# danihae/bio-image-unet

Hardware: AMD Instinct MI355X
Metric: voxels/sec fwd+bwd (higher is better)
Workload: dtype bf16; 1 GPU; cfg4: UNet3D(in_channels=1, out_channels=1, n_filter=32) input (4, 1, 128, 128, 128) per GPU, train step = forward + reference loss + backward + Adam; parallelism=dp1

## Files before the change

bio_image_unet_amd/_lib.py:

```python
from __future__ import annotations

import ctypes as C
import os

import torch

_HERE = os.path.dirname(os.path.abspath(__file__))
LIB_PATH = os.environ.get("BIU_LIB_PATH") or os.path.join(_HERE, "libbiu_hip.so")

BIU_F32, BIU_BF16 = 0, 1
BN_MAX_PARTIALS = 1024


class BiuError(RuntimeError):
    pass


class biu_act(C.Structure):
    _fields_ = [("p", C.c_void_p), ("n", C.c_int32), ("d", C.c_int32), ("h", C.c_int32), ("w", C.c_int32),
                ("c", C.c_int32), ("pitch", C.c_int32)]


class biu_pack_job(C.Structure):
    _fields_ = [("w", C.c_void_p), ("packed", C.c_void_p), ("transposed", C.c_int32), ("kind", C.c_int32), ("cin", C.c_int32),
                ("cout", C.c_int32), ("kd", C.c_int32), ("kh", C.c_int32), ("kw", C.c_int32), ("reserved", C.c_int32)]


class biu_xform(C.Structure):
    _fields_ = [("scale", C.c_void_p), ("shift", C.c_void_p), ("slope", C.c_void_p)]


class biu_mo2d_term(C.Structure):
    _fields_ = [("kind", C.c_int32), ("nb", C.c_int32), ("partial_off", C.c_longlong), ("numel", C.c_longlong), ("pixels", C.c_longlong),
                ("p0", C.c_float), ("p1", C.c_float), ("p2", C.c_float), ("weight", C.c_float)]


class biu_mo3d_term(C.Structure):
    _fields_ = [("kind", C.c_int32), ("rows", C.c_int32), ("partial_off", C.c_longlong), ("n", C.c_longlong), ("per_sample", C.c_longlong),
                ("pairs", C.c_longlong), ("p0", C.c_float), ("p1", C.c_float), ("p2", C.c_float), ("weight", C.c_float)]


class biu_aug_params(C.Structure):
    _fields_ = [("flags", C.c_uint32), ("rot_k", C.c_uint32), ("blur_k", C.c_uint32), ("index", C.c_uint32), ("m", C.c_double * 6),
                ("alpha", C.c_float), ("beta", C.c_float), ("noise_a", C.c_float), ("noise_b", C.c_float),
                ("angle", C.c_float), ("scale", C.c_float), ("dx", C.c_float), ("dy", C.c_float)]


class biu_augf_params(C.Structure):
    _fields_ = [("flags", C.c_uint32), ("rot_k", C.c_uint32), ("blur_k", C.c_uint32), ("index", C.c_uint32), ("m", C.c_double * 6),
                ("cos_t", C.c_float), ("sin_t", C.c_float), ("alpha", C.c_float), ("beta", C.c_float), ("shot_s", C.c_float),
                ("gauss_sigma", C.c_float), ("angle", C.c_float), ("scale", C.c_float), ("dx", C.c_float), ("dy", C.c_float)]


class biu_augf_source(C.Structure):
    _fields_ = [("offset", C.c_uint64), ("h", C.c_int32), ("w", C.c_int32)]


class biu_augv_source(C.Structure):
    _fields_ = [("offset", C.c_uint64), ("d", C.c_int32), ("h", C.c_int32), ("w", C.c_int32), ("z0", C.c_int32)]


_P = C.c_void_p
_A = C.POINTER(biu_act)
_X = C.POINTER(biu_xform)
_I = C.c_int
_F = C.c_float
_D = C.c_double
_Z = C.c_size_t

SIGNATURES = {
    "biu_last_error": (C.c_char_p, []),
    "biu_version": (_I, []),
    "biu_set_fp32_products": (_I, [_I]),
    "biu_set_fp32_products_3d": (_I, [_I]),
    "biu_conv_packed_bytes": (_Z, [_I, _I, _I, _I, _I, _I, _I, _I]),
    "biu_conv_pack": (_I, [_I, _P, _I, _I, _I, _I, _I, _I, _P, _P]),
    "biu_pack_batch": (_I, [_P, _I, _I, _P]),
    "biu_conv_split_workspace": (_Z, [_I, _A, _A, _I, _I, _I, _I, _I]),
    "biu_conv_fwd": (_I, [_A, _X, _P, _P, _P, _I, _I, _I, _I, _A, _P, _Z, _I, _P]),
    "biu_conv_fwd_stats_floats": (_Z, [_A, _I]),
    "biu_conv_fwd_stats": (_I, [_A, _X, _P, _P, _P, _I, _I, _I, _I, _A, _P, _Z, C.POINTER(C.c_int), _P, _Z, _I, _P]),
    "biu_conv_bwd_data": (_I, [_A, _P, _P, _I, _I, _I, _I, _A, _I, _P, _Z, _I, _P]),
    "biu_bwd_data_bnred_floats": (_Z, [_A, _I, _I]),
    "biu_conv_bwd_data_bnred": (_I, [_A, _P, _P, _I, _I, _I, _I, _A, _A, _P, _P, _P, _P, _P, _P, _Z, C.POINTER(C.c_int), _P, _Z, _I, _P]),
    "biu_convt_bwd_data_bnred": (_I, [_A, _P, _P, _I, _A, _A, _P, _P, _P, _P, _P, _P, _Z, C.POINTER(C.c_int), _I, _P]),
    "biu_conv_bwd_weight_workspace": (_Z, [_I, _I, _I, _I, _I, _I]),
    "biu_conv_bwd_weight": (_I, [_A, _X, _A, _I, _I, _I, _I, _P, _P, _P, _Z, _I, _P]),
    "biu_conv_bwd_weight_bn": (_I, [_A, _X, _A, _A, _P, _P, _P, _P, _P, _P, _I, _I, _I, _I, _P, _P, _Z, _I, _P]),
    "biu_conv_bwd_weight_bn_rank1_ok": (_I, [_A, _A, _A, _I, _I, _I, _I, _I, _I]),
    "biu_conv_bwd_weight_bn_rank1": (_I, [_A, _X, _P, _P, _I, _A, _A, _P, _P, _P, _P, _P, _P, _I, _I, _I, _I, _P, _P, _Z, _I, _P]),
    "biu_bn_stats": (_I, [_A, _P, C.POINTER(C.c_int), _I, _P]),
    "biu_bn_finalize": (_I, [_P, _I, _I, _D, _P, _P, _P, _P, _F, _F, _P, _P, _P, _P, _P]),
    "biu_bn_eval_affine": (_I, [_I, _P, _P, _P, _P, _F, _P, _P, _P]),
    "biu_xform_apply": (_I, [_A, _X, _A, _I, _P]),
    "biu_bn_bwd_reduce": (_I, [_A, _A, _P, _P, _P, _P, _P, _P, C.POINTER(C.c_int), _I, _P]),
    "biu_bn_bwd_finalize": (_I, [_P, _I, _I, _D, _P, _P, _P, _P, _P, _P, _P, _P, _P]),
    "biu_bn_bwd_finalize_eval": (_I, [_P, _I, _I, _P, _P, _P, _P, _P, _P, _P, _P]),
    "biu_bn_bwd_apply": (_I, [_A, _A, _P, _P, _P, _P, _P, _P, _A, _I, _P]),
    "biu_maxpool_fwd": (_I, [_A, _X, _A, _I, _P]),
    "biu_maxpool_bwd": (_I, [_A, _X, _A, _A, _I, _I, _P]),
    "biu_maxpool_bwd_bnred": (_I, [_A, _X, _A, _A, _I, _P, _P, _P, _Z, C.POINTER(C.c_int), _I, _P]),
    "biu_nearest_down_fwd": (_I, [_A, _X, _A, _I, _P]),
    "biu_nearest_down_bwd": (_I, [_A, _A, _I, _I, _P]),
    "biu_nearest_up_fwd": (_I, [_A, _X, _A, _I, _P]),
    "biu_upconv_ok": (_I, [_A, _A, _I]),
    "biu_upconv_packed_bytes": (_Z, [_I, _I, _I, _I]),
    "biu_upconv_pack": (_I, [_I, _P, _I, _I, _I, _P, _P]),
    "biu_upconv_bwd_data": (_I, [_A, _P, _A, _I, _I, _P]),
    "biu_upconv_bwd_weight_workspace": (_Z, [_I, _I, _I]),
    "biu_upconv_bwd_weight_bn": (_I, [_A, _X, _A, _A, _P, _P, _P, _P, _P, _P, _P, _P, _Z, _I, _P]),
    "biu_upconv_fwd_stats_floats": (_Z, [_A, _A]),
    "biu_upconv_fwd": (_I, [_A, _X, _P, _P, _A, _P, _Z, C.POINTER(C.c_int), _I, _P]),
    "biu_nearest_up_bwd": (_I, [_A, _A, _I, _I, _P]),
    "biu_bce_dice_blocks": (_I, [C.c_longlong]),
    "biu_bce_dice_fwd": (_I, [_P, _P, _I, C.c_longlong, _P, _P]),
    "biu_bce_dice_bwd": (_I, [_P, _P, _I, C.c_longlong, _P, _P, _I, _P]),
    "biu_pair_smooth_l1_blocks": (_I, [C.c_longlong]),
    "biu_pair_smooth_l1_fwd": (_I, [_P, _I, C.c_longlong, _P, _P]),
    "biu_pair_smooth_l1_bwd": (_I, [_P, _I, C.c_longlong, _P, _P, _I, _P]),
    "biu_seg_loss_finish": (_I, [_P, _I, _I, C.c_longlong, _P, _I, _F, _F, _F, _I, _F, _F, _F, _I, _F, _P, _P]),
    "biu_seg_loss_coef": (_I, [_P, _P, _I, C.c_longlong, _F, _F, _F, _I, _F, _F, _F, _I, _F, _P, _P, _P]),
    "biu_head_dlogits": (_I, [_P, _P, _P, _I, _I, _I, C.c_longlong, _P, _I, _I, _P]),
    "biu_mo2d_loss_blocks": (_I, [C.c_longlong]),
    "biu_mo2d_loss_fwd": (_I, [_I, _F, _F, _P, _I, _P, _I, _I, _I, _I, _P, _P]),
    "biu_mo2d_loss_finish": (_I, [_P, _I, _P, _P, _P]),
    "biu_mo2d_loss_coef": (_I, [_P, _I, _P, _P, _P, _P]),
    "biu_mo2d_loss_bwd": (_I, [_I, _F, _F, _P, _I, _P, _I, _I, _I, _I, _P, _P, _P]),
    "biu_mo3d_loss_blocks": (_I, [C.c_longlong]),
    "biu_mo3d_loss_fwd": (_I, [_I, _I, _P, _P, _I, _I, _I, _I, _I, _P, _P]),
    "biu_mo3d_loss_finish": (_I, [_P, _I, _P, _P, _P]),
    "biu_mo3d_loss_coef": (_I, [_P, _I, _P, _P, _P, _P]),
    "biu_mo3d_loss_bwd": (_I, [_I, _P, _P, _I, _I, _I, _I, _I, _P, _P, _P]),
    "biu_trilinear_up_fwd": (_I, [_A, _X, _A, _I, _P]),
    "biu_trilinear_up_bwd": (_I, [_A, _A, _I, _I, _P]),
    "biu_bilinear_up_fwd": (_I, [_A, _X, _A, _I, _P]),
    "biu_bilinear_up_bwd": (_I, [_A, _A, _I, _I, _P]),
    "biu_xcorr_fwd": (_I, [_A, _X, _A, _X, _A, _I, _P]),
    "biu_xcorr_bwd": (_I, [_A, _X, _A, _X, _A, _A, _A, _I, _I, _P]),
    "biu_conv_cat_ok": (_I, [_A, _A, _A, _I, _I, _I, _I, _I]),
    "biu_conv_fwd_cat": (_I, [_A, _X, _A, _X, _P, _P, _P, _I, _I, _I, _I, _A, _P, _Z, C.POINTER(C.c_int), _P, _Z, _I, _P]),
    "biu_conv_bwd_data_cat": (_I, [_A, _P, _P, _I, _I, _I, _I, _A, _I, _A, _I, _P, _Z, _I, _P]),
    "biu_conv_bwd_weight_cat": (_I, [_A, _X, _A, _X, _A, _A, _P, _P, _P, _P, _P, _P, _I, _I, _I, _I, _P, _P, _Z, _I, _P]),
    "biu_convt_packed_bytes": (_Z, [_I, _I, _I, _I, _I]),
    "biu_convt_pack": (_I, [_I, _P, _I, _I, _I, _I, _P, _P]),
    "biu_foldt_ok": (_I, [_A, _A, _A, _I]),
    "biu_foldt_packed_bytes": (_Z, [_I, _I, _I, _I]),
    "biu_foldt_pack": (_I, [_P, _P, _P, _P, _I, _I, _I, _I, _I, _P, _P]),
    "biu_foldt_fwd_stats_floats": (_Z, [_A, _A]),
    "biu_foldt_fwd_form": (_I, [_A, _A, _A, _I]),
    "biu_foldt_fwd": (_I, [_A, _X, _A, _X, _P, _A, _P, _Z, C.POINTER(C.c_int), _I, _P]),
    "biu_foldt_bwd_data_bnred_floats": (_Z, [_A]),
    "biu_foldt_bwd_data": (_I, [_A, _P, _A, _I, _A, _I, _A, _P, _P, _P, _P, _P, _P, _Z, C.POINTER(C.c_int), _P, _Z, _I, _P]),
    "biu_foldt_bwd_weight_workspace": (_Z, [_I, _I, _I, _I]),
    "biu_foldt_bwd_weight_bn": (_I, [_A, _X, _A, _X, _A, _A, _P, _P, _P, _P, _P, _P, _P, _P, _P, _P, _I, _P, _P, _P, _P, _Z, _I, _P]),
    "biu_foldt_bwd_weight_bn_phase": (_I, [_A, _X, _A, _X, _A, _A, _P, _P, _P, _P, _P, _P, _P, _P, _P, _P, _I, _P, _P, _P, _P, _Z, _I, _I, _P]),
    "biu_convt_fwd": (_I, [_A, _X, _P, _P, _P, _I, _A, _I, _P]),
    "biu_convt_bwd_data": (_I, [_A, _P, _P, _I, _A, _I, _I, _P]),
    "biu_convt_bwd_weight_workspace": (_Z, [_I, _I, _I, _I]),
    "biu_convt_bwd_weight": (_I, [_A, _X, _A, _I, _P, _P, _P, _Z, _I, _P]),
    "biu_head_fwd": (_I, [_A, _X, _P, _P, _I, _I, _P, _P, _I, _P]),
    "biu_head_bwd_workspace": (_Z, [_I]),
    "biu_head_bwd": (_I, [_A, _X, _P, _I, _P, _A, _P, _P, _P, _Z, _I, _P]),
    "biu_head_bwd_bnred": (_I, [_A, _X, _P, _I, _P, _A, _P, _P, _P, _Z, _P, _P, _P, _Z, C.POINTER(C.c_int), _I, _P]),
    "biu_max_join_fwd": (_I, [_A, _X, _A, _X, _A, _I, _P]),
    "biu_max_join_bwd": (_I, [_A, _X, _A, _X, _A, _A, _A, _I, _I, _P]),
    "biu_act_add": (_I, [_A, _A, _I, _I, _P]),
    "biu_add_relu_fwd": (_I, [_A, _X, _A, _X, _A, _I, _P]),
    "biu_add_relu_bwd": (_I, [_A, _A, _A, _A, _I, _I, _P]),
    "biu_gate_fwd": (_I, [_A, _X, _A, _X, _A, _I, _P]),
    "biu_gate_bwd": (_I, [_A, _X, _A, _X, _A, _A, _I, _A, _I, _P]),
    "biu_from_nchw": (_I, [_P, _A, _I, _P]),
    "biu_from_nchw_u8": (_I, [_P, _F, _A, _I, _P]),
    "biu_u8_to_f32": (_I, [_P, _F, _P, C.c_longlong, _P]),
    "biu_quantize_u8": (_I, [_P, _F, _P, C.c_longlong, _P]),
    "biu_stitch_add": (_I, [_P, _I, _P, _I, _I, _I, _I, _P, _P, _I, _I, _I, _I, _I, _I, _I, _P]),
    "biu_stitch_finish": (_I, [_P, _P, _I, _I, C.c_longlong, _P, _I, _P]),
    "biu_order_stats_workspace": (_Z, [C.c_longlong, _I]),
    "biu_order_stats": (_I, [_P, _I, C.c_longlong, C.c_longlong, C.c_longlong, C.POINTER(C.c_longlong), _I, _P, _P, _P, _Z, _P]),
    "biu_prep_finalize": (_I, [_P, _I, C.c_longlong, _D, _D, _I, _P, _P]),
    "biu_prep_tiles": (_I, [_P, _I, _I, _I, _I, _I, _P, _I, _I, _I, _I, _P, _I, _I, _I, _I, _P, _P]),
    "biu_lut_u8": (_I, [_P, _P, _P, C.c_longlong, _P]),
    "biu_morph_u8": (_I, [_P, _P, _I, _I, _I, _I, _I, _I, _P]),
    "biu_thin_step_u8": (_I, [_P, _P, _I, _I, _I, _I, _P, _P, _P]),
    "biu_tile_gather_u8": (_I, [_P, _I, _I, _I, _I, _P, _I, _I, _I, _I, _I, _P, _P]),
    "biu_to_nchw": (_I, [_A, _X, _P, _I, _P]),
    "biu_augment_u8": (_I, [_P, _P, _I, _I, _I, _I, _I, _P, _I, _I, C.c_ulonglong, C.c_uint, C.c_uint, _P]),
    "biu_augment_f32": (_I, [_P, _I, _P, _I, _I, _I, _I, _I, _P, _I, C.c_ulonglong, C.c_uint, C.c_uint, _P]),
    "biu_spline_prefilter_f32": (_I, [_P, _I, _P, _P, _I, _I, _I, _I, _P, _P]),
    "biu_augment_f32_cubic": (_I, [_P, _I, _P, _P, _P, _I, _I, _I, _I, _P, _P]),
    "biu_augment_f32_crop": (_I, [_P, _I, C.c_ulonglong, _P, _I, _I, _I, _I, _I, _P, _P, _F, _I, C.c_ulonglong, C.c_uint, C.c_uint, _P]),
    "biu_augment_vol_f32": (_I, [_P, _I, _P, _I, _I, _I, _I, _I, _I, _I, _P, _I, C.c_ulonglong, C.c_uint, C.c_uint, _P]),
    "biu_augment_vol_chunk": (_I, [_I] * 8),
    "biu_augment_vol_f32_crop": (_I, [_P, _I, C.c_ulonglong, _P, _I, _I, _I, _I, _I, _I, _I, _P, _P, _F, _I, C.c_ulonglong, C.c_uint, C.c_uint, _P]),
    "biu_philox_u32": (_I, [_P, C.c_longlong, C.c_ulonglong, C.c_uint, C.c_uint, C.c_uint, C.c_uint, _P]),
    "biu_adam_step": (_I, [_I, _P, _P, _P, _P, _P, _F, _F, _F, _F, _I, _F, _P]),
    "biu_adam_set_hyper": (_I, [_P, _F, _F, _F, _F, _I, _F, _P]),
    "biu_adam_step_hyper": (_I, [_I, _P, _P, _P, _P, _P, _P, _P]),
    "biu_grad_clip_scratch_floats": (_Z, [_I]),
    "biu_grad_clip": (_I, [_I, _P, _P, _F, _P, _Z, _P, _P]),
}


def _load():
    if not os.path.exists(LIB_PATH):
        raise ImportError(
            f"{LIB_PATH} is missing: the HIP kernels are not built. Run `python -c 'import __graft_entry__ as g; "
            f"g.build()'` from the repository root (needs hipcc). There is no CPU fallback.")
    lib = C.CDLL(LIB_PATH)
    for name, (res, args) in SIGNATURES.items():
        fn = getattr(lib, name)
        fn.restype = res
        fn.argtypes = args
    return lib


class _Lib:

    def __init__(self, cdll):
        object.__setattr__(self, "_c", cdll)
        object.__setattr__(self, "prof", None)
        object.__setattr__(self, "watch", None)
        object.__setattr__(self, "watched", [])
        object.__setattr__(self, "label", "")

    def __setattr__(self, k, v):
        object.__setattr__(self, k, v)

    def __getattr__(self, name):
        fn = getattr(self._c, name)
        if self.prof is None and self.watch is None:
            return fn
        if self.prof is None and self.watch != (name, self.label):
            return fn
        import torch

        def timed(*args):
            e0, e1 = torch.cuda.Event(enable_timing=True), torch.cuda.Event(enable_timing=True)
            e0.record()
            rc = fn(*args)
            e1.record()
            (self.prof if self.prof is not None else self.watched).append((name, self.label, e0, e1))
            return rc

        return timed


lib = _Lib(_load())


def ptr(t):
    return C.c_void_p(t.data_ptr()) if t is not None else None


def stream():
    return C.c_void_p(torch.cuda.current_stream().cuda_stream)


def check(status: int, what: str = ""):
    if status != 0:
        msg = lib.biu_last_error()
        raise BiuError(f"{what}: biu status {status}: {msg.decode() if msg else ''}")
```

bio_image_unet_amd/csrc/biu_api.hip:

```cpp
#include "biu_common.h"
#include "biu_internal.h"

#include <stdlib.h>
#include <string.h>

static const char* const kOffTokens[] = {
    "conv_fwd", "conv_dgrad", "conv_wgrad", "convt_fwd", "convt_dgrad", "convt_wgrad", "convt_all", "c1", "c1_mfma", "cat",
    "fused_stats", "wgrad_bn", "dgrad_bnred", "pool_pair", "pool_pipe", "pool_bnred", "head_bnred", "ksplit", "m16", "m16x2", "rr16",
    "wroll", "wroll16", "wroll2d", "upconv", "foldt", "foldall", "foldck8", "foldgemm", "croll", "froll", "prepack", "wsplitbn",
    "capturefork", "sidechain", "headrank1",
};
constexpr int kNumOffTokens = sizeof(kOffTokens) / sizeof(kOffTokens[0]);
static_assert(kNumOffTokens <= 64, "BiuEnv::off holds one bit per token");

static int off_index(const char* tok, size_t n) {
    for (int i = 0; i < kNumOffTokens; ++i)
        if (strlen(kOffTokens[i]) == n && strncmp(kOffTokens[i], tok, n) == 0) return i;
    return -1;
}
static void env_unknown(const char* var, const char* val, int n) {
    fprintf(stderr, "[biu] %s: unknown %s '%.*s' ignored\n", var, strcmp(var, "BIU_DISABLE") == 0 ? "token" : "value", n, val);
}
static bool parse_int(const char* s, int* v) {
    char* end = nullptr;
    const long r = strtol(s, &end, 10);
    if (end == s || *end) return false;
    *v = (int)r;
    return true;
}

const BiuEnv& biu_env() {
    static const BiuEnv env = [] {
        BiuEnv v{0, false, false, 0, 2, 0, 128};
        if (const char* p = getenv("BIU_DISABLE")) {
            while (true) {
                const size_t n = strcspn(p, ",");
                const int i = off_index(p, n);
                if (i >= 0) v.off |= 1ull << i;
                else if (n > 0) env_unknown("BIU_DISABLE", p, (int)n);
                if (!p[n]) break;
                p += n + 1;
            }
        }
        if (const char* e = getenv("BIU_ROLL"); e && *e) {
            if (strcmp(e, "always") == 0) v.roll_always = true;
            else env_unknown("BIU_ROLL", e, (int)strlen(e));
        }
        if (const char* e = getenv("BIU_FOLDT"); e && *e) {
            int n = 0;
            if (strcmp(e, "always") == 0) v.foldt_always = true;
            else if (strncmp(e, "cmax:", 5) == 0 && parse_int(e + 5, &n) && n > 0) v.foldt_cmax = n;
            else if (strcmp(e, "size") != 0) env_unknown("BIU_FOLDT", e, (int)strlen(e));
        }
        if (const char* e = getenv("BIU_FP32_PRODUCTS"); e && *e) {
            if (strcmp(e, "exact") == 0) v.fp32_products = 0;
            else if (strcmp(e, "bf16x3") == 0) v.fp32_products = 1;
            else if (strcmp(e, "bf16x6") != 0) env_unknown("BIU_FP32_PRODUCTS", e, (int)strlen(e));
        }
        if (const char* e = getenv("BIU_FP32_PRODUCTS_3D"); e && *e) {
            if (strcmp(e, "bf16x3") == 0) v.fp32_products_3d = 1;
            else if (strcmp(e, "bf16x6") == 0) v.fp32_products_3d = 2;
            else if (strcmp(e, "exact") != 0) env_unknown("BIU_FP32_PRODUCTS_3D", e, (int)strlen(e));
        }
        if (const char* e = getenv("BIU_FALL_MAXCA"); e && *e) {
            int n = 0;
            if (parse_int(e, &n)) v.fall_maxca = n;
            else env_unknown("BIU_FALL_MAXCA", e, (int)strlen(e));
        }
        return v;
    }();
    return env;
}

bool biu_off(const char* token) {
    const int i = off_index(token, strlen(token));
    return i >= 0 && ((biu_env().off >> i) & 1);
}

static void warn_slow_path(const char* op, const biu_act* x, const biu_act* y, int taps) {
    const double macs = (double)nvox(y) * x->c * y->c * taps;
    if (macs < 4e9) return;
    static int shown = 0;
    if (shown++ < 8)
        fprintf(stderr, "[biu] %s: %d->%d channels on %lld voxels takes the any-shape kernel (%.1f GMAC): expect it to be slow; "
                        "the MFMA path needs channel counts that are multiples of 8 (>= 16), dilation 1, 16-byte aligned slices "
                        "and samples under 4 GB\n", op, x->c, y->c, (long long)nvox(y), macs * 1e-9);
}

static bool conv_args_ok(const biu_act* x, const biu_act* y, int kd, int kh, int kw, int dil) {
    if (!valid_act(x) || !valid_act(y) || !same_space(x, y)) return false;
    if (!((kd == 1 || kd == 3) && kh == 3 && kw == 3) && !(kd == 1 && kh == 1 && kw == 1)) return false;
    return dil >= 1;
}

extern "C" size_t biu_conv_packed_bytes(int kind, int cin, int cout, int kd, int kh, int kw, int dilation, int dtype) {
    return biu_mfma_packed_bytes(kind, cin, cout, kd, kh, kw, dilation, dtype);
}

extern "C" int biu_conv_pack(int kind, const float* w, int cin, int cout, int kd, int kh, int kw, int dtype,
                             void* packed, biu_stream stream) {
    BIU_REQUIRE(w && packed, BIU_ERR_SHAPE, "conv_pack: null pointer");
    BIU_REQUIRE(biu_mfma_packed_bytes(kind, cin, cout, kd, kh, kw, 1, dtype) > 0, BIU_ERR_UNSUPPORTED,
                "conv_pack: shape (cin=%d, cout=%d, k=%dx%dx%d) is served by the direct kernels", cin, cout, kd, kh, kw);
    return biu_mfma_pack(kind, w, cin, cout, kd, kh, kw, dtype, packed, (hipStream_t)stream);
}

extern "C" int biu_pack_batch(const biu_pack_job* jobs, int n, int dtype, biu_stream stream) {
    BIU_REQUIRE(n >= 0 && (jobs || n == 0), BIU_ERR_SHAPE, "pack_batch: null job table");
    BIU_REQUIRE(n <= 65535, BIU_ERR_UNSUPPORTED, "pack_batch: more than 65535 jobs");
    return biu_mfma_pack_batch(jobs, n, dtype, (hipStream_t)stream);
}

static bool will_split(int cin, const biu_act* y, const biu_act* y1, int kd, int dtype, const void* ws, size_t ws_bytes) {
    const size_t need = biu_mfma_conv_split_bytes(cin, y, y1, kd, dtype);
    return need > 0 && ws && ws_bytes >= need;
}

extern "C" size_t biu_conv_split_workspace(int cin, const biu_act* y, const biu_act* y1, int kd, int kh, int kw, int dilation, int dtype) {
    if (!y || !valid_act(y) || (y1 && !valid_act(y1)) || kh != 3 || kw != 3 || (kd != 1 && kd != 3) || dilation != 1) return 0;
    biu_act xprobe = *y;
    xprobe.c = xprobe.pitch = cin;
    biu_act yall = *y;
    if (y1) yall.c = y->c + y1->c;
    if (!biu_mfma_conv_ok(&xprobe, &yall, kd, kh, kw, dilation, dtype)) return 0;
    return biu_mfma_conv_split_bytes(cin, y, y1, kd, dtype);
}

extern "C" int biu_conv_fwd_stats(const biu_act* x, const biu_xform* xf, const float* w, const void* packed,
                                  const float* bias, int kd, int kh, int kw, int dilation, const biu_act* y,
                                  float* bn_partial, size_t bn_partial_floats, int* bn_nblk, void* ws, size_t ws_bytes, int dtype,
                                  biu_stream stream) {
    BIU_REQUIRE(conv_args_ok(x, y, kd, kh, kw, dilation), BIU_ERR_SHAPE,
                "conv_fwd: x/y extents differ or unsupported kernel %dx%dx%d dil %d", kd, kh, kw, dilation);
    BIU_REQUIRE(w && bn_partial && bn_nblk, BIU_ERR_SHAPE, "conv_fwd_stats: null pointer");
    *bn_nblk = 0;
    if (!biu_off("c1") && !biu_off("fused_stats") && biu_c1m_ok(x, y, kd, kh, kw, dilation, dtype)) {
        const int nb = biu_c1m_fwd_rows(y, kd);
        if ((size_t)nb * y->c * 2 <= bn_partial_floats) {
            int rc = biu_c1m_fwd(x, xf, w, bias, kd, y, bn_partial, (hipStream_t)stream);
            if (rc == BIU_OK) *bn_nblk = nb;
            return rc;
        }
    }
    if (packed && !biu_off("conv_fwd") && !biu_off("fused_stats") && biu_mfma_conv_ok(x, y, kd, kh, kw, dilation, dtype) &&
        !will_split(x->c, y, nullptr, kd, dtype, ws, ws_bytes)) {
        const int nb = biu_mfma_conv_stat_rows(y, kd, x, dtype);
        if ((size_t)nb * y->c * 2 <= bn_partial_floats) {
            int rc = biu_mfma_conv(x, xf, packed, bias, kd, kh, kw, y, 0, bn_partial, dtype, (hipStream_t)stream);
            if (rc == BIU_OK) *bn_nblk = nb;
            return rc;
        }
    }
    int rc = biu_conv_fwd(x, xf, w, packed, bias, kd, kh, kw, dilation, y, ws, ws_bytes, dtype, stream);
    if (rc != BIU_OK) return rc;
    BIU_REQUIRE(bn_partial_floats >= (size_t)BIU_BN_MAX_PARTIALS * y->c * 2, BIU_ERR_WORKSPACE, "conv_fwd_stats: partial buffer too small");
    return biu_bn_stats(y, bn_partial, bn_nblk, dtype, stream);
}

extern "C" size_t biu_conv_fwd_stats_floats(const biu_act* y, int kd) {
    size_t a = (size_t)BIU_BN_MAX_PARTIALS * y->c * 2, b = (size_t)biu_mfma_conv_bricks(y, kd == 3 ? 3 : 1) * y->c * 2;
    return a > b ? a : b;
}

extern "C" int biu_conv_fwd(const biu_act* x, const biu_xform* xf, const float* w, const void* packed,
                            const float* bias, int kd, int kh, int kw, int dilation, const biu_act* y, void* ws, size_t ws_bytes,
                            int dtype, biu_stream stream) {
    BIU_REQUIRE(conv_args_ok(x, y, kd, kh, kw, dilation), BIU_ERR_SHAPE,
                "conv_fwd: x/y extents differ or unsupported kernel %dx%dx%d dil %d", kd, kh, kw, dilation);
    BIU_REQUIRE(w, BIU_ERR_SHAPE, "conv_fwd: null weight");
    if (!biu_off("c1") && biu_c1m_ok(x, y, kd, kh, kw, dilation, dtype))
        return biu_c1m_fwd(x, xf, w, bias, kd, y, nullptr, (hipStream_t)stream);
    if (!biu_off("c1") && biu_c1_conv_ok(x, y, kd, kh, kw, dilation, dtype))
        return biu_c1_conv_fwd(x, xf, w, bias, kd, y, dtype, (hipStream_t)stream);
    if (packed && !biu_off("conv_fwd") && biu_mfma_conv_ok(x, y, kd, kh, kw, dilation, dtype))
        return biu_mfma_conv(x, xf, packed, bias, kd, kh, kw, y, 0, nullptr, dtype, (hipStream_t)stream, nullptr, nullptr, ws, ws_bytes);
    warn_slow_path("conv_fwd", x, y, kd * kh * kw);
    return biu_conv_fwd_direct(x, xf, w, bias, kd, kh, kw, dilation, y, dtype, (hipStream_t)stream);
}

extern "C" int biu_conv_bwd_data(const biu_act* dy, const float* w, const void* packed, int kd, int kh, int kw,
                                 int dilation, const biu_act* dx, int accumulate, void* ws, size_t ws_bytes, int dtype, biu_stream stream) {
    BIU_REQUIRE(conv_args_ok(dy, dx, kd, kh, kw, dilation), BIU_ERR_SHAPE, "conv_bwd_data: dy/dx extents differ");
    BIU_REQUIRE(w, BIU_ERR_SHAPE, "conv_bwd_data: null weight");
    if (packed && !biu_off("conv_dgrad") && biu_mfma_conv_ok(dy, dx, kd, kh, kw, dilation, dtype))
        return biu_mfma_conv(dy, nullptr, packed, nullptr, kd, kh, kw, dx, accumulate, nullptr, dtype, (hipStream_t)stream, nullptr, nullptr, ws, ws_bytes);
    warn_slow_path("conv_bwd_data", dx, dy, kd * kh * kw);
    return biu_conv_bwd_data_direct(dy, w, kd, kh, kw, dilation, dx, accumulate, dtype, (hipStream_t)stream);
}

extern "C" size_t biu_bwd_data_bnred_floats(const biu_act* dx, int kd, int transposed) {
    size_t a = (size_t)BIU_BN_MAX_PARTIALS * dx->c * 2;
    size_t b = (size_t)(transposed ? biu_mfma_convt_dgrad_bricks(dx, kd) : biu_mfma_conv_bricks(dx, kd == 3 ? 3 : 1)) * dx->c * 2;
    return a > b ? a : b;
}
extern "C" int biu_conv_bwd_data_bnred(const biu_act* dy, const float* w, const void* packed, int kd, int kh, int kw, int dilation,
                                       const biu_act* dx, const biu_act* y_up, const float* scale, const float* shift,
                                       const float* slope, const float* mean, const float* invstd, float* partial,
                                       size_t partial_floats, int* nblk, void* ws, size_t ws_bytes, int dtype, biu_stream stream) {
    BIU_REQUIRE(conv_args_ok(dy, dx, kd, kh, kw, dilation) && valid_act(y_up) && same_space(y_up, dx) && y_up->c == dx->c, BIU_ERR_SHAPE,
                "conv_bwd_data_bnred: extents differ");
    BIU_REQUIRE(w && scale && shift && mean && invstd && partial && nblk, BIU_ERR_SHAPE, "conv_bwd_data_bnred: null pointer");
    const size_t es = dsize(dtype);
    const bool yok = ((uintptr_t)y_up->p % 16) == 0 && ((size_t)y_up->pitch * es) % 16 == 0;
    if (packed && yok && !biu_off("conv_dgrad") && !biu_off("dgrad_bnred") && biu_mfma_conv_ok(dy, dx, kd, kh, kw, dilation, dtype) &&
        !will_split(dy->c, dx, nullptr, kd, dtype, ws, ws_bytes)) {
        const int nb = biu_mfma_conv_stat_rows(dx, kd, dy, dtype, true);
        if ((size_t)nb * dx->c * 2 <= partial_floats) {
            BnRedFuse red{y_up, scale, shift, slope, mean, invstd};
            int rc = biu_mfma_conv(dy, nullptr, packed, nullptr, kd, kh, kw, dx, 0, partial, dtype, (hipStream_t)stream, &red);
            if (rc == BIU_OK) *nblk = nb;
            return rc;
        }
    }
    int rc = biu_conv_bwd_data(dy, w, packed, kd, kh, kw, dilation, dx, 0, ws, ws_bytes, dtype, stream);
    if (rc != BIU_OK) return rc;
    BIU_REQUIRE(partial_floats >= (size_t)BIU_BN_MAX_PARTIALS * dx->c * 2, BIU_ERR_WORKSPACE, "conv_bwd_data_bnred: partial buffer too small");
    return biu_bn_bwd_reduce(dx, y_up, scale, shift, slope, mean, invstd, partial, nblk, dtype, stream);
}
extern "C" int biu_convt_bwd_data_bnred(const biu_act* dy, const float* w, const void* packed, int kd, const biu_act* dx,
                                        const biu_act* y_up, const float* scale, const float* shift, const float* slope,
                                        const float* mean, const float* invstd, float* partial, size_t partial_floats, int* nblk,
                                        int dtype, biu_stream stream) {
    BIU_REQUIRE(valid_act(dx) && valid_act(dy) && w && biu_convt_shapes_ok(dx, dy, kd) && valid_act(y_up) && same_space(y_up, dx) &&
                    y_up->c == dx->c, BIU_ERR_SHAPE, "convt_bwd_data_bnred: extents differ");
    BIU_REQUIRE(scale && shift && mean && invstd && partial && nblk, BIU_ERR_SHAPE, "convt_bwd_data_bnred: null pointer");
    const size_t es = dsize(dtype);
    const bool yok = ((uintptr_t)y_up->p % 16) == 0 && ((size_t)y_up->pitch * es) % 16 == 0;
    if (packed && yok && !biu_off("convt_dgrad") && !biu_off("dgrad_bnred") && biu_mfma_convt_ok(1, dx, dy, kd, dtype) &&
        biu_convt_all_ok(dx, dy, kd, dtype)) {
        const int nb = biu_convt_all_dgrad_rows(dx, dy, kd);
        if ((size_t)nb * dx->c * 2 <= partial_floats) {
            BnRedFuse red{y_up, scale, shift, slope, mean, invstd};
            int rc = biu_convt_all_dgrad(dy, packed, kd, dx, 0, (hipStream_t)stream, partial, &red);
            if (rc == BIU_OK) *nblk = nb;
            return rc;
        }
    }
    if (packed && yok && !biu_off("convt_dgrad") && !biu_off("dgrad_bnred") && biu_mfma_convt_ok(1, dx, dy, kd, dtype)) {
        const int nb = biu_mfma_convt_dgrad_rows(dx, kd, dy->c, dtype);
        if ((size_t)nb * dx->c * 2 <= partial_floats) {
            BnRedFuse red{y_up, scale, shift, slope, mean, invstd};
            int rc = biu_mfma_convt_dgrad(dy, packed, kd, dx, 0, dtype, (hipStream_t)stream, partial, &red);
            if (rc == BIU_OK) *nblk = nb;
            return rc;
        }
    }
    int rc = biu_convt_bwd_data(dy, w, packed, kd, dx, 0, dtype, stream);
    if (rc != BIU_OK) return rc;
    BIU_REQUIRE(partial_floats >= (size_t)BIU_BN_MAX_PARTIALS * dx->c * 2, BIU_ERR_WORKSPACE, "convt_bwd_data_bnred: partial buffer too small");
    return biu_bn_bwd_reduce(dx, y_up, scale, shift, slope, mean, invstd, partial, nblk, dtype, stream);
}

extern "C" size_t biu_conv_bwd_weight_workspace(int cin, int cout, int kd, int kh, int kw, int dtype) {
    if (cin == 1 && kh == 3 && kw == 3) {
        const size_t a = biu_c1_wgrad_workspace(cout, kd), b = biu_c1m_wgrad_workspace(cout, kd);
        return a > b ? a : b;
    }
    return biu_mfma_wgrad_workspace(cin, cout, kd, kh, kw, dtype);
}

extern "C" int biu_conv_bwd_weight(const biu_act* x, const biu_xform* xf, const biu_act* dy, int kd, int kh, int kw,
                                   int dilation, float* dw, float* dbias, void* ws, size_t ws_bytes, int dtype,
                                   biu_stream stream) {
    BIU_REQUIRE(conv_args_ok(x, dy, kd, kh, kw, dilation), BIU_ERR_SHAPE, "conv_bwd_weight: x/dy extents differ");
    BIU_REQUIRE(dw, BIU_ERR_SHAPE, "conv_bwd_weight: null dw");
    if (!biu_off("c1") && biu_c1m_ok(x, dy, kd, kh, kw, dilation, dtype) && ws && ws_bytes >= biu_c1m_wgrad_workspace(dy->c, kd)) {
        int rc = biu_c1m_wgrad(x, xf, dy, nullptr, kd, dw, ws, ws_bytes, (hipStream_t)stream);
        if (rc == BIU_OK && dbias) rc = biu_chan_sum(dy, dbias, dtype, (hipStream_t)stream);
        return rc;
    }
    if (!biu_off("c1") && biu_c1_conv_ok(x, dy, kd, kh, kw, dilation, dtype) && ws && ws_bytes >= biu_c1_wgrad_workspace(dy->c, kd)) {
        int rc = biu_c1_conv_wgrad(x, xf, dy, kd, dw, ws, ws_bytes, dtype, (hipStream_t)stream);
        if (rc == BIU_OK && dbias) rc = biu_chan_sum(dy, dbias, dtype, (hipStream_t)stream);
        return rc;
    }
    if (!biu_off("conv_wgrad") && biu_mfma_wgrad_ok(x, dy, kd, kh, kw, dilation, dtype)) {
        BIU_REQUIRE(ws && ws_bytes >= biu_mfma_wgrad_workspace(x->c, dy->c, kd, kh, kw, dtype), BIU_ERR_WORKSPACE,
                    "conv_bwd_weight: workspace too small");
        return biu_mfma_wgrad(x, xf, dy, kd, kh, kw, dw, dbias, ws, ws_bytes, dtype, (hipStream_t)stream);
    }
    warn_slow_path("conv_bwd_weight", x, dy, kd * kh * kw);
    return biu_conv_bwd_weight_direct(x, xf, dy, kd, kh, kw, dilation, dw, dbias, dtype, (hipStream_t)stream);
}

extern "C" int biu_conv_bwd_weight_bn(const biu_act* x, const biu_xform* xf, const biu_act* da, const biu_act* y,
                                      const float* scale, const float* shift, const float* slope, const float* coefA,
                                      const float* coefB, const float* coefC, int kd, int kh, int kw, int dilation,
                                      float* dw, void* ws, size_t ws_bytes, int dtype, biu_stream stream) {
    BIU_REQUIRE(conv_args_ok(x, da, kd, kh, kw, dilation) && valid_act(y) && same_space(y, da) && y->c == da->c, BIU_ERR_SHAPE,
                "conv_bwd_weight_bn: extents differ");
    BIU_REQUIRE(dw && scale && shift && coefA && coefB && coefC, BIU_ERR_SHAPE, "conv_bwd_weight_bn: null pointer");
    const size_t es = dsize(dtype);
    const bool yok = ((uintptr_t)y->p % 16) == 0 && ((size_t)y->pitch * es) % 16 == 0 &&
                     (i64)y->d * y->h * y->w * y->pitch * (i64)es < (1LL << 32) - 65536;
    if (!biu_off("c1") && !biu_off("wgrad_bn") && yok && biu_c1m_ok(x, da, kd, kh, kw, dilation, dtype) && ws &&
        ws_bytes >= biu_c1m_wgrad_workspace(da->c, kd)) {
        BnBwdFuse bn{y, scale, shift, slope, coefA, coefB, coefC};
        return biu_c1m_wgrad(x, xf, da, &bn, kd, dw, ws, ws_bytes, (hipStream_t)stream);
    }
    if (!biu_off("conv_wgrad") && !biu_off("wgrad_bn") && yok && biu_mfma_wgrad_ok(x, da, kd, kh, kw, dilation, dtype)) {
        BIU_REQUIRE(ws && ws_bytes >= biu_mfma_wgrad_workspace(x->c, da->c, kd, kh, kw, dtype), BIU_ERR_WORKSPACE,
                    "conv_bwd_weight_bn: workspace too small");
        BnBwdFuse bn{y, scale, shift, slope, coefA, coefB, coefC};
        return biu_mfma_wgrad(x, xf, da, kd, kh, kw, dw, nullptr, ws, ws_bytes, dtype, (hipStream_t)stream, &bn);
    }
    int rc = biu_bn_bwd_apply(da, y, scale, shift, slope, coefA, coefB, coefC, da, dtype, stream);
    if (rc != BIU_OK) return rc;
    return biu_conv_bwd_weight(x, xf, da, kd, kh, kw, dilation, dw, nullptr, ws, ws_bytes, dtype, stream);
}

static bool rank1_y_ok(const biu_act* y, int dtype) {
    const size_t es = dsize(dtype);
    return ((uintptr_t)y->p % 16) == 0 && ((size_t)y->pitch * es) % 16 == 0 && (i64)y->d * y->h * y->w * y->pitch * (i64)es < (1LL << 32) - 65536;
// ... 269 lines not shown
```

bio_image_unet_amd/csrc/biu_conv_mfma.hip:

```cpp
#include "biu_internal.h"
#include <type_traits>
#include <cstring>
#include <mutex>
#include <cstdlib>

typedef float floatx16 __attribute__((ext_vector_type(16)));
typedef float floatx4 __attribute__((ext_vector_type(4)));
typedef __bf16 bf16x8 __attribute__((ext_vector_type(8)));

template <typename T> struct Frag;
template <> struct Frag<bf16_t> {
    static constexpr int PE = 8;
    __device__ static __forceinline__ void mma(const uint4& a, const uint4& b, floatx16& c) {
        c = __builtin_amdgcn_mfma_f32_32x32x16_bf16(__builtin_bit_cast(bf16x8, a), __builtin_bit_cast(bf16x8, b), c, 0, 0, 0);
    }
    __device__ static __forceinline__ void unpack(const uint4& v, float* f) {
        const unsigned u[4] = {v.x, v.y, v.z, v.w};
#pragma unroll
        for (int i = 0; i < 4; ++i) {
            f[2 * i] = __uint_as_float(u[i] << 16);
            f[2 * i + 1] = __uint_as_float(u[i] & 0xffff0000u);
        }
    }
    __device__ static __forceinline__ uint4 pack(const float* f) {
// ... 3388 lines not shown
            RSTAMP(3);
            finish(other, (s + 2) & 3, (s + 1) % 3, 2 * s + 2, true);
        }
        RSTAMP(4);
        __syncthreads();
        RSTAMP(5);
#ifdef BIU_DIAG
        dsum_[7] += 1;
#endif
    };
    __syncthreads();
    for (int kc = 0;; ++kc) {
        const int col = column_of(kc);
        if (col >= ncols) break;
        set_column(col);
        fetch_all(sl0, fetch_ctx(0, -1, 0, 0), false);
        wait_vmcnt<0>();
        finish(sl0, 0, 0, 0, false);
        fetch_all(sl0, fetch_ctx(1, 1, 0, 0), true);
        if (nsteps > 1) fetch_all(sl1, fetch_ctx(2, 3, 1, 2), true);
        wait_vmcnt<0>();
        finish(sl0, 1, 0, 0, true);
        __syncthreads();
        for (int s = 0; s < nsteps; s += 2) {
            step(sl0, sl1, s);
            if (s + 1 < nsteps) step(sl1, sl0, s + 1);
        }
    }

#ifdef BIU_DIAG
    if (wdiag && (tid & 63) == 0 && (tid >> 6) == (BIU_DIAG_WAVE)) {
        for (int q_ = 0; q_ < 8; ++q_) atomicAdd(wdiag + q_, dsum_[q_]);
        atomicAdd(wdiag + 8, __builtin_readcyclecounter() - t0c_);
        atomicAdd(wdiag + 9, __builtin_amdgcn_s_memrealtime() - t0r_);
    }
#endif
    const int hf = lane >> 5;
    const int jj = jt * CT + (lane & 31);
    if constexpr (A16) {
        const int uj = wave & 3;
        if (jj < a.CB) {
#pragma unroll
            for (int u = 0; u < 2; ++u) {
                if (u == 1 && !has_x) break;
                const int kw = u ? 2 : (wave >> 2);
#pragma unroll
                for (int tb = 0; tb < 3; ++tb)
#pragma unroll
                    for (int e = 0; e < 16; ++e) {
                        const int kd = uj - (e >> 3), ii = (e & 3) + 8 * ((e >> 2) & 1) + 4 * hf;
                        if (kd >= 0 && kd <= 2 && ii < a.CA) atomicAdd(a.ws + ((size_t)((kd * 3 + tb) * 3 + kw) * a.CA + ii) * a.CB + jj, acc[u * 3 + tb][e]);
                    }
            }
        }
        return;
    }
    if (jj < a.CB) {
#pragma unroll
        for (int t2 = 0; t2 < IPW; ++t2) {
            const int tap = tapid[t2];
            if (tap < TAPS) {
#pragma unroll
                for (int e = 0; e < 16; ++e) {
                    const int ii = it * CT + (e & 3) + 8 * (e >> 2) + 4 * hf;
                    if (ii < a.CA) atomicAdd(a.ws + ((size_t)tap * a.CA + ii) * a.CB + jj, acc[t2][e]);
                }
            }
        }
    }
}

static bool wroll_fits(const WgradArgs& a) {
    const int ncols = a.N * ((a.GH + WR_TH - 1) / WR_TH) * ((a.GW + WR_TW - 1) / WR_TW);
    return a.GD >= 8 && ncols >= 8;
}
static bool wroll2d_fits(const WgradArgs& a, i64 bytesA, i64 bytesB, i64 bytesY) {
    const int ncols = ((a.GH + WR_TH - 1) / WR_TH) * ((a.GW + WR_TW - 1) / WR_TW);
    return a.N >= 8 && ncols >= 8 && a.CA * a.CB > 1024 && bytesA < BIU_MAX_SAMPLE_BYTES && bytesB < BIU_MAX_SAMPLE_BYTES && bytesY < BIU_MAX_SAMPLE_BYTES;
}

static int launch_wgrad_roll(WgradArgs a, hipStream_t st, bool k2d = false) {
    if (k2d) { a.GD = a.BD = a.N; a.N = 1; }
    const bool a16 = !k2d && a.CA == 16 && !biu_off("wroll16");
    if (a.r1_dl && !(a16 && a.py)) return biu_fail(BIU_ERR_UNSUPPORTED, "wgrad_roll: the rank-one loader exists for the fused 16-channel form only");
    a.nbd = 1;
    a.nbh = (a.GH + WR_TH - 1) / WR_TH;
    a.nbw = (a.GW + WR_TW - 1) / WR_TW;
    const int ncols = a.N * a.nbh * a.nbw;
    a.nbricks = ncols;
    const int nit = (a.CA + 31) / 32;
    a.njt = (a.CB + 31) / 32;
    a.bricks_per_block = 0;
#ifdef BIU_DIAG
    a.diag = biu_diag_buffer;
#else
    a.diag = nullptr;
#endif
    static bool attr_set = false;
    if (!attr_set) {
        if (hipFuncSetAttribute((const void*)k_wgrad_roll<false, false>, hipFuncAttributeMaxDynamicSharedMemorySize, (int)WR_LDS) != hipSuccess ||
            hipFuncSetAttribute((const void*)k_wgrad_roll<true, false>, hipFuncAttributeMaxDynamicSharedMemorySize, (int)WR_LDS) != hipSuccess ||
            hipFuncSetAttribute((const void*)k_wgrad_roll<false, true>, hipFuncAttributeMaxDynamicSharedMemorySize, (int)WR_LDS) != hipSuccess ||
            hipFuncSetAttribute((const void*)k_wgrad_roll<true, true>, hipFuncAttributeMaxDynamicSharedMemorySize, (int)WR_LDS) != hipSuccess ||
            hipFuncSetAttribute((const void*)k_wgrad_roll<false, false, true>, hipFuncAttributeMaxDynamicSharedMemorySize, (int)WR_LDS) != hipSuccess ||
            hipFuncSetAttribute((const void*)k_wgrad_roll<true, false, true>, hipFuncAttributeMaxDynamicSharedMemorySize, (int)WR_LDS) != hipSuccess ||
            hipFuncSetAttribute((const void*)k_wgrad_roll<true, false, true, true>, hipFuncAttributeMaxDynamicSharedMemorySize, (int)WR_LDS) != hipSuccess)
            return biu_fail(BIU_ERR_LAUNCH, "wgrad_roll: cannot reserve %zu bytes of LDS", WR_LDS);
        attr_set = true;
    }
    auto launch = [&](int jt_begin, int jt_count, int write_back, bool with_bn) {
        WgradArgs b = a;
        if (!with_bn) b.py = nullptr;
        b.jt_begin = jt_begin; b.jt_count = jt_count; b.write_back = write_back;
        const int pairs = nit * jt_count;
        int g = num_cus() / pairs;
        if (g >= 16) g = grid_per_column(num_cus(), pairs);
        if (g < 1) g = 1;
        if (g > ncols) g = ncols;
        if (k2d) {
            if (with_bn) hipLaunchKernelGGL((k_wgrad_roll<true, true>), dim3(g, pairs), dim3(512), WR_LDS, st, b);
            else hipLaunchKernelGGL((k_wgrad_roll<false, true>), dim3(g, pairs), dim3(512), WR_LDS, st, b);
        } else if (a16) {
            if (with_bn && b.r1_dl) hipLaunchKernelGGL((k_wgrad_roll<true, false, true, true>), dim3(g, pairs), dim3(512), WR_LDS, st, b);
            else if (with_bn) hipLaunchKernelGGL((k_wgrad_roll<true, false, true>), dim3(g, pairs), dim3(512), WR_LDS, st, b);
            else hipLaunchKernelGGL((k_wgrad_roll<false, false, true>), dim3(g, pairs), dim3(512), WR_LDS, st, b);
        } else {
            if (with_bn) hipLaunchKernelGGL((k_wgrad_roll<true, false>), dim3(g, pairs), dim3(512), WR_LDS, st, b);
            else hipLaunchKernelGGL((k_wgrad_roll<false, false>), dim3(g, pairs), dim3(512), WR_LDS, st, b);
        }
    };
    if (a.py && a.njt > 1) {
        launch(0, 1, 1, true);
        BIU_CHECK_LAUNCH("wgrad_roll");
        launch(1, a.njt - 1, 0, false);
    } else {
        launch(0, a.njt, a.py ? 1 : 0, a.py != nullptr);
    }
    BIU_CHECK_LAUNCH("wgrad_roll");
    return BIU_OK;
}

__global__ void k_wgrad_finalize(const float* __restrict__ ws, int rows, int cols, int taps, float* __restrict__ dw, int ld_cols = 0, int c_off = 0) {
    const size_t total = (size_t)rows * cols * taps;
    for (size_t i = (size_t)blockIdx.x * blockDim.x + threadIdx.x; i < total; i += (size_t)gridDim.x * blockDim.x) {
        const int tap = (int)(i % taps);
        const size_t r = i / taps;
        const int c = (int)(r % cols);
        const int rr = (int)(r / cols);
        const size_t o = ld_cols > 0 ? ((size_t)rr * ld_cols + c_off + c) * taps + tap : i;
        dw[o] = ws[((size_t)tap * rows + rr) * cols + c];
    }
}

__global__ void k_zero_f32(float* __restrict__ p, size_t n, float* __restrict__ q, int nq) {
    for (size_t i = (size_t)blockIdx.x * blockDim.x + threadIdx.x; i < n; i += (size_t)gridDim.x * blockDim.x) p[i] = 0.f;
    if (q && blockIdx.x == 0)
        for (int i = threadIdx.x; i < nq; i += blockDim.x) q[i] = 0.f;
}
static int zero_ws(void* ws, size_t bytes, float* extra, int nextra, hipStream_t st) {
    const size_t n = bytes / sizeof(float);
    hipLaunchKernelGGL(k_zero_f32, dim3(grid_for((i64)n, 256, 1024)), dim3(256), 0, st, (float*)ws, n, extra, nextra);
    if (hipGetLastError() != hipSuccess) return biu_fail(BIU_ERR_LAUNCH, "wgrad: zero-fill launch failed");
    return BIU_OK;
}

static bool wgrad_chan_ok(int cin, int cout) { return cin >= 16 && cin % 8 == 0 && cout >= 16 && cout % 8 == 0; }

static size_t wgrad_acc_bytes(int cin, int cout, int taps) { return (((size_t)cin * cout * taps * sizeof(float)) + 255) & ~(size_t)255; }

size_t biu_mfma_wgrad_workspace(int cin, int cout, int kd, int kh, int kw, int dtype) {
    if (!wgrad_chan_ok(cin, cout)) return 0;
    const size_t red = biu_chan_sum_workspace(cout);
    if (kh == 3 && kw == 3 && (kd == 1 || kd == 3)) return wgrad_acc_bytes(cin, cout, kd * 9) + red;
    if (kh == 2 && kw == 2 && (kd == 1 || kd == 2)) return wgrad_acc_bytes(cin, cout, kd * 4) + red;
    return 0;
}

static bool wgrad_ptrs_ok(const biu_act* x, const biu_act* dy, int dtype) {
    const size_t es = dsize(dtype);
    if ((uintptr_t)x->p % 16 || (uintptr_t)dy->p % 16 || ((size_t)x->pitch * es) % 16 || ((size_t)dy->pitch * es) % 16) return false;
    if (sample_bytes(x, es) >= BIU_MAX_SAMPLE_BYTES || sample_bytes(dy, es) >= BIU_MAX_SAMPLE_BYTES) return false;
    const i64 plane_x = (i64)x->h * x->w, plane_y = (i64)dy->h * dy->w;
    return 10 * (plane_x > plane_y ? plane_x : plane_y) < (1LL << 24);
}

bool biu_mfma_wgrad_ok(const biu_act* x, const biu_act* dy, int kd, int kh, int kw, int dilation, int dtype) {
    if (dilation != 1 || kh != 3 || kw != 3 || (kd != 1 && kd != 3)) return false;
    if (!wgrad_chan_ok(x->c, dy->c) || !wgrad_ptrs_ok(x, dy, dtype)) return false;
    if (kd == 1 && x->d != 1) return false;
    return true;
}

bool biu_mfma_convt_wgrad_ok(const biu_act* x, const biu_act* dy, int kd, int dtype) {
    return (kd == 1 || kd == 2) && wgrad_chan_ok(x->c, dy->c) && wgrad_ptrs_ok(x, dy, dtype);
}

template <typename T, int KD, int KHW, int S, int TD, int TH, int TW, int KSPLIT, int NI = 1, bool RR16 = false, bool FALL = false>
static int launch_wgrad(WgradArgs a, hipStream_t st) {
    constexpr int SD = (KD == 1) ? 1 : S;
    constexpr int HV = ((TD - 1) * SD + (FALL ? 3 : KD)) * ((TH - 1) * S + (FALL ? 3 : KHW)) * ((TW - 1) * S + (FALL ? 3 : KHW));
    constexpr int BV = (FALL ? 8 : 1) * TD * TH * TW;
    constexpr int PPV_ = 32 / (16 / (int)sizeof(T));
    constexpr int NA_ = (BV * PPV_ * NI + 511) / 512, NB_ = (HV * PPV_ + 511) / 512;
    const size_t tile_bytes = (size_t)(HV + BV * NI) * 32 * (SplitOf<T>::parts ? 2 * SplitOf<T>::parts : sizeof(T));
    const size_t lds_bytes = tile_bytes + (3 + 9 * NI) * 32 * sizeof(float) + (wgrad_tab_in_lds(tile_bytes, NA_ + NB_) ? (size_t)(NA_ + NB_) * 512 * sizeof(unsigned) : 0);
    a.nbd = (a.GD + TD - 1) / TD;
    a.nbh = (a.GH + TH - 1) / TH;
    a.nbw = (a.GW + TW - 1) / TW;
    a.nbricks = a.N * a.nbd * a.nbh * a.nbw;
    const int nit = (a.CA + 32 * NI - 1) / (32 * NI);
    a.njt = (a.CB + 31) / 32;
    a.bricks_per_block = 0;
    auto kern = k_wgrad_pipe<T, KD, KHW, S, TD, TH, TW, KSPLIT, NI, RR16, FALL>;
    static bool attr_set = false;
    if (!attr_set) {
        if (hipFuncSetAttribute((const void*)kern, hipFuncAttributeMaxDynamicSharedMemorySize, (int)lds_bytes) != hipSuccess)
            return biu_fail(BIU_ERR_LAUNCH, "wgrad_pipe: cannot reserve %zu bytes of LDS", lds_bytes);
        attr_set = true;
    }
    auto launch = [&](int jt_begin, int jt_count, int write_back, bool with_bn) {
        WgradArgs b = a;
#ifdef BIU_DIAG
        b.diag = biu_diag_buffer;
#else
        b.diag = nullptr;
#endif
        if (!with_bn) b.py = nullptr;
        b.jt_begin = jt_begin; b.jt_count = jt_count; b.write_back = write_back;
        const int pairs = nit * jt_count;
        int g = num_cus() / pairs;
        if (g >= 16) g = grid_per_column(num_cus(), pairs);
        if (g < 1) g = 1;
        if (g > b.nbricks) g = b.nbricks;
        hipLaunchKernelGGL(kern, dim3(g, pairs), dim3(512), lds_bytes, st, b);
    };
    if (a.py && a.njt > 1) {
        launch(0, 1, 1, true);
        BIU_CHECK_LAUNCH("wgrad_pipe");
        launch(1, a.njt - 1, 0, false);
    } else {
        launch(0, a.njt, a.py ? 1 : 0, a.py != nullptr);
    }
    BIU_CHECK_LAUNCH("wgrad_pipe");
    return BIU_OK;
}

static int wgrad_xf(const biu_xform* xf, const float** s, const float** b, const float** l) {
    const bool has = xf && (xf->scale || xf->shift || xf->slope);
    if (has) BIU_REQUIRE(xf->scale && xf->shift && xf->slope, BIU_ERR_UNSUPPORTED, "wgrad_mfma: partial biu_xform");
    *s = has ? xf->scale : nullptr;
    *b = has ? xf->shift : nullptr;
    *l = has ? xf->slope : nullptr;
    return BIU_OK;
}

bool biu_mfma_wgrad_rank1_ok(const biu_act* x, const biu_act* dy, int kd, int kh, int kw, int dilation, int dtype) {
    if (dtype != BIU_BF16 || kd != 3 || dy->c != 16 || !biu_mfma_wgrad_ok(x, dy, kd, kh, kw, dilation, dtype)) return false;
    if (biu_off("wroll") || biu_off("wroll16") || (x->c == 16 && !biu_off("rr16"))) return false;
    if (!biu_off("wsplitbn") && x->c > 32 && nvox(dy) <= 4 * 32 * 32 * 32) return false;
    if ((i64)x->d * x->h * x->w * 4 >= (1LL << 32)) return false;
    WgradArgs a;
    a.N = x->n; a.GD = x->d; a.GH = x->h; a.GW = x->w;
    return biu_env().roll_always || wroll_fits(a);
}

int biu_mfma_wgrad(const biu_act* x, const biu_xform* xf, const biu_act* dy, int kd, int kh, int kw, float* dw, float* dbias,
                   void* ws, size_t ws_bytes, int dtype, hipStream_t st, const BnBwdFuse* bn, const biu_act* x1, const biu_xform* xf1,
                   int dw_ld_cols, int dw_c_off) {
    WgradArgs a;
    int rc_ = BIU_OK;
    if (bn && !biu_off("wsplitbn") && dtype == BIU_BF16 && kd == 3 && x->c + (x1 ? x1->c : 0) > 32 && nvox(dy) <= 4 * 32 * 32 * 32) {
        rc_ = biu_bn_bwd_apply(dy, bn->y, bn->scale, bn->shift, bn->slope, bn->cA, bn->cB, bn->cC, dy, dtype, (biu_stream)st);
        if (rc_ != BIU_OK) return rc_;
        bn = nullptr;
    }
    if (bn) {
        a.py = (const char*)bn->y->p; a.ypitch = bn->y->pitch;
        a.bn_scale = bn->scale; a.bn_shift = bn->shift; a.bn_slope = bn->slope;
        a.bn_cA = bn->cA; a.bn_cB = bn->cB; a.bn_cC = bn->cC;
        a.r1_dl = bn->r1_dl; a.r1_w = bn->r1_w;
    } else {
        a.py = nullptr; a.ypitch = 0;
        a.bn_scale = a.bn_shift = a.bn_slope = a.bn_cA = a.bn_cB = a.bn_cC = nullptr;
    }
    a.pa = (const char*)dy->p;  a.apitch = dy->pitch;  a.CA = dy->c;
    a.pb = (const char*)x->p;   a.bpitch = x->pitch;   a.CB = x->c;
    a.dbias_out = nullptr;
    a.fold_par = -1;
    a.pb1 = nullptr; a.bpitch1 = 0; a.bsplit = 0; a.bs1_ = a.bb1_ = a.bl1_ = nullptr;
    if (x1) {
        a.pb1 = (const char*)x1->p; a.bpitch1 = x1->pitch; a.bsplit = x->c; a.CB = x->c + x1->c;
        rc_ = wgrad_xf(xf1, &a.bs1_, &a.bb1_, &a.bl1_);
        if (rc_) return rc_;
    }
    a.ws = (float*)ws;
    a.as_ = a.ab_ = a.al_ = nullptr;
    int rc = wgrad_xf(xf, &a.bs_, &a.bb_, &a.bl_);
    if (rc) return rc;
    a.N = x->n;
    a.GD = a.BD = x->d; a.GH = a.BH = x->h; a.GW = a.BW = x->w;
    const int taps = kd * 9;
    const size_t need = wgrad_acc_bytes(a.CA, a.CB, taps);
    BIU_REQUIRE(ws_bytes >= need + (dbias ? biu_chan_sum_workspace(dy->c) : 0), BIU_ERR_WORKSPACE, "wgrad_mfma: workspace %zu too small", ws_bytes);
    if (int zr = zero_ws(ws, need, nullptr, 0, st)) return zr;
    if (a.r1_dl) rc = launch_wgrad_roll(a, st);
    else if (dtype == BIU_BF16 && kd == 3 && a.CB == 16 && !x1 && !biu_off("rr16")) rc = launch_wgrad<bf16_t, 3, 3, 1, 4, 8, 16, 1, 1, true>(a, st);
    else if (dtype == BIU_BF16 && kd == 3 && !biu_off("wroll") && wroll_fits(a)) rc = launch_wgrad_roll(a, st);
    else if (dtype == BIU_BF16 && kd == 1 && !biu_off("wroll") && !biu_off("wroll2d") &&
             wroll2d_fits(a, (i64)nvox(dy) * dy->pitch * 2, (i64)nvox(x) * x->pitch * 2 > (x1 ? (i64)nvox(x1) * x1->pitch * 2 : 0) ? (i64)nvox(x) * x->pitch * 2 : (i64)nvox(x1) * x1->pitch * 2,
                          bn ? (i64)nvox(bn->y) * bn->y->pitch * 2 : 0))
        rc = launch_wgrad_roll(a, st, true);
    else if (dtype == BIU_BF16) rc = (kd == 3) ? launch_wgrad<bf16_t, 3, 3, 1, 4, 8, 16, 1>(a, st) : launch_wgrad<bf16_t, 1, 3, 1, 1, 16, 32, 4>(a, st);
    else if (kd == 1 && x3_mode_of(kd, dtype) == 2) rc = launch_wgrad<f32x6_t, 1, 3, 1, 1, 16, 16, 4>(a, st);
    else if (kd == 1 && x3_mode_of(kd, dtype) == 1) rc = launch_wgrad<f32x3_t, 1, 3, 1, 1, 16, 16, 4>(a, st);
    else if (kd == 3 && x3_mode_of(kd, dtype) == 2) rc = launch_wgrad<f32x6_t, 3, 3, 1, 2, 4, 16, 1>(a, st);
    else if (kd == 3 && x3_mode_of(kd, dtype) == 1) rc = launch_wgrad<f32x3_t, 3, 3, 1, 2, 4, 16, 1>(a, st);
    else rc = (kd == 3) ? launch_wgrad<float, 3, 3, 1, 4, 4, 16, 1>(a, st) : launch_wgrad<float, 1, 3, 1, 1, 16, 16, 4>(a, st);
    if (rc != BIU_OK) return rc;
    hipLaunchKernelGGL(k_wgrad_finalize, dim3(grid_for((i64)a.CA * a.CB * taps, 256, 2048)), dim3(256), 0, st, (const float*)ws,
                       a.CA, a.CB, taps, dw, dw_ld_cols, dw_c_off);
    BIU_CHECK_LAUNCH("wgrad_finalize");
    if (dbias) return biu_chan_sum_vec(dy, dbias, (char*)ws + need, dtype, st);
    return BIU_OK;
}

__global__ void k_upconv_wgrad_unfold(const float* __restrict__ ws, size_t slice_f, int cout, int cin, float* __restrict__ dw) {
    const size_t total = (size_t)cout * cin * 27;
    for (size_t idx = (size_t)blockIdx.x * blockDim.x + threadIdx.x; idx < total; idx += (size_t)gridDim.x * blockDim.x) {
        const int k = (int)(idx % 27);
        const size_t r = idx / 27;
        const int ci = (int)(r % cin), co = (int)(r / cin);
        const int kk[3] = {k / 9, (k / 3) % 3, k % 3};
        float sum = 0.f;
        for (int p = 0; p < 8; ++p) {
            int t = 0;
#pragma unroll
            for (int ax = 0; ax < 3; ++ax) {
                const int pa = (p >> (2 - ax)) & 1;
                const int ta = pa == 0 ? (kk[ax] >= 1 ? 1 : 0) : (kk[ax] == 2 ? 1 : 0);
                t |= ta << (2 - ax);
            }
            sum += ws[(size_t)p * slice_f + ((size_t)t * cout + co) * cin + ci];
        }
        dw[idx] = sum;
    }
}
size_t biu_mfma_upconv_wgrad_workspace(int cin, int cout, int dtype) {
    if ((dtype != BIU_BF16 && dtype != BIU_F32) || !wgrad_chan_ok(cin, cout)) return 0;
    return 8 * wgrad_acc_bytes(cout, cin, 8);
}
int biu_mfma_upconv_wgrad(const biu_act* x, const biu_xform* xf, const biu_act* dy, float* dw, void* ws, size_t ws_bytes, int dtype,
                          hipStream_t st, const BnBwdFuse* bn) {
    WgradArgs a;
    if (bn) {
        a.py = (const char*)bn->y->p; a.ypitch = bn->y->pitch;
        a.bn_scale = bn->scale; a.bn_shift = bn->shift; a.bn_slope = bn->slope;
        a.bn_cA = bn->cA; a.bn_cB = bn->cB; a.bn_cC = bn->cC;
    } else {
        a.py = nullptr; a.ypitch = 0;
        a.bn_scale = a.bn_shift = a.bn_slope = a.bn_cA = a.bn_cB = a.bn_cC = nullptr;
    }
    a.pa = (const char*)dy->p;  a.apitch = dy->pitch;  a.CA = dy->c;
    a.pb = (const char*)x->p;   a.bpitch = x->pitch;   a.CB = x->c;
    a.dbias_out = nullptr;
    a.pb1 = nullptr; a.bpitch1 = 0; a.bsplit = 0; a.bs1_ = a.bb1_ = a.bl1_ = nullptr;
    a.as_ = a.ab_ = a.al_ = nullptr;
    int rc = wgrad_xf(xf, &a.bs_, &a.bb_, &a.bl_);
    if (rc) return rc;
    a.N = x->n;
    a.GD = a.BD = x->d; a.GH = a.BH = x->h; a.GW = a.BW = x->w;
    const size_t slice = wgrad_acc_bytes(a.CA, a.CB, 8);
    BIU_REQUIRE(ws_bytes >= 8 * slice, BIU_ERR_WORKSPACE, "upconv_wgrad: workspace %zu too small (need %zu)", ws_bytes, 8 * slice);
    if (int zr = zero_ws(ws, 8 * slice, nullptr, 0, st)) return zr;
    a.fold_slice_f = slice / sizeof(float);
    if (dtype == BIU_BF16 && a.CA <= biu_env().fall_maxca && bn == nullptr && !biu_off("foldall")) {
        a.ws = (float*)ws;
        a.fold_par = 8;
        rc = launch_wgrad<bf16_t, 2, 2, 1, 2, 4, 16, 8, 1, false, true>(a, st);
        if (rc != BIU_OK) return rc;
    } else
    for (int p = 0; p < 8; ++p) {
        a.ws = (float*)((char*)ws + (size_t)p * slice);
        a.fold_par = p;
        if (x3_mode_of(2, dtype) == 2) rc = launch_wgrad<f32x6_t, 2, 2, 1, 4, 4, 16, 1>(a, st);
        else if (x3_mode_of(2, dtype) == 1) rc = launch_wgrad<f32x3_t, 2, 2, 1, 4, 4, 16, 1>(a, st);
        else if (a.CA > 32) rc = dtype == BIU_BF16 ? launch_wgrad<bf16_t, 2, 2, 1, 4, 8, 16, 1, 2>(a, st) : launch_wgrad<float, 2, 2, 1, 4, 4, 16, 1, 2>(a, st);
        else rc = dtype == BIU_BF16 ? launch_wgrad<bf16_t, 2, 2, 1, 4, 8, 16, 1>(a, st) : launch_wgrad<float, 2, 2, 1, 4, 4, 16, 1>(a, st);
        if (rc != BIU_OK) return rc;
    }
    if (!dw) return BIU_OK;
    hipLaunchKernelGGL(k_upconv_wgrad_unfold, dim3(grid_for((i64)a.CA * a.CB * 27, 256, 2048)), dim3(256), 0, st, (const float*)ws, slice / sizeof(float),
                       a.CA, a.CB, dw);
    BIU_CHECK_LAUNCH("upconv_wgrad_unfold");
    return BIU_OK;
}

int biu_mfma_foldt_dgrad(const biu_act* dy, const void* packed, const biu_act* dx_low, int acc_low, const biu_act* dskip, int acc_skip, int dtype,
                         hipStream_t st, float* bn_partial_low, const BnRedFuse* red_low, void* ws, size_t ws_bytes) {
    const FoldtBlob b = foldt_blob(dx_low->c, dskip->c, dy->c, dtype);
    const char* base = (const char*)packed;
    int rc = biu_mfma_conv(dy, nullptr, base + b.sdg, nullptr, 3, 3, 3, dskip, acc_skip, nullptr, dtype, st, nullptr, nullptr, ws, ws_bytes);
    if (rc != BIU_OK) return rc;
    return biu_mfma_upconv_dgrad(dy, base + b.dg, dx_low, acc_low, dtype, st, bn_partial_low, red_low);
}
constexpr int FOLDT_SUM_BLOCKS = 1024;
inline size_t foldt_sum_lds(int c) { return (size_t)27 * (c > 256 ? c : 256) * sizeof(float); }
template <typename T>
__global__ __launch_bounds__(256) void k_foldt_border_sums(const char* __restrict__ dy, ShellDims sd, int c, int pitch, float* __restrict__ partial) {
    extern __shared__ float tab[];
    const int lanes_c = c < 256 ? c : 256, slots = 256 / lanes_c;
    for (int i = threadIdx.x; i < slots * 27 * c; i += 256) tab[i] = 0.f;
    __syncthreads();
    const int cc0 = (int)threadIdx.x % lanes_c, slot = (int)threadIdx.x / lanes_c;
    const long nsv = sd.nA + sd.nB + sd.nC;
    const long stride = (long)gridDim.x * slots;
    if (slot < slots) {
        float* mine = tab + (size_t)slot * 27 * c;
        for (long v = (long)blockIdx.x * slots + slot; v < nsv; v += 4 * stride) {
            const T* p[4]; float* r[4]; bool ok[4];
#pragma unroll
            for (int u = 0; u < 4; ++u) {
                const long vv = v + u * stride;
                ok[u] = vv < nsv;
                long vox = 0; int st = 0;
                if (ok[u]) shell_voxel(sd, vv, vox, st);
                p[u] = (const T*)dy + (size_t)vox * pitch;
                r[u] = mine + st * c;
            }
            for (int cc = cc0; cc < c; cc += lanes_c) {
                float val[4];
#pragma unroll
                for (int u = 0; u < 4; ++u) val[u] = ok[u] ? (float)p[u][cc] : 0.f;
#pragma unroll
                for (int u = 0; u < 4; ++u) if (ok[u]) r[u][cc] += val[u];
            }
        }
    }
    __syncthreads();
    for (int i = threadIdx.x; i < 27 * c; i += 256) {
        float t = 0.f;
        for (int sl = 0; sl < slots; ++sl) t += tab[(size_t)sl * 27 * c + i];
        partial[(size_t)blockIdx.x * 27 * c + i] = t;
    }
}
constexpr int FOLDT_RED_SPLIT = 8;
__global__ __launch_bounds__(256) void k_foldt_reduce_tables(const float* __restrict__ partial, int nblocks, int cout, float* __restrict__ R) {
    __shared__ float red[256];
    const int s_ = (int)blockIdx.x, per = (nblocks + (int)gridDim.y - 1) / (int)gridDim.y;
    const int b0 = (int)blockIdx.y * per, b1 = b0 + per < nblocks ? b0 + per : nblocks;
    for (int c0 = 0; c0 < cout; c0 += 32) {
        const int co = c0 + (int)(threadIdx.x & 31), part = (int)(threadIdx.x >> 5);
        float s4[4] = {0.f, 0.f, 0.f, 0.f};
        if (co < cout) {
            int b = b0 + part;
            for (; b + 24 < b1; b += 32)
#pragma unroll
                for (int u = 0; u < 4; ++u) s4[u] += partial[((size_t)(b + 8 * u) * 27 + s_) * cout + co];
            for (; b < b1; b += 8) s4[0] += partial[((size_t)b * 27 + s_) * cout + co];
        }
        red[threadIdx.x] = (s4[0] + s4[1]) + (s4[2] + s4[3]);
        __syncthreads();
        if (threadIdx.x < 32 && co < cout) {
            float t = 0.f;
            for (int pp = 0; pp < 8; ++pp) t += red[pp * 32 + threadIdx.x];
            R[((size_t)blockIdx.y * 27 + s_) * cout + co] = t;
        }
        __syncthreads();
    }
}
__global__ __launch_bounds__(256) void k_foldt_inside_sums(const float* __restrict__ R, int nsplit, int cout, float* __restrict__ Sk, const float* __restrict__ total) {
    __shared__ float red[256];
    const int k = (int)blockIdx.x, co = (int)blockIdx.y * 32 + (int)(threadIdx.x & 31), part = (int)(threadIdx.x >> 5);
    float sum = (total && part == 0 && co < cout) ? total[co] : 0.f;
    if (co < cout)
        for (int sp = part; sp < nsplit; sp += 8) {
#pragma unroll 9
            for (int s_ = 0; s_ < 27; ++s_) {
                const float v = R[((size_t)sp * 27 + s_) * cout + co];
                sum -= (s_ != 13 && tap_outside(k, s_)) ? v : 0.f;
            }
        }
    red[threadIdx.x] = sum;
    __syncthreads();
    if (threadIdx.x < 32 && co < cout) {
        float t = 0.f;
        for (int pp = 0; pp < 8; ++pp) t += red[pp * 32 + threadIdx.x];
        Sk[k * cout + co] = t;
    }
}
__global__ __launch_bounds__(256) void k_foldt_chain_wconv(const float* __restrict__ G, size_t slice_f, const float* __restrict__ wt, int cin_low, int cup, int cout,
                                                           int ccat, float* __restrict__ dwc, const float* __restrict__ bt, const float* __restrict__ Sk) {
    __shared__ long offA[8], offB[8];
    const int k = (int)blockIdx.z;
    if (threadIdx.x < 8) {
        int t, q;
        foldt_tq((int)threadIdx.x, k, t, q);
        offA[threadIdx.x] = (long)threadIdx.x * (long)slice_f + (long)t * cout * cin_low;
        offB[threadIdx.x] = q;
    }
    __syncthreads();
    const int m0 = (int)blockIdx.y * 32, n0 = (int)blockIdx.x * 32;
    float acc[2][2] = {{0.f, 0.f}, {0.f, 0.f}};
    small_gemm_tile(8, cout, cup, cin_low, m0, n0, SgView{G, cin_low, 1}, offA, SgView{wt, (long)cup * 8, 8}, offB, acc);
    const int ty = threadIdx.x >> 4, tx = threadIdx.x & 15;
#pragma unroll
    for (int i = 0; i < 2; ++i)
#pragma unroll
        for (int j = 0; j < 2; ++j) {
            const int co = m0 + 2 * ty + i, c = n0 + 2 * tx + j;
            if (co < cout && c < cup) dwc[((size_t)co * ccat + c) * 27 + k] = bt ? fmaf(bt[c], Sk[k * cout + co], acc[i][j]) : acc[i][j];
        }
}
__global__ __launch_bounds__(256) void k_foldt_chain_wt(const float* __restrict__ G, size_t slice_f, const float* __restrict__ wc, int cin_low, int cup, int cout,
                                                        int ccat, float* __restrict__ dwt) {
    __shared__ long offA[27], offB[27];
    const int q = (int)blockIdx.z;
    if (threadIdx.x < 27) {
        const int k = (int)threadIdx.x, kk[3] = {k / 9, (k / 3) % 3, k % 3};
        int p = 0, t = 0;
#pragma unroll
        for (int ax = 0; ax < 3; ++ax) {
            const int qa = (q >> (2 - ax)) & 1, pa = (qa + kk[ax] + 1) & 1;
            const int ta = pa == 0 ? (kk[ax] >= 1 ? 1 : 0) : (kk[ax] == 2 ? 1 : 0);
            p |= pa << (2 - ax); t |= ta << (2 - ax);
        }
        offA[k] = (long)p * (long)slice_f + (long)t * cout * cin_low;
        offB[k] = k;
    }
    __syncthreads();
    const int m0 = (int)blockIdx.y * 32, n0 = (int)blockIdx.x * 32;
    float acc[2][2] = {{0.f, 0.f}, {0.f, 0.f}};
    small_gemm_tile(27, cin_low, cup, cout, m0, n0, SgView{G, 1, cin_low}, offA, SgView{wc, (long)ccat * 27, 27}, offB, acc);
    const int ty = threadIdx.x >> 4, tx = threadIdx.x & 15;
#pragma unroll
    for (int i = 0; i < 2; ++i)
#pragma unroll
        for (int j = 0; j < 2; ++j) {
            const int ci = m0 + 2 * ty + i, c = n0 + 2 * tx + j;
            if (ci < cin_low && c < cup) dwt[((size_t)ci * cup + c) * 8 + q] = acc[i][j];
        }
}
__global__ __launch_bounds__(256) void k_foldt_chain_bt(const float* __restrict__ Sk, const float* __restrict__ wc, int cup, int cout, int ccat, float* __restrict__ dbt) {
    __shared__ float red[256];
    const int c = (int)blockIdx.x;
    float sum = 0.f;
    for (int i = threadIdx.x; i < cout * 27; i += 256) {
        const int co = i / 27, k = i % 27;
        sum = fmaf(wc[((size_t)co * ccat + c) * 27 + k], Sk[k * cout + co], sum);
    }
    red[threadIdx.x] = sum;
    __syncthreads();
    for (int st = 128; st > 0; st >>= 1) {
        if ((int)threadIdx.x < st) red[threadIdx.x] += red[threadIdx.x + st];
        __syncthreads();
    }
    if (threadIdx.x == 0) dbt[c] = red[0];
}
size_t biu_mfma_foldt_wgrad_workspace(int cin_low, int cskip, int cout, int dtype) {
    if (!wgrad_chan_ok(cin_low, cout) || !wgrad_chan_ok(cskip, cout)) return 0;
    const size_t g = 8 * wgrad_acc_bytes(cout, cin_low, 8), sk = biu_mfma_wgrad_workspace(cskip, cout, 3, 3, 3, dtype);
    return (g > sk ? g : sk) + al256((size_t)FOLDT_SUM_BLOCKS * 27 * cout * sizeof(float)) + al256((size_t)(1 + FOLDT_RED_SPLIT) * 27 * cout * sizeof(float)) +
           al256(biu_fold_gemm_layout_floats(cin_low, cin_low, cout) * sizeof(float));
}
int biu_mfma_foldt_wgrad(const biu_act* x_low, const biu_xform* xf_low, const biu_act* skip, const biu_xform* xf_skip, const biu_act* da, const BnBwdFuse* bn,
                         const float* dy_sum, const float* w_conv, const float* w_t, const float* b_t, int cup, float* dw_conv, float* dw_t, float* db_t, void* ws, size_t ws_bytes,
                         int dtype, hipStream_t st, int phases) {
    const int cin_low = x_low->c, cskip = skip->c, cout = da->c, ccat = cup + cskip;
    const size_t need = biu_mfma_foldt_wgrad_workspace(cin_low, cskip, cout, dtype);
    BIU_REQUIRE(need > 0 && ws_bytes >= need, BIU_ERR_WORKSPACE, "foldt_wgrad: workspace %zu too small (need %zu)", ws_bytes, need);
    const size_t pbytes = al256((size_t)FOLDT_SUM_BLOCKS * 27 * cout * sizeof(float)), sbytes = al256((size_t)(1 + FOLDT_RED_SPLIT) * 27 * cout * sizeof(float));
    const size_t lbytes = al256(biu_fold_gemm_layout_floats(cin_low, cin_low, cout) * sizeof(float));
    const size_t main_bytes = need - pbytes - sbytes - lbytes;
    float* R = (float*)((char*)ws + main_bytes);
    float* Sk = (float*)((char*)ws + main_bytes + pbytes);
    float* lay = (float*)((char*)ws + main_bytes + pbytes + sbytes);
    const bool has_bias = b_t != nullptr || db_t != nullptr;
    if (phases & 1) {
        int rc = biu_mfma_wgrad(skip, xf_skip, da, 3, 3, 3, dw_conv, nullptr, ws, main_bytes, dtype, st, bn, nullptr, nullptr, ccat, cup);
        if (rc != BIU_OK) return rc;
    }
    if (phases & 4) {
        int rc = biu_mfma_upconv_wgrad(x_low, xf_low, da, nullptr, ws, main_bytes, dtype, st, nullptr);
        if (rc != BIU_OK) return rc;
    }
    if (!(phases & 2)) return BIU_OK;
    if (has_bias) {
        const ShellDims sh = shell_dims(da->n, da->d, da->h, da->w);
        BIU_DISPATCH_DTYPE(dtype, hipLaunchKernelGGL(k_foldt_border_sums<T>, dim3(FOLDT_SUM_BLOCKS), dim3(256), foldt_sum_lds(cout), st,
                                                     (const char*)da->p, sh, da->c, da->pitch, R));
        BIU_CHECK_LAUNCH("foldt_border_sums");
        float* Rsum = Sk + 27 * cout;
        hipLaunchKernelGGL(k_foldt_reduce_tables, dim3(27, FOLDT_RED_SPLIT), dim3(256), 0, st, (const float*)R, FOLDT_SUM_BLOCKS, cout, Rsum);
        hipLaunchKernelGGL(k_foldt_inside_sums, dim3(27, (cout + 31) / 32), dim3(256), 0, st, (const float*)Rsum, FOLDT_RED_SPLIT, cout, Sk, dy_sum);
        BIU_CHECK_LAUNCH("foldt_inside_sums");
    }
    const size_t slice_f = wgrad_acc_bytes(cout, cin_low, 8) / sizeof(float);
    if (cup <= cin_low && biu_fold_gemm_ok(cin_low, cup, cout)) {
        int rc = biu_fold_gemm_layouts(w_conv, ccat, cup, cout, w_t, cin_low, lay, st);
        if (rc == BIU_OK) rc = biu_fold_gemm_chain((const float*)ws, slice_f, lay, cin_low, cup, cout, ccat, dw_conv, dw_t, b_t, (const float*)Sk, st);
        if (rc != BIU_OK) return rc;
        if (db_t) hipLaunchKernelGGL(k_foldt_chain_bt, dim3(cup), dim3(256), 0, st, (const float*)Sk, w_conv, cup, cout, ccat, db_t);
        BIU_CHECK_LAUNCH("foldt_chain_bt");
        return BIU_OK;
    }
    hipLaunchKernelGGL(k_foldt_chain_wconv, dim3((cup + 31) / 32, (cout + 31) / 32, 27), dim3(256), 0, st, (const float*)ws, slice_f, w_t, cin_low, cup, cout, ccat,
                       dw_conv, b_t, (const float*)Sk);
    hipLaunchKernelGGL(k_foldt_chain_wt, dim3((cup + 31) / 32, (cin_low + 31) / 32, 8), dim3(256), 0, st, (const float*)ws, slice_f, w_conv, cin_low, cup, cout, ccat,
                       dw_t);
    if (db_t) hipLaunchKernelGGL(k_foldt_chain_bt, dim3(cup), dim3(256), 0, st, (const float*)Sk, w_conv, cup, cout, ccat, db_t);
    BIU_CHECK_LAUNCH("foldt_chain");
    return BIU_OK;
}

int biu_mfma_convt_wgrad(const biu_act* x, const biu_xform* xf, const biu_act* dy, int kd, float* dw, float* dbias, void* ws,
                         size_t ws_bytes, int dtype, hipStream_t st) {
    WgradArgs a;
    a.py = nullptr; a.ypitch = 0;
    a.bn_scale = a.bn_shift = a.bn_slope = a.bn_cA = a.bn_cB = a.bn_cC = nullptr;
    a.pa = (const char*)x->p;   a.apitch = x->pitch;   a.CA = x->c;
    a.pb = (const char*)dy->p;  a.bpitch = dy->pitch;  a.CB = dy->c;
    a.fold_par = -1;
    a.pb1 = nullptr; a.bpitch1 = 0; a.bsplit = 0; a.bs1_ = a.bb1_ = a.bl1_ = nullptr;
    a.ws = (float*)ws;
    int rc = wgrad_xf(xf, &a.as_, &a.ab_, &a.al_);
    if (rc) return rc;
    a.bs_ = a.bb_ = a.bl_ = nullptr;
    a.N = x->n;
    a.GD = x->d; a.GH = x->h; a.GW = x->w;
    a.BD = dy->d; a.BH = dy->h; a.BW = dy->w;
    const int taps = kd * 4;
    const size_t need = wgrad_acc_bytes(a.CA, a.CB, taps);
    BIU_REQUIRE(ws_bytes >= need + (dbias ? biu_chan_sum_workspace(dy->c) : 0), BIU_ERR_WORKSPACE, "convt_wgrad_mfma: workspace %zu too small", ws_bytes);
    a.dbias_out = dbias;
    if (int zr = zero_ws(ws, need, dbias, dbias ? dy->c : 0, st)) return zr;
    const bool wide = a.CA > 32;
    if (dtype == BIU_BF16) {
        if (wide) rc = (kd == 2) ? launch_wgrad<bf16_t, 2, 2, 2, 2, 4, 16, 2, 2>(a, st) : launch_wgrad<bf16_t, 1, 2, 2, 1, 8, 16, 4, 2>(a, st);
        else rc = (kd == 2) ? launch_wgrad<bf16_t, 2, 2, 2, 2, 4, 16, 2>(a, st) : launch_wgrad<bf16_t, 1, 2, 2, 1, 8, 16, 4>(a, st);
    } else {
        if (kd == 1 && x3_mode_of(kd, dtype) == 2) rc = wide ? launch_wgrad<f32x6_t, 1, 2, 2, 1, 8, 16, 4, 2>(a, st) : launch_wgrad<f32x6_t, 1, 2, 2, 1, 8, 16, 4>(a, st);
        else if (kd == 1 && x3_mode_of(kd, dtype) == 1) rc = wide ? launch_wgrad<f32x3_t, 1, 2, 2, 1, 8, 16, 4, 2>(a, st) : launch_wgrad<f32x3_t, 1, 2, 2, 1, 8, 16, 4>(a, st);
        else if (kd == 2 && x3_mode_of(kd, dtype) == 2) rc = launch_wgrad<f32x6_t, 2, 2, 2, 1, 4, 16, 2>(a, st);
        else if (kd == 2 && x3_mode_of(kd, dtype) == 1) rc = launch_wgrad<f32x3_t, 2, 2, 2, 2, 4, 16, 2>(a, st);
        else if (wide && kd == 1) rc = launch_wgrad<float, 1, 2, 2, 1, 8, 16, 4, 2>(a, st);
        else rc = (kd == 2) ? launch_wgrad<float, 2, 2, 2, 2, 4, 16, 2>(a, st) : launch_wgrad<float, 1, 2, 2, 1, 8, 16, 4>(a, st);
    }
    if (rc != BIU_OK) return rc;
    hipLaunchKernelGGL(k_wgrad_finalize, dim3(grid_for((i64)a.CA * a.CB * taps, 256, 2048)), dim3(256), 0, st, (const float*)ws,
                       a.CA, a.CB, taps, dw);
    BIU_CHECK_LAUNCH("convt_wgrad_finalize");
    return BIU_OK;
}
```

bio_image_unet_amd/csrc/biu_internal.h:

```cpp
#pragma once
#include "biu_common.h"

struct BiuEnv {
    unsigned long long off;
    bool roll_always;
    bool foldt_always;
    int foldt_cmax;
    int fp32_products;
    int fp32_products_3d;
    int fall_maxca;
};
const BiuEnv& biu_env();
bool biu_off(const char* token);

#define BIU_HIDDEN __attribute__((visibility("hidden")))
extern "C" BIU_HIDDEN int biu_conv_fwd_direct(const biu_act* x, const biu_xform* xf, const float* w, const float* bias, int kd,
                                   int kh, int kw, int dil, const biu_act* y, int dtype, hipStream_t st);
extern "C" BIU_HIDDEN int biu_conv_bwd_data_direct(const biu_act* dy, const float* w, int kd, int kh, int kw, int dil,
                                        const biu_act* dx, int accumulate, int dtype, hipStream_t st);
extern "C" BIU_HIDDEN int biu_conv_bwd_weight_direct(const biu_act* x, const biu_xform* xf, const biu_act* dy, int kd, int kh,
                                          int kw, int dil, float* dw, float* dbias, int dtype, hipStream_t st);
extern "C" BIU_HIDDEN int biu_convt_fwd_direct(const biu_act* x, const biu_xform* xf, const float* w, const float* bias, int kd,
                                    const biu_act* y, int dtype, hipStream_t st);
extern "C" BIU_HIDDEN int biu_convt_bwd_data_direct(const biu_act* dy, const float* w, int kd, const biu_act* dx, int accumulate,
                                         int dtype, hipStream_t st);
extern "C" BIU_HIDDEN int biu_convt_bwd_weight_direct(const biu_act* x, const biu_xform* xf, const biu_act* dy, int kd, float* dw,
                                           float* dbias, int dtype, hipStream_t st);
int biu_chan_sum(const biu_act* a, float* out, int dtype, hipStream_t st);
bool biu_convt_shapes_ok(const biu_act* lo, const biu_act* hi, int kd);

size_t biu_mfma_packed_bytes(int kind, int cin, int cout, int kd, int kh, int kw, int dilation, int dtype);
int biu_mfma_pack(int kind, const float* w, int cin, int cout, int kd, int kh, int kw, int dtype, void* packed,
                  hipStream_t st);
bool biu_mfma_conv_ok(const biu_act* x, const biu_act* y, int kd, int kh, int kw, int dilation, int dtype);
struct BnRedFuse {
    const biu_act* y;
    const float *scale, *shift, *slope, *mean, *invstd;
};
bool biu_mfma_conv_cat_ok(const biu_act* x0, const biu_act* x1, const biu_act* y, int kd, int kh, int kw, int dilation, int dtype);
struct ConvCat {
    const biu_act* x1; const biu_xform* xf1;
    const biu_act* y1; int accumulate1;
};
int biu_mfma_conv(const biu_act* x, const biu_xform* xf, const void* packed, const float* bias, int kd, int kh, int kw,
                  const biu_act* y, int accumulate, float* bn_partial, int dtype, hipStream_t st, const BnRedFuse* red = nullptr,
                  const ConvCat* cat = nullptr, void* split_ws = nullptr, size_t split_ws_bytes = 0);
bool biu_conv_roll_ok(const biu_act* x, const biu_act* y, int dtype, bool has_cat, int accumulate, bool red);
int biu_conv_roll_mshape(const biu_act* x, const biu_act* y, int dtype);
int biu_conv_roll_rows(const biu_act* x, const biu_act* y, int dtype);
int biu_conv_roll(const biu_act* x, const biu_xform* xf, const void* packed, const float* bias, const biu_act* y, float* bn_partial, const BnRedFuse* red,
                  hipStream_t st, int accumulate = 0);
bool biu_fold_roll_ok(const biu_act* x_low, const biu_act* y, int dtype);
int biu_fold_roll(const biu_act* x_low, const biu_xform* xf, const void* packed_fwd, const float* bias_sum, const float* fix, const biu_act* y, hipStream_t st);
size_t biu_fold_gemm_layout_floats(int cin_low, int cup, int cout);
bool biu_fold_gemm_ok(int cin_low, int cup, int cout);
int biu_fold_gemm_layouts(const float* w_conv, int ccat, int cup, int cout, const float* w_t, int cin_low, float* layouts, hipStream_t st);
int biu_fold_gemm_compose(const float* layouts, int cin_low, int cup, int cout, const float* b_t, float* wfold, float* wb, hipStream_t st);
int biu_fold_gemm_chain(const float* G, size_t slice_f, const float* layouts, int cin_low, int cup, int cout, int ccat, float* dw_conv, float* dw_t,
                        const float* b_t, const float* Sk, hipStream_t st);
size_t biu_mfma_conv_split_bytes(int cin, const biu_act* y, const biu_act* y1, int kd, int dtype);
int biu_mfma_convt_dgrad_bricks(const biu_act* dx, int kd);
int biu_mfma_convt_dgrad_rows(const biu_act* dx, int kd, int cdy, int dtype);
int biu_mfma_pack_batch(const biu_pack_job* jobs_device, int n, int dtype, hipStream_t st);
int biu_mfma_set_fp32_products(int mode);
int biu_mfma_set_fp32_products_3d(int mode);
int biu_mfma_conv_ksplit(int cin, const biu_act* y, int kd, int dtype);
int biu_mfma_conv_stat_rows(const biu_act* y, int kd, const biu_act* x = nullptr, int dtype = -1, bool red = false, int cin = -1);
int biu_mfma_conv_bricks(const biu_act* y, int kd, const biu_act* x = nullptr, int dtype = -1, int cin = -1);
size_t biu_mfma_wgrad_workspace(int cin, int cout, int kd, int kh, int kw, int dtype);
bool biu_mfma_wgrad_ok(const biu_act* x, const biu_act* dy, int kd, int kh, int kw, int dilation, int dtype);
struct BnBwdFuse {
    const biu_act* y;
    const float *scale, *shift, *slope, *cA, *cB, *cC;
    const float* r1_dl = nullptr;
    const float* r1_w = nullptr;
};
bool biu_mfma_wgrad_rank1_ok(const biu_act* x, const biu_act* dy, int kd, int kh, int kw, int dilation, int dtype);
int biu_mfma_wgrad(const biu_act* x, const biu_xform* xf, const biu_act* dy, int kd, int kh, int kw, float* dw,
                   float* dbias, void* ws, size_t ws_bytes, int dtype, hipStream_t st, const BnBwdFuse* bn = nullptr,
                   const biu_act* x1 = nullptr, const biu_xform* xf1 = nullptr, int dw_ld_cols = 0, int dw_c_off = 0);

size_t biu_mfma_convt_packed_bytes(int kind, int cin, int cout, int kd, int dtype);
int biu_mfma_convt_pack(int kind, const float* w, int cin, int cout, int kd, int dtype, void* packed, hipStream_t st);
bool biu_mfma_upconv_ok(const biu_act* x, const biu_act* y, int dtype);
size_t biu_mfma_upconv_packed_bytes(int kind, int cin, int cout, int dtype);
int biu_mfma_upconv_pack(int kind, const float* w, int cin, int cout, int dtype, void* packed, hipStream_t st, const float* wf = nullptr);
int biu_mfma_upconv_dgrad_rows(const biu_act* dx);
int biu_mfma_upconv_dgrad(const biu_act* dy, const void* packed, const biu_act* dx, int accumulate, int dtype, hipStream_t st, float* bn_partial = nullptr,
                          const BnRedFuse* red = nullptr);
struct BnBwdFuse;
size_t biu_mfma_upconv_wgrad_workspace(int cin, int cout, int dtype);
int biu_mfma_upconv_wgrad(const biu_act* x, const biu_xform* xf, const biu_act* dy, float* dw, void* ws, size_t ws_bytes, int dtype,
                          hipStream_t st, const BnBwdFuse* bn);
int biu_mfma_upconv_stat_rows(const biu_act* x, const biu_act* y);
int biu_mfma_upconv_fwd(const biu_act* x, const biu_xform* xf, const void* packed, const float* bias, const biu_act* y, float* bn_partial,
                        int dtype, hipStream_t st, int accumulate = 0);
bool biu_mfma_foldt_ok(const biu_act* x_low, const biu_act* skip, const biu_act* y, int dtype);
bool biu_mfma_foldt_worth(const biu_act* x_low, const biu_act* y);
size_t biu_mfma_foldt_packed_bytes(int cin_low, int cskip, int cout, int dtype);
int biu_mfma_foldt_pack(const float* w_conv, const float* b_conv, const float* w_t, const float* b_t, int cin_low, int cup, int cskip, int cout, int dtype,
                        void* packed, hipStream_t st);
int biu_mfma_foldt_stat_rows(const biu_act* x_low, const biu_act* y, const biu_act* skip = nullptr, int dtype = -1);
int biu_mfma_foldt_form(const biu_act* x_low, const biu_act* skip, const biu_act* y, int dtype);
int biu_mfma_foldt_fwd(const biu_act* x_low, const biu_xform* xf_low, const biu_act* skip, const biu_xform* xf_skip, const void* packed, const biu_act* y,
                       float* bn_partial, int dtype, hipStream_t st);
int biu_mfma_foldt_dgrad(const biu_act* dy, const void* packed, const biu_act* dx_low, int acc_low, const biu_act* dskip, int acc_skip, int dtype,
                         hipStream_t st, float* bn_partial_low, const BnRedFuse* red_low, void* ws, size_t ws_bytes);
size_t biu_mfma_foldt_wgrad_workspace(int cin_low, int cskip, int cout, int dtype);
int biu_mfma_foldt_wgrad(const biu_act* x_low, const biu_xform* xf_low, const biu_act* skip, const biu_xform* xf_skip, const biu_act* da, const BnBwdFuse* bn,
                         const float* dy_sum, const float* w_conv, const float* w_t, const float* b_t, int cup, float* dw_conv, float* dw_t, float* db_t, void* ws, size_t ws_bytes,
                         int dtype, hipStream_t st, int phases = 7);
bool biu_mfma_convt_ok(int kind, const biu_act* lo, const biu_act* hi, int kd, int dtype);
int biu_mfma_convt_fwd(const biu_act* x, const biu_xform* xf, const void* packed, const float* bias, int kd, const biu_act* y,
                       int dtype, hipStream_t st);
int biu_mfma_convt_dgrad(const biu_act* dy, const void* packed, int kd, const biu_act* dx, int accumulate, int dtype, hipStream_t st,
                         float* bn_partial = nullptr, const BnRedFuse* red = nullptr);
bool biu_mfma_convt_wgrad_ok(const biu_act* x, const biu_act* dy, int kd, int dtype);
int biu_mfma_convt_wgrad(const biu_act* x, const biu_xform* xf, const biu_act* dy, int kd, float* dw, float* dbias, void* ws,
                         size_t ws_bytes, int dtype, hipStream_t st);

bool biu_c1_conv_ok(const biu_act* x, const biu_act* y, int kd, int kh, int kw, int dil, int dtype);
int biu_c1_conv_fwd(const biu_act* x, const biu_xform* xf, const float* w, const float* bias, int kd, const biu_act* y, int dtype, hipStream_t st);
size_t biu_c1_wgrad_workspace(int cout, int kd);
int biu_c1_conv_wgrad(const biu_act* x, const biu_xform* xf, const biu_act* dy, int kd, float* dw, void* ws, size_t ws_bytes, int dtype, hipStream_t st);
bool biu_vec_reduce_ok(const biu_act* a, int dtype);
int biu_bn_stats_vec(const biu_act* y, float* partial, int* nblk_out, int dtype, hipStream_t st);
int biu_bn_bwd_reduce_vec(const biu_act* da, const biu_act* y, const float* scale, const float* shift, const float* slope,
                          const float* mean, const float* invstd, float* partial, int* nblk_out, int dtype, hipStream_t st);
size_t biu_chan_sum_workspace(int c);
int biu_chan_sum_vec(const biu_act* a, float* out, void* ws, int dtype, hipStream_t st);
bool biu_head_bwd_fused_ok(const biu_act* x, const biu_act* dx, int cout, int dtype);
size_t biu_head_bwd_fused_workspace(int cin);
bool biu_head_bwd_bnred_ok(const biu_act* x, const biu_act* dx, int cout, int dtype);
int biu_head_bwd_bnred_fused(const biu_act* x, const biu_xform* xf, const float* w, int cout, const float* dl, const biu_act* dx, float* dw,
                             float* db, void* ws, const float* mean, const float* invstd, float* bn_partial, int* bn_nblk, int dtype,
                             hipStream_t st);
int biu_head_bwd_fused(const biu_act* x, const biu_xform* xf, const float* w, int cout, const float* dl, const biu_act* dx, float* dw,
                       float* db, void* ws, size_t ws_bytes, int dtype, hipStream_t st);
bool biu_rowvec_ok(const biu_act* a, int dtype);
int biu_bn_bwd_apply_rv(const biu_act* da, const biu_act* y, const float* scale, const float* shift, const float* slope,
                        const float* A, const float* B, const float* Cc, const biu_act* dy, int dtype, hipStream_t st);
int biu_xform_apply_rv(const biu_act* x, const biu_xform* xf, const biu_act* out, int dtype, hipStream_t st);
int biu_maxpool_fwd_rv(const biu_act* x, const biu_xform* xf, const biu_act* out, int pd, int dtype, hipStream_t st);
int biu_maxpool_bwd_rv(const biu_act* x, const biu_xform* xf, const biu_act* dout, const biu_act* dx, int pd, int accumulate, int dtype, hipStream_t st);
int biu_maxpool_bwd_bnred_rv(const biu_act* x, const biu_xform* xf, const biu_act* dout, const biu_act* dx, int pd, int accumulate,
                             const float* mean, const float* invstd, float* partial, size_t partial_floats, int* nblk, int dtype,
                             hipStream_t st);
int biu_nearest_rv(int mode, const biu_act* src, const biu_xform* xf, const biu_act* dst, int pd, int accumulate, int dtype, hipStream_t st);

bool biu_convt_all_ok(const biu_act* lo, const biu_act* hi, int kd, int dtype);
int biu_convt_all_fwd(const biu_act* x, const biu_xform* xf, const void* packed, const float* bias, int kd, const biu_act* y, hipStream_t st);
int biu_convt_all_dgrad_rows(const biu_act* dx, const biu_act* dy, int kd);
int biu_convt_all_dgrad(const biu_act* dy, const void* packed, int kd, const biu_act* dx, int accumulate, hipStream_t st,
                        float* bn_partial = nullptr, const BnRedFuse* red = nullptr);

bool biu_c1m_ok(const biu_act* x, const biu_act* y, int kd, int kh, int kw, int dil, int dtype);
int biu_c1m_fwd_rows(const biu_act* y, int kd);
int biu_c1m_fwd(const biu_act* x, const biu_xform* xf, const float* w, const float* bias, int kd, const biu_act* y, float* bn_partial, hipStream_t st);
size_t biu_c1m_wgrad_workspace(int cout, int kd);
int biu_c1m_wgrad(const biu_act* x, const biu_xform* xf, const biu_act* da, const BnBwdFuse* bn, int kd, float* dw, void* ws, size_t ws_bytes,
                  hipStream_t st);
```

bio_image_unet_amd/engine.py:

```python
from __future__ import annotations

import contextlib
import ctypes as C
import os
import weakref
from typing import Dict, List, Optional, Sequence, Tuple

import torch
from torch import nn

from . import _lib
from ._lib import BIU_BF16, BIU_F32, BN_MAX_PARTIALS, biu_act, biu_xform, check, lib
from ._lib import ptr as _ptr, stream as _stream

LRELU_SLOPE = 0.1


def _disabled(token: str, env: Optional[str] = None) -> bool:
    return token in (os.environ.get("BIU_DISABLE", "") if env is None else env).split(",")


_NO_CAPTURE_FORK = _disabled("capturefork")
_NO_SIDE_CHAIN = _disabled("sidechain")
_NO_PREPACK = _disabled("prepack")
_NO_HEAD_RANK1 = _disabled("headrank1") or _disabled("head_bnred")
_SIDE_WGRAD_VOX = int(os.environ.get("BIU_SIDE_WGRAD_VOX", str(4 * 32 ** 3)))

class Buf:

    def __init__(self, eng: "Engine", n, d, h, w, c):
        self.eng = eng
        self.shape = (n, d, h, w, c)
        self.t = torch.empty(self.shape, dtype=eng.tdtype, device=eng.device)
        self.g: Optional[torch.Tensor] = None
        self.scale = torch.ones(c, dtype=torch.float32, device=eng.device)
        self.shift = torch.zeros(c, dtype=torch.float32, device=eng.device)
        self.slope = torch.ones(c, dtype=torch.float32, device=eng.device)
        self.leaves: Dict[Tuple[int, int], bool] = {}
        self.lazy: Dict[Tuple[int, int], bool] = {}
        self.ncons: Dict[Tuple[int, int], int] = {}
        self.nwr: Dict[Tuple[int, int], int] = {}
        self.producer: Dict[Tuple[int, int], "Node"] = {}
        self.acts = []

    def slice(self, c0: int, c: int, lazy: bool) -> "Act":
        self.leaves[(c0, c)] = False
        self.lazy[(c0, c)] = lazy
        return Act(self, c0, c, [(c0, c)])

    def span(self, c0: int, c: int) -> "Act":
        keys = sorted(k for k in self.leaves if c0 <= k[0] < c0 + c)
        cov = c0
        for k0, kc in keys:
            assert k0 == cov, "span has a hole"
            cov += kc
        assert cov == c0 + c, "span does not end on a slice boundary"
        return Act(self, c0, c, keys)

    def full(self) -> "Act":
        keys = sorted(self.leaves)
        cov = 0
        for c0, c in keys:
            assert c0 == cov, "concat buffer has a hole"
            cov += c
        assert cov == self.shape[4]
        return Act(self, 0, cov, keys)

    def grad(self) -> torch.Tensor:
        assert self.t is not None, "a released buffer has no gradient either"
        if self.g is None:
            self.g = torch.empty(self.shape, dtype=self.eng.tdtype, device=self.eng.device)
        return self.g

    def release(self):
        self.t = None
        self.g = None
        for a in self.acts:
            a._a.p = None


class Act:

    def __init__(self, buf: Buf, c0: int, c: int, leaves):
        self.buf, self.c0, self.c, self.leaves = buf, c0, c, leaves
        n, d, h, w, ctot = buf.shape
        isz = buf.t.element_size()
        self.n, self.d, self.h, self.w = n, d, h, w
        self._a = biu_act(buf.t.data_ptr() + c0 * isz, n, d, h, w, c, ctot)
        self._g = None
        self._x = None
        self.is_input = False
        buf.acts.append(self)

    @property
    def nvox(self):
        return self.n * self.d * self.h * self.w

    @property
    def space(self):
        return (self.n, self.d, self.h, self.w)

    def a(self):
        return C.byref(self._a)

    def g(self):
        if self._g is None:
            gt = self.buf.grad()
            self._g = biu_act(gt.data_ptr() + self.c0 * gt.element_size(), self.n, self.d, self.h, self.w, self.c,
                              self.buf.shape[4])
        return C.byref(self._g)

    def is_lazy(self):
        return any(self.buf.lazy[k] for k in self.leaves)

    def xf(self):
        if not self.is_lazy():
            return None
        if self._x is None:
            o = 4 * self.c0
            self._x = biu_xform(self.buf.scale.data_ptr() + o, self.buf.shift.data_ptr() + o,
                                self.buf.slope.data_ptr() + o)
        return C.byref(self._x)

    def vec(self, name):
        buf = self.buf
        return getattr(buf, name)[self.c0:self.c0 + self.c]

    def g_written(self) -> bool:
        flags = [self.buf.leaves[k] for k in self.leaves]
        assert all(flags) or not any(flags), "partially written concat gradient"
        return flags[0]

    def g_accumulate(self) -> int:
        flags = [self.buf.leaves[k] for k in self.leaves]
        if all(flags) or not any(flags):
            return int(flags[0])
        g = self.buf.grad()
        for k, f in zip(self.leaves, flags):
            if not f:
                g[..., k[0]:k[0] + k[1]].zero_()
                self.buf.leaves[k] = True
        return 1

    def mark_g(self):
        for k in self.leaves:
            self.buf.leaves[k] = True
            self.buf.nwr[k] = self.buf.nwr.get(k, 0) + 1

    def completed_producer(self, k: int = 1, unwritten: bool = False):
        if len(self.leaves) != 1:
            return None
        key = self.leaves[0]
        if self.buf.ncons.get(key, 0) - self.buf.nwr.get(key, 0) != k or (unwritten and self.buf.leaves[key]):
            return None
        up = self.buf.producer.get(key)
        if up is None or not up.batch_stats or up.y.c != self.c or up.y.c0 != self.c0:
            return None
        return up

    def consumed(self):
        for k in self.leaves:
            self.buf.ncons[k] = self.buf.ncons.get(k, 0) + 1


class CatAct:

    def __init__(self, p0: Act, p1: Act):
        assert p0.space == p1.space
        self.parts = (p0, p1)
        self.c = p0.c + p1.c
        self.n, self.d, self.h, self.w = p0.n, p0.d, p0.h, p0.w
        self.is_input = False

    @property
    def nvox(self):
        return self.parts[0].nvox

    @property
    def space(self):
        return self.parts[0].space

    def consumed(self):
        for p in self.parts:
            p.consumed()


class CatBuf:

    def __init__(self, eng: "Engine", space, c_first, c_second):
        n, d, h, w = space
        self.c_first, self.c_second = c_first, c_second
        self.bufs = (eng.new_buf(n, d, h, w, c_first), eng.new_buf(n, d, h, w, c_second))
        self.acts = [None, None]

    def slice(self, c0: int, c: int, lazy: bool) -> Act:
        k = 0 if (c0, c) == (0, self.c_first) else 1
        assert (c0, c) == ((0, self.c_first) if k == 0 else (self.c_first, self.c_second)), "a planar concat has exactly two slices"
        self.acts[k] = self.bufs[k].slice(0, c, lazy)
        return self.acts[k]

    def full(self) -> CatAct:
        assert self.acts[0] is not None and self.acts[1] is not None, "both parts must be produced before the concatenation is read"
        return CatAct(self.acts[0], self.acts[1])


class Packed:

    def __init__(self, eng: "Engine", nbytes: int, params, what: str, pack, job=None):
        self.buf = torch.empty(nbytes, dtype=torch.uint8, device=eng.device) if nbytes else None
        self.params = [p for p in params if p is not None]
        self.what, self.pack, self.job = what, pack, job
        self.ver = None
        self.used = False
        eng.images.append(self)

    def version(self):
        return tuple((p.data_ptr(), p._version) for p in self.params)

    def ptr(self, ahead=None):
        if self.buf is None:
            return None
        self.used = True
        ver = self.version()
        if self.ver != ver:
            check(self.pack(_ptr(self.buf), _stream()), self.what)
            self.ver = ver
        elif ahead is not None:
            torch.cuda.current_stream().wait_event(ahead)
        return _ptr(self.buf)


class Node:
    params: Sequence[nn.Parameter] = ()
    label = "node"

    def fwd(self, eng: "Engine"):
        raise NotImplementedError

    def bwd(self, eng: "Engine"):
        raise NotImplementedError


def _ksize(w: torch.Tensor):
    if w.dim() == 5:
        return tuple(w.shape[2:])
    return (1,) + tuple(w.shape[2:])


class ConvBlockNode(Node):

    def __init__(self, eng, seq: nn.Sequential, xin: Act, yout: Act, dropout_follows: bool = False, fold_src: Optional[Act] = None,
                 convt: Optional["ConvTNode"] = None):
        conv, bn = seq[0], seq[1]
        self.conv, self.bn, self.xin, self.y = conv, bn, xin, yout
        act = seq[2] if len(seq) > 2 else None
        self.slope = float(act.negative_slope) if isinstance(act, nn.LeakyReLU) else (0.0 if isinstance(act, nn.ReLU) else 1.0)
        xin.consumed()
        if len(yout.leaves) == 1:
            yout.buf.producer[yout.leaves[0]] = self
        self.batch_stats = False
        self.red_partial: Optional[torch.Tensor] = None
        self.red_nblk = 0
        self.rank1 = None
        self.fold_ws, self.fold_ev = None, None
        self.wg_ws, self.wg_ev = None, None
        self.kd, self.kh, self.kw = _ksize(conv.weight)
        self.dil = int(conv.dilation[0])
        drop = seq[3] if len(seq) > 3 else None
        if drop is not None and getattr(drop, "p", 0.0) != 0.0 and not dropout_follows:
            raise NotImplementedError("Dropout p != 0 needs a DropoutNode behind the block (models.Unet_v0 / BabyUnet build one)")
        assert tuple(conv.weight.shape[:2]) == (yout.c, xin.c), (conv.weight.shape, yout.c, xin.c)
        assert xin.space == yout.space
        self.params = [conv.weight, conv.bias, bn.weight, bn.bias]
        w, cout, dt, dev = conv.weight, yout.c, eng.dtype, eng.device
        self.save_mean = torch.empty(cout, dtype=torch.float32, device=dev)
        self.save_invstd = torch.empty(cout, dtype=torch.float32, device=dev)
        yout.vec("slope").fill_(self.slope)
        eng.need_partial(cout)
        eng.need_partial_floats(lib.biu_conv_fwd_stats_floats(yout.a(), self.kd))
        parts = xin.parts if isinstance(xin, CatAct) else (xin,)
        k333 = (self.kd, self.kh, self.kw, self.dil) == (3, 3, 3, 1)
        self.form = "cat" if len(parts) == 2 else "plain"
        self.foldt, self.foldt_img = None, None
        self.fold_src, self.fold_slot, self.fold_dg_slot, self.fold_wg, self.fold_all = None, None, None, False, False
        if (convt is not None and len(parts) == 2 and parts[0] is convt.y and convt.kd == 2 and k333 and convt.up.bias is not None
                and lib.biu_foldt_ok(convt.xin.a(), parts[1].a(), yout.a(), dt)
                and lib.biu_foldt_bwd_weight_workspace(convt.xin.c, parts[1].c, cout, dt) > 0):
            self.form, self.foldt = "foldt", convt
            lo, skip, up = convt.xin, parts[1], convt.up
            self.foldt_img = Packed(eng, lib.biu_foldt_packed_bytes(lo.c, skip.c, cout, dt), (w, conv.bias, up.weight, up.bias), "foldt_pack",
                                    lambda dst, st: lib.biu_foldt_pack(_ptr(w.data), _ptr(conv.bias.data) if conv.bias is not None else None,
                                                                       _ptr(up.weight.data), _ptr(up.bias.data), lo.c, convt.y.c, skip.c, cout, dt, dst, st))
            eng.need_partial_floats(lib.biu_foldt_fwd_stats_floats(lo.a(), yout.a()))
            eng.need_ws(lib.biu_foldt_bwd_weight_workspace(lo.c, skip.c, cout, dt))
        elif (fold_src is not None and k333 and len(parts) == 1 and fold_src.c == xin.c and lib.biu_upconv_ok(fold_src.a(), yout.a(), dt)):
            self.form, self.fold_src = "upconv", fold_src

            def folded(kind, nbytes):
                return Packed(eng, nbytes, (w,), "upconv_pack", lambda dst, st: lib.biu_upconv_pack(kind, _ptr(w.data), xin.c, cout, dt, dst, st))
            self.fold_slot = folded(0, lib.biu_upconv_packed_bytes(0, xin.c, cout, dt))
            nb1 = lib.biu_upconv_packed_bytes(1, xin.c, cout, dt)
            if nb1:
                self.fold_dg_slot = folded(1, nb1)
            wsf = lib.biu_upconv_bwd_weight_workspace(xin.c, cout, dt)
            if wsf:
                self.fold_wg = True
                eng.need_ws(wsf)
            self.fold_all = self.fold_dg_slot is not None and self.fold_wg
            eng.need_partial_floats(lib.biu_upconv_fwd_stats_floats(fold_src.a(), yout.a()))
        geom = (xin.c, cout, self.kd, self.kh, self.kw)
        self.pk_f, self.pk_b = (Packed(eng, lib.biu_conv_packed_bytes(kind, *geom, self.dil, dt), (w,), "conv_pack",
                                       lambda dst, st, kind=kind: lib.biu_conv_pack(kind, _ptr(w.data), *geom, dt, dst, st), job=(0, kind) + geom)
                                for kind in (0, 1))
        eng.need_ws(lib.biu_conv_bwd_weight_workspace(*geom, dt))
        eng.need_ws(lib.biu_conv_split_workspace(xin.c, yout.a(), None, self.kd, self.kh, self.kw, self.dil, dt))
        eng.need_ws(lib.biu_conv_split_workspace(cout, parts[0].a(), parts[1].a() if len(parts) == 2 else None, self.kd, self.kh, self.kw, self.dil, dt))

    def fwd(self, eng):
        st, y, train = _stream(), self.y, eng.bn_training(self.bn)
        w, b = self.conv.weight.data, self.conv.bias.data if self.conv.bias is not None else None
        packed = self.pk_f.ptr()
        nblk = C.c_int(0)
        stats = (_ptr(eng.partial), eng.partial.numel(), C.byref(nblk)) if train else (None, 0, None)
        if self.form == "foldt":
            lo, skip = self.foldt.xin, self.xin.parts[1]
            blob = self.foldt_img.ptr(ahead=eng._fold_ev)
            check(lib.biu_foldt_fwd(lo.a(), lo.xf(), skip.a(), skip.xf(), blob, y.a(), *stats, eng.dtype, st), "foldt_fwd")
        elif self.form == "upconv":
            src, folded = self.fold_src, self.fold_slot.ptr()
            check(lib.biu_upconv_fwd(src.a(), src.xf(), folded, _ptr(b), y.a(), *stats, eng.dtype, st), "upconv_fwd")
        elif self.form == "cat":
            p0, p1 = self.xin.parts
            check(lib.biu_conv_fwd_cat(p0.a(), p0.xf(), p1.a(), p1.xf(), _ptr(w), packed, _ptr(b), self.kd, self.kh, self.kw, self.dil, y.a(),
                                       *stats, _ptr(eng.ws), eng.ws_bytes, eng.dtype, st), "conv_fwd_cat")
        elif train:
            check(lib.biu_conv_fwd_stats(self.xin.a(), self.xin.xf(), _ptr(w), packed, _ptr(b), self.kd, self.kh, self.kw, self.dil, y.a(),
                                         *stats, _ptr(eng.ws), eng.ws_bytes, eng.dtype, st), "conv_fwd_stats")
        else:
            check(lib.biu_conv_fwd(self.xin.a(), self.xin.xf(), _ptr(w), packed, _ptr(b), self.kd, self.kh, self.kw, self.dil, y.a(),
                                   _ptr(eng.ws), eng.ws_bytes, eng.dtype, st), "conv_fwd")
        self._fwd_bn(eng, train, nblk.value, st)

    def _fwd_bn(self, eng, train: bool, nblk: int, st):
        bn, y = self.bn, self.y
        scale, shift = y.vec("scale"), y.vec("shift")
        if train:
            mom = bn.momentum if bn.momentum is not None else 0.1
            track = bn.track_running_stats and bn.running_mean is not None
            check(lib.biu_bn_finalize(_ptr(eng.partial), nblk, y.c, float(y.nvox), _ptr(bn.weight.data),
                                      _ptr(bn.bias.data), _ptr(bn.running_mean) if track else None,
                                      _ptr(bn.running_var) if track else None, mom, bn.eps, _ptr(scale), _ptr(shift),
                                      _ptr(self.save_mean), _ptr(self.save_invstd), st), "bn_finalize")
            if track and bn.num_batches_tracked is not None:
                eng.nbt_bump.append(bn.num_batches_tracked)
        else:
            check(lib.biu_bn_eval_affine(y.c, _ptr(bn.weight.data), _ptr(bn.bias.data), _ptr(bn.running_mean),
                                         _ptr(bn.running_var), bn.eps, _ptr(scale), _ptr(shift), st), "bn_eval_affine")
            if eng.grad_mode:
                self.save_mean.copy_(bn.running_mean)
                torch.rsqrt(bn.running_var.float() + bn.eps, out=self.save_invstd)
        self.batch_stats = train

    def wgrad_route(self, eng, rank1: bool):
        if self.form == "foldt":
            return "foldt", eng.chain_stream()
        if self.form == "cat":
            return "cat", None
        if self.fold_wg:
            return "upconv", None
        if self.kd == 3 and eng.tdtype == torch.bfloat16 and self.y.nvox <= _SIDE_WGRAD_VOX:
            side = eng.chain_stream()
            if side is not None:
                return "side", side
        return ("rank1" if rank1 else "fused"), None

    def rank1_ok(self, eng, head_cout: int) -> bool:
        if eng.trace or _NO_HEAD_RANK1 or eng.tdtype != torch.bfloat16 or not self.batch_stats:
            return False
        if self.wgrad_route(eng, True)[0] != "rank1":
            return False
        return bool(lib.biu_conv_bwd_weight_bn_rank1_ok(self.xin.a(), self.y.g(), self.y.a(), head_cout, self.kd, self.kh, self.kw, self.dil,
                                                        eng.dtype))

    def bwd(self, eng):
        rank1, self.rank1 = self.rank1, None
        if not self.y.g_written():
            return
        st = _stream()
        y, cout, xin, w = self.y, self.y.c, self.xin, self.conv.weight
        k4 = (self.kd, self.kh, self.kw, self.dil)
        scale, shift, slope = _ptr(y.vec("scale")), _ptr(y.vec("shift")), _ptr(y.vec("slope"))
        nblk = C.c_int(0)
        if self.red_nblk:
            partial, nblk.value, self.red_nblk = self.red_partial, self.red_nblk, 0
        else:
            partial = eng.partial
            check(lib.biu_bn_bwd_reduce(y.g(), y.a(), scale, shift, slope, _ptr(self.save_mean), _ptr(self.save_invstd),
                                        _ptr(partial), C.byref(nblk), eng.dtype, st), "bn_bwd_reduce")
        dgamma, dbeta = eng.new_grad(self.bn.weight), eng.new_grad(self.bn.bias)
        A, B, Cc = eng.coef[0][:cout], eng.coef[1][:cout], eng.coef[2][:cout]
        dw = eng.new_grad(w)
        dy_sum = None
        if self.batch_stats:
            check(lib.biu_bn_bwd_finalize(_ptr(partial), nblk.value, cout, float(y.nvox), scale, _ptr(self.save_mean),
                                          _ptr(self.save_invstd), _ptr(dgamma), _ptr(dbeta), _ptr(A), _ptr(B), _ptr(Cc), st),
                  "bn_bwd_finalize")
            db = eng.zero_like_bias(self.conv.bias) if self.conv.bias is not None else None
        else:
            dy_sum = torch.empty(cout, dtype=torch.float32, device=eng.device)
            check(lib.biu_bn_bwd_finalize_eval(_ptr(partial), nblk.value, cout, scale, _ptr(dgamma), _ptr(dbeta), _ptr(dy_sum), _ptr(A), _ptr(B),
                                               _ptr(Cc), st), "bn_bwd_finalize_eval")
            db = dy_sum if self.conv.bias is not None else None
        bn_args = (y.g(), y.a(), scale, shift, slope, _ptr(A), _ptr(B), _ptr(Cc))
        ws = (_ptr(eng.ws), eng.ws_bytes, eng.dtype, st)
        route, side = self.wgrad_route(eng, rank1 is not None)
        if route == "foldt":
            ct, skip = self.foldt, xin.parts[1]
            lo, up = ct.xin, ct.up
            dwt, dbt = eng.new_grad(up.weight), eng.new_grad(up.bias)
            args = (lo.a(), lo.xf(), skip.a(), skip.xf(), *bn_args, _ptr(dy_sum), _ptr(w.data), _ptr(up.weight.data), _ptr(up.bias.data), ct.y.c,
                    _ptr(dw), _ptr(dwt), _ptr(dbt))
            if side is None:
                check(lib.biu_foldt_bwd_weight_bn(*args, *ws), "foldt_bwd_weight_bn")
                eng.add_grad(up.weight, dwt)
                eng.add_grad(up.bias, dbt)
            else:
                if self.fold_ws is None:
                    self.fold_ws = torch.empty(lib.biu_foldt_bwd_weight_workspace(lo.c, skip.c, cout, eng.dtype), dtype=torch.uint8, device=eng.device)
                    self.fold_ev = (torch.cuda.Event(), torch.cuda.Event())
                args += (_ptr(self.fold_ws), self.fold_ws.numel(), eng.dtype)
                check(lib.biu_foldt_bwd_weight_bn_phase(*args, 1 | 4, st), "foldt_bwd_weight_bn_phase(1 | 4)")
                with eng.fork(side, self.fold_ev, "/chain", [(up.weight, dwt), (up.bias, dbt), (w, dw)], keep=(A, B, Cc, dy_sum)):
                    check(lib.biu_foldt_bwd_weight_bn_phase(*args, 2, _stream()), "foldt_bwd_weight_bn_phase(2)")
        elif route == "cat":
            p0, p1 = xin.parts
            check(lib.biu_conv_bwd_weight_cat(p0.a(), p0.xf(), p1.a(), p1.xf(), *bn_args, *k4, _ptr(dw), *ws), "conv_bwd_weight_cat")
        elif route == "upconv":
            check(lib.biu_upconv_bwd_weight_bn(self.fold_src.a(), self.fold_src.xf(), *bn_args, _ptr(dw), *ws), "upconv_bwd_weight_bn")
        elif route == "side":
            check(lib.biu_bn_bwd_apply(*bn_args, y.g(), eng.dtype, st), "bn_bwd_apply")
            if self.wg_ws is None:
                self.wg_ws = torch.empty(max(lib.biu_conv_bwd_weight_workspace(xin.c, cout, self.kd, self.kh, self.kw, eng.dtype), 16), dtype=torch.uint8,
                                         device=eng.device)
                self.wg_ev = (torch.cuda.Event(), torch.cuda.Event())
            with eng.fork(side, self.wg_ev, "/wgrad", [(w, dw)]):
                check(lib.biu_conv_bwd_weight(xin.a(), xin.xf(), y.g(), *k4, _ptr(dw), None, _ptr(self.wg_ws), self.wg_ws.numel(), eng.dtype, _stream()),
                      "conv_bwd_weight")
        elif route == "rank1":
            check(lib.biu_conv_bwd_weight_bn_rank1(xin.a(), xin.xf(), _ptr(rank1[0]), _ptr(rank1[1]), 1, *bn_args, *k4, _ptr(dw), *ws),
                  "conv_bwd_weight_bn_rank1")
        else:
            check(lib.biu_conv_bwd_weight_bn(xin.a(), xin.xf(), *bn_args, *k4, _ptr(dw), *ws), "conv_bwd_weight_bn")
        if side is None:
            eng.add_grad(w, dw)
        if db is not None:
            eng.add_grad(self.conv.bias, db)
        eng.add_grad(self.bn.weight, dgamma)
        eng.add_grad(self.bn.bias, dbeta)
        if self.form == "foldt":
            lo, skip = self.foldt.xin, xin.parts[1]
            if not eng.wants_grad(lo):
                raise NotImplementedError("foldt: the coarse input of a decoder level always wants its gradient")
            blob = self.foldt_img.ptr()
            up = lo.completed_producer(unwritten=True)
            if up is not None:
                up.red_from(eng, lib.biu_foldt_bwd_data_bnred_floats(lo.a()), "foldt_bwd_data", lambda *red: lib.biu_foldt_bwd_data(
                    y.g(), blob, lo.g(), 0, skip.g(), int(skip.g_written()), lo.a(), *up.red_coeffs(), *red, *ws))
            else:
                check(lib.biu_foldt_bwd_data(y.g(), blob, lo.g(), int(lo.g_written()), skip.g(), int(skip.g_written()), None, None, None, None, None, None,
                                             None, 0, None, *ws), "foldt_bwd_data")
            lo.mark_g()
            skip.mark_g()
        elif self.form == "cat":
            p0, p1 = xin.parts
            check(lib.biu_conv_bwd_data_cat(y.g(), _ptr(w.data), self.pk_b.ptr(), *k4, p0.g(), p0.g_accumulate(), p1.g(), p1.g_accumulate(), *ws),
                  "conv_bwd_data_cat")
            p0.mark_g()
            p1.mark_g()
        elif self.fold_dg_slot is not None and eng.wants_grad(self.fold_src):
            src = self.fold_src
            check(lib.biu_upconv_bwd_data(y.g(), self.fold_dg_slot.ptr(), src.g(), int(src.g_written()), eng.dtype, st), "upconv_bwd_data")
            src.mark_g()
        elif eng.wants_grad(xin):
            packed = self.pk_b.ptr()
            up = xin.completed_producer(unwritten=True)
            if up is not None:
                up.red_from(eng, lib.biu_bwd_data_bnred_floats(xin.a(), self.kd, 0), "conv_bwd_data_bnred", lambda *red: lib.biu_conv_bwd_data_bnred(
                    y.g(), _ptr(w.data), packed, *k4, xin.g(), xin.a(), *up.red_coeffs(), *red, *ws))
            else:
                check(lib.biu_conv_bwd_data(y.g(), _ptr(w.data), packed, *k4, xin.g(), int(xin.g_written()), *ws), "conv_bwd_data")
            xin.mark_g()

    def red_from(self, eng, need: int, what: str, call):
        if self.red_partial is None or self.red_partial.numel() < need:
            self.red_partial = torch.empty(need, dtype=torch.float32, device=eng.device)
        n = C.c_int(0)
        check(call(_ptr(self.red_partial), self.red_partial.numel(), C.byref(n)), what)
        self.red_nblk = n.value

    def red_coeffs(self):
        y = self.y
        return (_ptr(y.vec("scale")), _ptr(y.vec("shift")), _ptr(y.vec("slope")), _ptr(self.save_mean),
                _ptr(self.save_invstd))


class ConvTNode(Node):

    def __init__(self, eng, up: nn.Module, xin: Act, yout: Act):
        self.up, self.xin, self.y = up, xin, yout
        xin.consumed()
        w = up.weight
        self.kd = 2 if w.dim() == 5 else 1
        assert tuple(w.shape[:2]) == (xin.c, yout.c)
        self.params = [up.weight, up.bias]
        self.folded_into = None
        geom, dt = (xin.c, yout.c, self.kd), eng.dtype
        self.pk_f, self.pk_b = (Packed(eng, lib.biu_convt_packed_bytes(kind, *geom, dt), (w,), "convt_pack",
                                       lambda dst, st, kind=kind: lib.biu_convt_pack(kind, _ptr(w.data), *geom, dt, dst, st), job=(1, kind) + geom + (2, 2))
                                for kind in (0, 1))
        eng.need_ws(lib.biu_convt_bwd_weight_workspace(*geom, dt))

    def fwd(self, eng):
        if self.folded_into is not None:
            return
        check(lib.biu_convt_fwd(self.xin.a(), self.xin.xf(), _ptr(self.up.weight.data), self.pk_f.ptr(), _ptr(self.up.bias.data),
                                self.kd, self.y.a(), eng.dtype, _stream()), "convt_fwd")

    def bwd(self, eng):
        if self.folded_into is not None or not self.y.g_written():
            return
        st = _stream()
        dw, db = eng.new_grad(self.up.weight), eng.new_grad(self.up.bias)
        check(lib.biu_convt_bwd_weight(self.xin.a(), self.xin.xf(), self.y.g(), self.kd, _ptr(dw), _ptr(db), _ptr(eng.ws),
                                       eng.ws_bytes, eng.dtype, st), "convt_bwd_weight")
        eng.add_grad(self.up.weight, dw)
        eng.add_grad(self.up.bias, db)
        if eng.wants_grad(self.xin):
            packed = self.pk_b.ptr()
            up = self.xin.completed_producer(unwritten=True)
            if up is not None:
                up.red_from(eng, lib.biu_bwd_data_bnred_floats(self.xin.a(), self.kd, 1), "convt_bwd_data_bnred", lambda *red: lib.biu_convt_bwd_data_bnred(
                    self.y.g(), _ptr(self.up.weight.data), packed, self.kd, self.xin.g(), self.xin.a(), *up.red_coeffs(), *red, eng.dtype, st))
            else:
                check(lib.biu_convt_bwd_data(self.y.g(), _ptr(self.up.weight.data), packed, self.kd, self.xin.g(),
                                             int(self.xin.g_written()), eng.dtype, st), "convt_bwd_data")
            self.xin.mark_g()


class ResampleNode(Node):

    def __init__(self, eng, kind: str, xin: Act, yout: Act):
        assert kind in ("maxpool", "down", "up", "trilinear", "bilinear")
        self.kind, self.xin, self.y = kind, xin, yout
        self.only_for_backward = False
        self.skip = False
        xin.consumed()

    def fwd(self, eng):
        if self.skip or (self.only_for_backward and not eng.grad_mode):
            return
        f = {"maxpool": lib.biu_maxpool_fwd, "down": lib.biu_nearest_down_fwd, "up": lib.biu_nearest_up_fwd,
             "trilinear": lib.biu_trilinear_up_fwd, "bilinear": lib.biu_bilinear_up_fwd}[self.kind]
        check(f(self.xin.a(), self.xin.xf(), self.y.a(), eng.dtype, _stream()), self.kind + "_fwd")

    def bwd(self, eng):
        if not self.y.g_written() or not eng.wants_grad(self.xin):
            return
        acc, st = int(self.xin.g_written()), _stream()
        if self.kind == "maxpool":
            up = self.xin.completed_producer() if self.xin.xf() is not None else None
            if up is not None:
                up.red_from(eng, lib.biu_bwd_data_bnred_floats(self.xin.a(), up.kd, 0), "maxpool_bwd_bnred", lambda *red: lib.biu_maxpool_bwd_bnred(
                    self.xin.a(), self.xin.xf(), self.y.g(), self.xin.g(), acc, _ptr(up.save_mean), _ptr(up.save_invstd), *red, eng.dtype, st))
            else:
                check(lib.biu_maxpool_bwd(self.xin.a(), self.xin.xf(), self.y.g(), self.xin.g(), acc, eng.dtype, st), "maxpool_bwd")
        elif self.kind == "down":
            check(lib.biu_nearest_down_bwd(self.y.g(), self.xin.g(), acc, eng.dtype, st), "nearest_down_bwd")
        elif self.kind == "trilinear":
            check(lib.biu_trilinear_up_bwd(self.y.g(), self.xin.g(), acc, eng.dtype, st), "trilinear_up_bwd")
        elif self.kind == "bilinear":
            check(lib.biu_bilinear_up_bwd(self.y.g(), self.xin.g(), acc, eng.dtype, st), "bilinear_up_bwd")
        else:
            check(lib.biu_nearest_up_bwd(self.y.g(), self.xin.g(), acc, eng.dtype, st), "nearest_up_bwd")
        self.xin.mark_g()


class MaxJoinNode(Node):

    def __init__(self, eng, a: Act, b: Act, out: Act):
        self.a_, self.b_, self.y = a, b, out
        a.consumed()
        b.consumed()

    def fwd(self, eng):
        check(lib.biu_max_join_fwd(self.a_.a(), self.a_.xf(), self.b_.a(), self.b_.xf(), self.y.a(), eng.dtype, _stream()),
              "max_join_fwd")

    def bwd(self, eng):
        if not self.y.g_written():
            return
        assert self.a_.g_written() == self.b_.g_written()
        check(lib.biu_max_join_bwd(self.a_.a(), self.a_.xf(), self.b_.a(), self.b_.xf(), self.y.g(), self.a_.g(),
                                   self.b_.g(), int(self.a_.g_written()), eng.dtype, _stream()), "max_join_bwd")
        self.a_.mark_g()
        self.b_.mark_g()


class XCorrNode(Node):

    def __init__(self, eng, a: Act, b: Act, out: Act):
        self.a_, self.b_, self.y = a, b, out
        a.consumed()
        b.consumed()

    def fwd(self, eng):
        check(lib.biu_xcorr_fwd(self.a_.a(), self.a_.xf(), self.b_.a(), self.b_.xf(), self.y.a(), eng.dtype, _stream()), "xcorr_fwd")

    def bwd(self, eng):
        if not self.y.g_written():
            return
        assert self.a_.g_written() == self.b_.g_written()
        check(lib.biu_xcorr_bwd(self.a_.a(), self.a_.xf(), self.b_.a(), self.b_.xf(), self.y.g(), self.a_.g(), self.b_.g(),
                                int(self.a_.g_written()), eng.dtype, _stream()), "xcorr_bwd")
        self.a_.mark_g()
        self.b_.mark_g()


class CopyNode(Node):

    def __init__(self, eng, xin: Act, out: Act):
        self.xin, self.y = xin, out
        xin.consumed()

    def fwd(self, eng):
        check(lib.biu_xform_apply(self.xin.a(), self.xin.xf(), self.y.a(), eng.dtype, _stream()), "xform_apply")

    def bwd(self, eng):
        if not self.y.g_written() or not eng.wants_grad(self.xin):
            return
        check(lib.biu_act_add(self.y.g(), self.xin.g(), self.xin.g_accumulate(), eng.dtype, _stream()), "act_add")
        self.xin.mark_g()


class DropoutNode(Node):

    def __init__(self, eng, drop: nn.Module, xin: Act, out: Act):
        self.drop, self.xin, self.y = drop, xin, out
        xin.consumed()
        self.mask_override: Optional[torch.Tensor] = None
        self.factor: Optional[torch.Tensor] = None
        self._keep = []

    def _sample(self, act: Act, tensor: torch.Tensor, n: int) -> biu_act:
        per = act.d * act.h * act.w * act.buf.shape[4] * tensor.element_size()
        return biu_act(tensor.data_ptr() + act.c0 * tensor.element_size() + n * per, 1, act.d, act.h, act.w, act.c, act.buf.shape[4])

    def fwd(self, eng):
        x, st = self.xin, _stream()
        p = float(self.drop.p)
        if self.drop.training and p > 0.0:
            if self.mask_override is not None:
                keep = self.mask_override.to(device=eng.device, dtype=torch.float32)
            else:
                keep = torch.bernoulli(torch.full((x.n, x.c), 1.0 - p, device=eng.device))
            self.factor = keep / (1.0 - p)
        else:
            self.factor = torch.ones((x.n, x.c), device=eng.device)
        sc = (x.vec("scale")[None, :] * self.factor).contiguous()
        sh = (x.vec("shift")[None, :] * self.factor).contiguous()
        sl = x.vec("slope").contiguous()
        self._keep = [sc, sh, sl]
        for n in range(x.n):
            xf = biu_xform(sc[n].data_ptr(), sh[n].data_ptr(), sl.data_ptr())
            a_in, a_out = self._sample(x, x.buf.t, n), self._sample(self.y, self.y.buf.t, n)
            check(lib.biu_xform_apply(C.byref(a_in), C.byref(xf), C.byref(a_out), eng.dtype, st), "dropout_fwd")

    def bwd(self, eng):
        if not self.y.g_written() or not eng.wants_grad(self.xin):
            return
        assert not self.xin.g_written(), "DropoutNode is the only reader of its input"
        st = _stream()
        f = self.factor.contiguous()
        zero, one = torch.zeros_like(f[0]), torch.ones_like(f[0])
        self._keep += [f, zero, one]
        for n in range(self.xin.n):
            xf = biu_xform(f[n].data_ptr(), zero.data_ptr(), one.data_ptr())
            g_out, g_in = self._sample(self.y, self.y.buf.grad(), n), self._sample(self.xin, self.xin.buf.grad(), n)
            check(lib.biu_xform_apply(C.byref(g_out), C.byref(xf), C.byref(g_in), eng.dtype, st), "dropout_bwd")
        self.xin.mark_g()


class AddReluNode(Node):

    def __init__(self, eng, a: Act, b: Act, out: Act):
        self.a_, self.b_, self.y = a, b, out
        a.consumed()
        b.consumed()

    def fwd(self, eng):
        check(lib.biu_add_relu_fwd(self.a_.a(), self.a_.xf(), self.b_.a(), self.b_.xf(), self.y.a(), eng.dtype, _stream()), "add_relu_fwd")

    def bwd(self, eng):
        if not self.y.g_written():
            return
        assert self.a_.g_written() == self.b_.g_written()
        check(lib.biu_add_relu_bwd(self.y.a(), self.y.g(), self.a_.g(), self.b_.g(), int(self.a_.g_written()), eng.dtype, _stream()),
              "add_relu_bwd")
        self.a_.mark_g()
        self.b_.mark_g()


class GateNode(Node):

    def __init__(self, eng, e: Act, psi: Act, out: Act):
        assert psi.c == 1 and e.c == out.c
        self.e_, self.psi_, self.y = e, psi, out
        e.consumed()
        psi.consumed()

    def fwd(self, eng):
        check(lib.biu_gate_fwd(self.e_.a(), self.e_.xf(), self.psi_.a(), self.psi_.xf(), self.y.a(), eng.dtype, _stream()), "gate_fwd")

    def bwd(self, eng):
        if not self.y.g_written():
            return
        assert not self.psi_.g_written()
        check(lib.biu_gate_bwd(self.e_.a(), self.e_.xf(), self.psi_.a(), self.psi_.xf(), self.y.g(), self.e_.g(),
                               int(self.e_.g_written()), self.psi_.g(), eng.dtype, _stream()), "gate_bwd")
        self.e_.mark_g()
        self.psi_.mark_g()


_ACT_CODE = {None: 0, "none": 0, "sigmoid": 1, "tanh": 2, "relu": 3}


class HeadNode(Node):

    def __init__(self, eng, conv: nn.Module, xin: Act, activation, want_logits: bool, want_act: bool):
        self.conv, self.xin = conv, xin
        xin.consumed()
        self.cout = conv.weight.shape[0]
        assert conv.weight.shape[1] == xin.c
        if activation not in _ACT_CODE:
            activation = None
        self.activation = activation
        self.act = _ACT_CODE[activation]
        self.want_logits, self.want_act = want_logits, want_act
        self.params = [conv.weight, conv.bias]
        eng.need_ws(lib.biu_head_bwd_workspace(xin.c))
        self.logits = self.activated = None
        self._keep = ()

    def out_shape(self, eng):
        x = self.xin
        return (x.n, self.cout, x.d, x.h, x.w) if eng.nd == 3 else (x.n, self.cout, x.h, x.w)

    def fwd(self, eng):
        shp = self.out_shape(eng)
        self.logits = torch.empty(shp, dtype=torch.float32, device=eng.device) if self.want_logits else None
        self.activated = torch.empty(shp, dtype=torch.float32, device=eng.device) if self.want_act else None
        w = self.conv.weight.data.reshape(self.cout, self.xin.c)
        check(lib.biu_head_fwd(self.xin.a(), self.xin.xf(), _ptr(w), _ptr(self.conv.bias.data), self.cout, self.act,
                               _ptr(self.logits), _ptr(self.activated), eng.dtype, _stream()), "head_fwd")

    def dlogits(self, eng, g_logits, g_act, a, dst=None, ctot=None, c0=0):
        if g_act is None and dst is None and g_logits.dtype == torch.float32 and g_logits.is_contiguous():
            return g_logits
        shp = self.out_shape(eng)
        n, spatial = shp[0], 1
        for v in shp[2:]:
            spatial *= v
        if dst is None:
            dst, ctot, c0 = torch.empty(shp, dtype=torch.float32, device=eng.device), self.cout, 0
        f32 = lambda t: None if t is None else t.contiguous().float()
        gl, ga = f32(g_logits), f32(g_act)
        self._keep = (gl, ga, a)
        check(lib.biu_head_dlogits(_ptr(gl), _ptr(ga), _ptr(a) if ga is not None else None, self.act, n, self.cout, spatial,
                                   _ptr(dst), ctot, c0, _stream()), "head_dlogits")
        return dst

    def bwd_with(self, eng, dl: Optional[torch.Tensor], logits_only: bool = False):
        if dl is None:
            return
        dl = dl.contiguous().float()
        st = _stream()
        dw, db = eng.new_grad(self.conv.weight), eng.new_grad(self.conv.bias)
        want_dx = eng.wants_grad(self.xin)
        assert not self.xin.g_written(), "heads that share a trunk go through Engine._backward_heads"
        up = self.xin.completed_producer() if (want_dx and self.xin.xf() is not None) else None
        if up is not None:
            need = lib.biu_bwd_data_bnred_floats(self.xin.a(), up.kd, 0)
            rank1 = logits_only and self.cout == 1 and up.rank1_ok(eng, self.cout)
            if rank1:
                up.rank1 = (dl, self.conv.weight.data)
            up.red_from(eng, need, "head_bwd_bnred", lambda *red: lib.biu_head_bwd_bnred(
                self.xin.a(), self.xin.xf(), _ptr(self.conv.weight.data), self.cout, _ptr(dl), None if rank1 else self.xin.g(), _ptr(dw), _ptr(db),
                _ptr(eng.ws), eng.ws_bytes, _ptr(up.save_mean), _ptr(up.save_invstd), *red, eng.dtype, st))
        else:
            check(lib.biu_head_bwd(self.xin.a(), self.xin.xf(), _ptr(self.conv.weight.data), self.cout, _ptr(dl),
                                   self.xin.g() if want_dx else None, _ptr(dw), _ptr(db), _ptr(eng.ws), eng.ws_bytes,
                                   eng.dtype, st), "head_bwd")
        eng.add_grad(self.conv.weight, dw)
        eng.add_grad(self.conv.bias, db)
        if want_dx:
            self.xin.mark_g()


class Engine:

    def __init__(self, device, tdtype, nd: int):
        if torch.device(device).type != "cuda":
            raise RuntimeError("bio_image_unet_amd executes only through its HIP kernels on an MI355X; "
                               f"got device '{device}'. There is no CPU fallback.")
        self.device, self.tdtype, self.nd = torch.device(device), tdtype, nd
        self.dtype = {torch.float32: BIU_F32, torch.bfloat16: BIU_BF16}[tdtype]
        self.nodes: List[Node] = []
        self.heads: List[HeadNode] = []
        self.bufs: List[Buf] = []
        self.inputs: List[Act] = []
        self._partial_c, self._partial_floats = 0, 0
        self.ws_bytes = 0
        self.partial = self.ws = None
        self.coef = None
        self.params: List[nn.Parameter] = []
        self._pcount: Dict[nn.Parameter, int] = {}
        self._pseen: Dict[nn.Parameter, int] = {}
        self.grads: Dict[nn.Parameter, torch.Tensor] = {}
        self.nbt_bump: List[torch.Tensor] = []
        self.grad_mode = False
        self.input_requires_grad = False
        self._zero_flat, self._zero_used = None, 0
        self._stack_w: Dict[tuple, torch.Tensor] = {}
        self.images: List[Packed] = []
        self._job_key, self._job_tab = None, None
        self.grad_hook = None
        self.grad_alloc = None
        self.trace = None
        self.generation = 0
        self._live = None
        self._side = None
        self._deferred = []
        self._fold_ev = None

    def busy(self) -> bool:
        return self._live is not None and self._live() is not None

    def invalidate_packed(self):
        for im in self.images:
            im.ver = None

    def new_buf(self, n, d, h, w, c) -> Buf:
        b = Buf(self, n, d, h, w, c)
        self.bufs.append(b)
        return b

    def new_cat(self, space, c_first, c_second, consumer_cout, kd):
        n, d, h, w = space
        probe = lambda c: biu_act(256, n, d, h, w, c, c)
        a0, a1, ay = probe(c_first), probe(c_second), probe(consumer_cout)
        if lib.biu_conv_cat_ok(C.byref(a0), C.byref(a1), C.byref(ay), kd, 3, 3, 1, self.dtype) == 1:
            return CatBuf(self, space, c_first, c_second)
        return self.new_buf(n, d, h, w, c_first + c_second)

    def new_act(self, space, c, lazy: bool) -> Act:
        n, d, h, w = space
        return self.new_buf(n, d, h, w, c).slice(0, c, lazy)

    def add(self, node: Node):
        self.nodes.append(node)
        return node

    def need_partial(self, c):
        self._partial_c = max(self._partial_c, c)

    def need_partial_floats(self, n):
        self._partial_floats = max(self._partial_floats, int(n))

    def need_ws(self, nbytes):
        self.ws_bytes = max(self.ws_bytes, int(nbytes))

    def finalize(self):
        dev = self.device
        c = max(self._partial_c, 1)
        self.partial = torch.empty(max(BN_MAX_PARTIALS * c * 2, self._partial_floats), dtype=torch.float32, device=dev)
        self.coef = torch.empty((3, c), dtype=torch.float32, device=dev)
        self.ws = torch.empty(max(self.ws_bytes, 16), dtype=torch.uint8, device=dev)
        seen = set()
        for nd_ in self.nodes:
            for p in nd_.params:
                if p is not None:
                    self._pcount[p] = self._pcount.get(p, 0) + 1
                    if id(p) not in seen:
                        seen.add(id(p))
                        self.params.append(p)

    def pack_all(self):
        stale = [s for s in self.images if s.job is not None and s.used and s.ver != s.version()]
        if len(stale) < 2:
            return
        key = tuple((id(s), s.params[0].data_ptr()) for s in stale)
        if self._job_key != key:
            from ._lib import biu_pack_job
            arr = (biu_pack_job * len(stale))()
            for j, s in zip(arr, stale):
                tr, kind, cin, cout, kd, kh, kw = s.job
                j.w, j.packed = s.params[0].data_ptr(), s.buf.data_ptr()
                j.transposed, j.kind, j.cin, j.cout, j.kd, j.kh, j.kw, j.reserved = tr, kind, cin, cout, kd, kh, kw, 0
            raw = torch.frombuffer(bytearray(bytes(arr)), dtype=torch.uint8)
            self._job_tab = raw.to(self.device)
            self._job_key = key
        check(lib.biu_pack_batch(_ptr(self._job_tab), len(stale), self.dtype, _stream()), "pack_batch")
        for s in stale:
            s.ver = s.version()

    def bn_training(self, bn: nn.Module) -> bool:
        return bn.training or bn.running_mean is None

    def wants_grad(self, act: Act) -> bool:
        return self.input_requires_grad if act.is_input else True

    def new_input(self, space, c) -> Act:
        a = self.new_act(space, c, lazy=False)
        a.is_input = True
        self.inputs.append(a)
        return a

    def new_grad(self, p: nn.Parameter) -> torch.Tensor:
        if self.grad_alloc is not None and self._pcount.get(p, 1) == 1:
            v = self.grad_alloc(p)
            if v is not None:
                return v
        return torch.empty(p.shape, dtype=torch.float32, device=self.device)

    def zero_like_bias(self, b: torch.Tensor) -> torch.Tensor:
        n = b.numel()
        if self._zero_flat is None or self._zero_used + n > self._zero_flat.numel() or self._zero_flat.dtype != b.dtype:
            self._zero_flat = torch.zeros(max(4096, 4 * n), dtype=b.dtype, device=b.device)
            self._zero_used = 0
        v = self._zero_flat[self._zero_used:self._zero_used + n].view_as(b)
        self._zero_used += n
        return v

    def add_grad(self, p: nn.Parameter, g: torch.Tensor):
        if p in self.grads:
            self.grads[p] = self.grads[p] + g
        else:
            self.grads[p] = g
        if self.grad_hook is not None:
            self._pseen[p] = self._pseen.get(p, 0) + 1
            if self._pseen[p] == self._pcount.get(p, 1):
                self.grad_hook(p, self.grads[p])

    def load_inputs(self, xs: Sequence[torch.Tensor]):
        st = _stream()
        for act, x in zip(self.inputs, xs):
            x = x.detach()
            if x.dtype == torch.uint8:
                x = x.contiguous()
                check(lib.biu_from_nchw_u8(_ptr(x), 255.0, act.a(), self.dtype, st), "from_nchw_u8")
                continue
            if x.dtype != torch.float32:
                x = x.float()
            x = x.contiguous()
            check(lib.biu_from_nchw(_ptr(x), act.a(), self.dtype, st), "from_nchw")

    def _prepack_folds(self):
        self._fold_ev = None
        if _NO_PREPACK or (torch.cuda.is_current_stream_capturing() and _NO_CAPTURE_FORK):
            return
        stale = [n for n in self.nodes if isinstance(n, ConvBlockNode) and n.form == "foldt" and n.foldt_img.ver != n.foldt_img.version()]
        if not stale:
            return
        cur = torch.cuda.current_stream()
        if self._side is None:
            self._side = torch.cuda.Stream(device=self.device)
        self._side.wait_stream(cur)
        with torch.cuda.stream(self._side):
            for n in stale:
                lib.label = n.label + ":pack"
                n.foldt_img.ptr()
            self._fold_ev = torch.cuda.Event()
            self._fold_ev.record(self._side)

    def forward(self):
        self.generation += 1
        self.nbt_bump = []
        lib.label = "pack:fwd"
        self.pack_all()
        self._prepack_folds()
        for nd_ in self.nodes:
            lib.label = nd_.label + ":fwd"
            if self.trace:
                self.trace("fwd", nd_, "pre")
            nd_.fwd(self)
            if self.trace:
                self.trace("fwd", nd_, "post")
        if self.nbt_bump:
            counts: Dict[int, list] = {}
            for t in self.nbt_bump:
                counts.setdefault(id(t), [t, 0])[1] += 1
            by_k: Dict[int, list] = {}
            for t, k in counts.values():
                by_k.setdefault(k, []).append(t)
            for k, ts in by_k.items():
                torch._foreach_add_(ts, k)

    def chain_stream(self):
        if self.trace or _NO_SIDE_CHAIN or (torch.cuda.is_current_stream_capturing() and _NO_CAPTURE_FORK):
            return None
        if self._side is None:
            self._side = torch.cuda.Stream(device=self.device)
        return self._side

    @contextlib.contextmanager
    def fork(self, side, events, suffix: str, grads, keep=()):
        ready, done = events
        ready.record(torch.cuda.current_stream())
        side.wait_event(ready)
        label = lib.label
        with torch.cuda.stream(side):
            lib.label = label + suffix
            yield
            done.record(side)
        lib.label = label
        self._deferred.append((done, grads, keep))

    def _flush_deferred(self, keep_last: int):
        while len(self._deferred) > keep_last:
            done, grads, _ = self._deferred.pop(0)
            torch.cuda.current_stream().wait_event(done)
            for p, g in grads:
                self.add_grad(p, g)

    def backward(self, head_grads: Sequence[Optional[torch.Tensor]]):
        self.grads = {}
        self._deferred = []
        self._pseen = {}
        self._zero_flat, self._zero_used = None, 0
        for b in self.bufs:
            for k in b.leaves:
                b.leaves[k] = False
                b.nwr[k] = 0
        lib.label = "head:bwd"
        if self.trace:
            self.trace("bwd", ("heads", head_grads), "pre")
        self._backward_heads(head_grads)
        if self.trace:
            self.trace("bwd", ("heads", head_grads), "post")
        for nd_ in reversed(self.nodes):
            if isinstance(nd_, HeadNode):
                continue
            lib.label = nd_.label + ":bwd"
            if self.trace:
                self.trace("bwd", nd_, "pre")
            self._flush_deferred(2)
            nd_.bwd(self)
            if self.trace:
                self.trace("bwd", nd_, "post")
        self._flush_deferred(0)
        return self.grads

    def _backward_heads(self, head_grads):
        live = [(h, g) for h, g in zip(self.heads, head_grads) if g is not None]
        if not live:
            return
        groups: Dict[int, list] = {}
        for h, g in live:
            groups.setdefault(id(h.xin), []).append((h, g))
        for grp in groups.values():
            self._backward_head_group(grp)

    def _backward_head_group(self, live):
        if len(live) == 1:
            h, (gl, ga, a) = live[0]
            h.bwd_with(self, h.dlogits(self, gl, ga, a), logits_only=ga is None)
            return
        x = live[0][0].xin
        assert all(h.xin is x for h, _ in live)
        cout = sum(h.cout for h, _ in live)
        shp = live[0][0].out_shape(self)
        dl = torch.empty((shp[0], cout) + tuple(shp[2:]), dtype=torch.float32, device=self.device)
        key = tuple(id(h) for h, _ in live)
        if key not in self._stack_w:
            self._stack_w[key] = torch.empty((cout, x.c), dtype=torch.float32, device=self.device)
        w, o = self._stack_w[key], 0
        for h, (gl, ga, a) in live:
            w[o:o + h.cout].copy_(h.conv.weight.data.reshape(h.cout, x.c))
            h.dlogits(self, gl, ga, a, dst=dl, ctot=cout, c0=o)
            o += h.cout
        dw = torch.empty_like(w)
        db = torch.empty(cout, dtype=torch.float32, device=self.device)
        up = x.completed_producer(len(live), unwritten=True) if (self.wants_grad(x) and x.xf() is not None) else None
        if up is not None:
            up.red_from(self, lib.biu_bwd_data_bnred_floats(x.a(), up.kd, 0), "head_bwd_bnred(stacked)", lambda *red: lib.biu_head_bwd_bnred(
                x.a(), x.xf(), _ptr(w), cout, _ptr(dl), x.g(), _ptr(dw), _ptr(db), _ptr(self.ws), self.ws_bytes, _ptr(up.save_mean),
                _ptr(up.save_invstd), *red, self.dtype, _stream()))
        else:
            check(lib.biu_head_bwd(x.a(), x.xf(), _ptr(w), cout, _ptr(dl), x.g(), _ptr(dw), _ptr(db), _ptr(self.ws),
                                   self.ws_bytes, self.dtype, _stream()), "head_bwd(stacked)")
        x.mark_g()
        o = 0
        for h, _ in live:
            self.add_grad(h.conv.weight, dw[o:o + h.cout].reshape(h.conv.weight.shape).clone())
            self.add_grad(h.conv.bias, db[o:o + h.cout].clone())
            o += h.cout

    def input_grads(self) -> List[Optional[torch.Tensor]]:
        outs = []
        st = _stream()
        for act in self.inputs:
            if not self.input_requires_grad or not act.g_written():
                outs.append(None)
                continue
            shp = (act.n, act.c, act.d, act.h, act.w) if self.nd == 3 else (act.n, act.c, act.h, act.w)
            t = torch.empty(shp, dtype=torch.float32, device=self.device)
            ga = biu_act(act.buf.grad().data_ptr(), act.n, act.d, act.h, act.w, act.c, act.buf.shape[4])
            check(lib.biu_to_nchw(C.byref(ga), None, _ptr(t), self.dtype, st), "to_nchw")
            outs.append(t)
        return outs


class _Token:
    __slots__ = ("__weakref__",)


class _NetFn(torch.autograd.Function):

    @staticmethod
    def forward(ctx, eng: Engine, n_inputs: int, out_spec, *tensors):
        xs, ctx.n_inputs = tensors[:n_inputs], n_inputs
        if eng.busy():
            raise RuntimeError("engine re-entered while an earlier forward still awaits its backward (models take a second "
                               "engine for that case: this is a bug in the caller of engine.run)")
        eng.load_inputs(xs)
        eng.forward()
        ctx.eng, ctx.out_spec = eng, out_spec
        ctx.generation = eng.generation
        if eng.grad_mode:
            ctx.token = _Token()
            eng._live = weakref.ref(ctx.token)
        else:
            eng._live = None
        outs = []
        for hi, kind in out_spec:
            h = eng.heads[hi]
            outs.append(h.logits if kind == "logits" else h.activated)
        ctx.act_slot = {hi: i for i, (hi, kind) in enumerate(out_spec) if kind == "act"}
        ctx.save_for_backward(*[outs[i] for i in ctx.act_slot.values()])
        ctx.set_materialize_grads(False)
        for h in eng.heads:
            h.logits = h.activated = None
        return tuple(outs)

    @staticmethod
    def backward(ctx, *gouts):
        eng: Engine = ctx.eng
        if ctx.generation != eng.generation:
            raise RuntimeError("backward of a forward whose activations were overwritten: the engine ran another forward of the "
                               "same input shape in between (generation %d, now %d)" % (ctx.generation, eng.generation))
        per_head: Dict[int, List[Optional[torch.Tensor]]] = {}
        for (hi, kind), g in zip(ctx.out_spec, gouts):
            slot = per_head.setdefault(hi, [None, None])
            slot[0 if kind == "logits" else 1] = g
        saved = dict(zip(ctx.act_slot.keys(), ctx.saved_tensors))
        head_grads = []
        for hi, h in enumerate(eng.heads):
            gl, ga = per_head.get(hi, [None, None])
            head_grads.append((gl, ga, saved.get(hi)) if (gl is not None or ga is not None) else None)
        grads = eng.backward(head_grads)
        dxs = eng.input_grads()
        pg = [grads.pop(p, None) for p in eng.params]
        eng.grads = {}
        del grads
        ctx.token = None
        eng._live = None
        eng.generation += 1
        return (None, None, None, *dxs, *pg)


def run(eng: Engine, xs: Sequence[torch.Tensor], out_spec):
    eng.grad_mode = torch.is_grad_enabled()
    eng.input_requires_grad = eng.grad_mode and any(x.requires_grad for x in xs)
    return _NetFn.apply(eng, len(xs), tuple(out_spec), *xs, *eng.params)
```

include/biu.h:

```cpp
#ifndef BIU_H
#define BIU_H

#include <stddef.h>
#include <stdint.h>

#ifdef __cplusplus
extern "C" {
#endif

typedef void* biu_stream;

enum { BIU_F32 = 0, BIU_BF16 = 1 };

typedef enum {
    BIU_OK = 0,
    BIU_ERR_SHAPE = -1,
    BIU_ERR_UNSUPPORTED = -2,
    BIU_ERR_ALIGN = -3,
    BIU_ERR_WORKSPACE = -4,
    BIU_ERR_LAUNCH = -5
} biu_status;

typedef struct {
    void*   p;
    int32_t n, d, h, w;
    int32_t c;
    int32_t pitch;
} biu_act;

typedef struct {
    const float* scale;
    const float* shift;
    const float* slope;
} biu_xform;

const char* biu_last_error(void);
int  biu_version(void);

int  biu_set_fp32_products(int mode);

int  biu_set_fp32_products_3d(int mode);


size_t biu_conv_packed_bytes(int kind, int cin, int cout, int kd, int kh, int kw, int dilation, int dtype);
int    biu_conv_pack(int kind, const float* w, int cin, int cout, int kd, int kh, int kw, int dtype,
                     void* packed, biu_stream stream);

typedef struct biu_pack_job {
    const void* w;
    void* packed;
    int32_t transposed, kind, cin, cout, kd, kh, kw, reserved;
} biu_pack_job;
int biu_pack_batch(const biu_pack_job* jobs, int n, int dtype, biu_stream stream);

size_t biu_conv_split_workspace(int cin, const biu_act* y, const biu_act* y1, int kd, int kh, int kw, int dilation, int dtype);

int biu_conv_fwd(const biu_act* x, const biu_xform* xf, const float* w, const void* packed,
                 const float* bias, int kd, int kh, int kw, int dilation,
                 const biu_act* y, void* ws, size_t ws_bytes, int dtype, biu_stream stream);

size_t biu_conv_fwd_stats_floats(const biu_act* y, int kd);
int biu_conv_fwd_stats(const biu_act* x, const biu_xform* xf, const float* w, const void* packed,
                       const float* bias, int kd, int kh, int kw, int dilation, const biu_act* y,
                       float* bn_partial, size_t bn_partial_floats, int* bn_nblk, void* ws, size_t ws_bytes, int dtype,
                       biu_stream stream);

int biu_conv_bwd_data(const biu_act* dy, const float* w, const void* packed,
                      int kd, int kh, int kw, int dilation,
                      const biu_act* dx, int accumulate, void* ws, size_t ws_bytes, int dtype, biu_stream stream);

size_t biu_bwd_data_bnred_floats(const biu_act* dx, int kd, int transposed);
int biu_conv_bwd_data_bnred(const biu_act* dy, const float* w, const void* packed, int kd, int kh, int kw, int dilation,
                            const biu_act* dx, const biu_act* y_up, const float* scale, const float* shift,
                            const float* slope, const float* mean, const float* invstd, float* partial,
                            size_t partial_floats, int* nblk, void* ws, size_t ws_bytes, int dtype, biu_stream stream);
int biu_convt_bwd_data_bnred(const biu_act* dy, const float* w, const void* packed, int kd, const biu_act* dx,
                             const biu_act* y_up, const float* scale, const float* shift, const float* slope,
                             const float* mean, const float* invstd, float* partial, size_t partial_floats, int* nblk,
                             int dtype, biu_stream stream);

size_t biu_conv_bwd_weight_workspace(int cin, int cout, int kd, int kh, int kw, int dtype);
int biu_conv_bwd_weight(const biu_act* x, const biu_xform* xf, const biu_act* dy,
                        int kd, int kh, int kw, int dilation,
                        float* dw, float* dbias, void* ws, size_t ws_bytes, int dtype, biu_stream stream);

int biu_conv_bwd_weight_bn(const biu_act* x, const biu_xform* xf, const biu_act* da, const biu_act* y,
                           const float* scale, const float* shift, const float* slope, const float* coefA,
                           const float* coefB, const float* coefC, int kd, int kh, int kw, int dilation,
                           float* dw, void* ws, size_t ws_bytes, int dtype, biu_stream stream);
int biu_conv_bwd_weight_bn_rank1_ok(const biu_act* x, const biu_act* dy, const biu_act* y, int head_cout, int kd, int kh, int kw,
                                    int dilation, int dtype);
int biu_conv_bwd_weight_bn_rank1(const biu_act* x, const biu_xform* xf, const float* dlogits, const float* w_head, int head_cout,
                                 const biu_act* dy, const biu_act* y, const float* scale, const float* shift, const float* slope,
                                 const float* coefA, const float* coefB, const float* coefC, int kd, int kh, int kw, int dilation,
                                 float* dw, void* ws, size_t ws_bytes, int dtype, biu_stream stream);

#define BIU_BN_MAX_PARTIALS 1024
int biu_bn_stats(const biu_act* y, float* partial, int* nblk_out, int dtype, biu_stream stream);

int biu_bn_finalize(const float* partial, int nblk, int c, double count,
                    const float* gamma, const float* beta, float* running_mean, float* running_var,
                    float momentum, float eps, float* scale, float* shift,
                    float* save_mean, float* save_invstd, biu_stream stream);

int biu_bn_eval_affine(int c, const float* gamma, const float* beta, const float* running_mean,
                       const float* running_var, float eps, float* scale, float* shift, biu_stream stream);

int biu_xform_apply(const biu_act* x, const biu_xform* xf, const biu_act* out, int dtype, biu_stream stream);

int biu_bn_bwd_reduce(const biu_act* da, const biu_act* y, const float* scale, const float* shift,
                      const float* slope, const float* save_mean, const float* save_invstd,
                      float* partial, int* nblk_out, int dtype, biu_stream stream);
int biu_bn_bwd_finalize(const float* partial, int nblk, int c, double count,
                        const float* scale, const float* save_mean, const float* save_invstd,
                        float* dgamma, float* dbeta, float* coefA, float* coefB, float* coefC,
                        biu_stream stream);
int biu_bn_bwd_finalize_eval(const float* partial, int nblk, int c, const float* scale,
                             float* dgamma, float* dbeta, float* dbias, float* coefA, float* coefB, float* coefC,
                             biu_stream stream);
int biu_bn_bwd_apply(const biu_act* da, const biu_act* y, const float* scale, const float* shift,
                     const float* slope, const float* coefA, const float* coefB, const float* coefC,
                     const biu_act* dy, int dtype, biu_stream stream);

int biu_maxpool_fwd(const biu_act* x, const biu_xform* xf, const biu_act* out, int dtype, biu_stream stream);
int biu_maxpool_bwd(const biu_act* x, const biu_xform* xf, const biu_act* dout, const biu_act* dx,
                    int accumulate, int dtype, biu_stream stream);
int biu_maxpool_bwd_bnred(const biu_act* x, const biu_xform* xf, const biu_act* dout, const biu_act* dx, int accumulate,
                          const float* mean, const float* invstd, float* partial, size_t partial_floats, int* nblk,
                          int dtype, biu_stream stream);
int biu_nearest_down_fwd(const biu_act* x, const biu_xform* xf, const biu_act* out, int dtype, biu_stream stream);
int biu_nearest_down_bwd(const biu_act* dout, const biu_act* dx, int accumulate, int dtype, biu_stream stream);
int biu_nearest_up_fwd(const biu_act* x, const biu_xform* xf, const biu_act* out, int dtype, biu_stream stream);
int biu_nearest_up_bwd(const biu_act* dout, const biu_act* dx, int accumulate, int dtype, biu_stream stream);

int    biu_upconv_ok(const biu_act* x, const biu_act* y, int dtype);
size_t biu_upconv_packed_bytes(int kind, int cin, int cout, int dtype);
int    biu_upconv_pack(int kind, const float* w, int cin, int cout, int dtype, void* packed, biu_stream stream);
int    biu_upconv_bwd_data(const biu_act* dy, const void* packed, const biu_act* dx, int accumulate, int dtype, biu_stream stream);
size_t biu_upconv_bwd_weight_workspace(int cin, int cout, int dtype);
int    biu_upconv_bwd_weight_bn(const biu_act* x, const biu_xform* xf, const biu_act* da, const biu_act* y, const float* scale,
                                const float* shift, const float* slope, const float* coefA, const float* coefB, const float* coefC,
                                float* dw, void* ws, size_t ws_bytes, int dtype, biu_stream stream);
size_t biu_upconv_fwd_stats_floats(const biu_act* x, const biu_act* y);
int    biu_upconv_fwd(const biu_act* x, const biu_xform* xf, const void* packed, const float* bias, const biu_act* y,
                      float* bn_partial, size_t bn_partial_floats, int* bn_nblk, int dtype, biu_stream stream);

int biu_bce_dice_blocks(long long per_sample);
int biu_bce_dice_fwd(const float* logits, const float* target, int n, long long per_sample, float* partial, biu_stream stream);
int biu_bce_dice_bwd(const float* logits, const float* target, int n, long long per_sample, const float* coef, float* dlogits,
                     int accumulate, biu_stream stream);

int biu_pair_smooth_l1_blocks(long long pairs);
int biu_pair_smooth_l1_fwd(const float* logits, int n, long long per_sample, float* partial, biu_stream stream);
int biu_pair_smooth_l1_bwd(const float* logits, int n, long long per_sample, const float* coef, float* dlogits, int accumulate,
                           biu_stream stream);
int biu_seg_loss_finish(const float* partial, int n, int nb, long long per_sample, const float* time_partial, int nbt,
                        float a_bce, float a_dice, float smooth, int has_tversky, float tv_alpha, float tv_beta, float tv_smooth,
                        int logcosh, float w_time, float* saved, biu_stream stream);
int biu_seg_loss_coef(const float* g, const float* saved, int n, long long per_sample, float a_bce, float a_dice, float smooth,
                      int has_tversky, float tv_alpha, float tv_beta, float tv_smooth, int logcosh, float w_time, float* coef,
                      float* time_coef, biu_stream stream);
int biu_head_dlogits(const float* g_logits, const float* g_act, const float* activated, int act, int n, int ch, long long spatial,
                     float* dst, int dst_channels, int dst_c0, biu_stream stream);

#define BIU_MO2D_MAX_LEVELS 4
#define BIU_MO2D_MAX_TERMS 32
#define BIU_MO2D_SLOTS 8
typedef struct biu_mo2d_term {
    int kind, nb;
    long long partial_off;
    long long numel, pixels;
    float p0, p1, p2, weight;
} biu_mo2d_term;
int biu_mo2d_loss_blocks(long long numel);
int biu_mo2d_loss_fwd(int kind, float ea, float eb, const float* const* pred, int nlev, const float* target, int n, int c, int h, int w,
                      float* partial, biu_stream stream);
int biu_mo2d_loss_finish(const biu_mo2d_term* terms, int nterms, const float* workspace, float* saved, biu_stream stream);
int biu_mo2d_loss_coef(const biu_mo2d_term* terms, int nterms, const float* g, const float* saved, float* coef, biu_stream stream);
int biu_mo2d_loss_bwd(int kind, float ea, float eb, const float* const* pred, int nlev, const float* target, int n, int c, int h, int w,
                      const float* coef, float* const* dpred, biu_stream stream);

#define BIU_MO3D_MAX_TERMS 16
#define BIU_MO3D_SLOTS 8
#define BIU_MO3D_SAVED_HEADER 32
typedef struct biu_mo3d_term {
    int kind, rows;
    long long partial_off;
    long long n, per_sample;
    long long pairs;
    float p0, p1, p2, weight;
} biu_mo3d_term;
int biu_mo3d_loss_blocks(long long numel);
int biu_mo3d_loss_fwd(int kind, int pre_act, const float* x, const float* target, int n, int c, int d, int h, int w, float* partial,
                      biu_stream stream);
int biu_mo3d_loss_finish(const biu_mo3d_term* terms, int nterms, const float* workspace, float* saved, biu_stream stream);
int biu_mo3d_loss_coef(const biu_mo3d_term* terms, int nterms, const float* g, const float* saved, float* coef, biu_stream stream);
int biu_mo3d_loss_bwd(int kind, const float* x, const float* target, int n, int c, int d, int h, int w, const float* coef, float* dx,
                      biu_stream stream);

int biu_trilinear_up_fwd(const biu_act* x, const biu_xform* xf, const biu_act* out, int dtype, biu_stream stream);
int biu_trilinear_up_bwd(const biu_act* dout, const biu_act* dx, int accumulate, int dtype, biu_stream stream);

int biu_bilinear_up_fwd(const biu_act* x, const biu_xform* xf, const biu_act* out, int dtype, biu_stream stream);
int biu_bilinear_up_bwd(const biu_act* dout, const biu_act* dx, int accumulate, int dtype, biu_stream stream);

int biu_xcorr_fwd(const biu_act* cur, const biu_xform* xc, const biu_act* prev, const biu_xform* xp, const biu_act* out,
                  int dtype, biu_stream stream);
int biu_xcorr_bwd(const biu_act* cur, const biu_xform* xc, const biu_act* prev, const biu_xform* xp, const biu_act* dout,
                  const biu_act* dcur, const biu_act* dprev, int accumulate, int dtype, biu_stream stream);

int biu_conv_cat_ok(const biu_act* x0, const biu_act* x1, const biu_act* y, int kd, int kh, int kw, int dilation, int dtype);
int biu_conv_fwd_cat(const biu_act* x0, const biu_xform* xf0, const biu_act* x1, const biu_xform* xf1, const float* w,
                     const void* packed, const float* bias, int kd, int kh, int kw, int dilation, const biu_act* y,
                     float* bn_partial, size_t bn_partial_floats, int* bn_nblk, void* ws, size_t ws_bytes, int dtype,
                     biu_stream stream);
int biu_conv_bwd_data_cat(const biu_act* dy, const float* w, const void* packed, int kd, int kh, int kw, int dilation,
                          const biu_act* dx0, int accumulate0, const biu_act* dx1, int accumulate1, void* ws, size_t ws_bytes,
                          int dtype, biu_stream stream);
int biu_conv_bwd_weight_cat(const biu_act* x0, const biu_xform* xf0, const biu_act* x1, const biu_xform* xf1,
                            const biu_act* da, const biu_act* y, const float* scale, const float* shift, const float* slope,
                            const float* coefA, const float* coefB, const float* coefC, int kd, int kh, int kw, int dilation,
                            float* dw, void* ws, size_t ws_bytes, int dtype, biu_stream stream);

size_t biu_convt_packed_bytes(int kind, int cin, int cout, int kd, int dtype);
int    biu_convt_pack(int kind, const float* w, int cin, int cout, int kd, int dtype, void* packed, biu_stream stream);
int biu_convt_fwd(const biu_act* x, const biu_xform* xf, const float* w, const void* packed, const float* bias,
                  int kd, const biu_act* y, int dtype, biu_stream stream);
int biu_convt_bwd_data(const biu_act* dy, const float* w, const void* packed, int kd, const biu_act* dx,
                       int accumulate, int dtype, biu_stream stream);
size_t biu_convt_bwd_weight_workspace(int cin, int cout, int kd, int dtype);
int biu_convt_bwd_weight(const biu_act* x, const biu_xform* xf, const biu_act* dy, int kd, float* dw, float* dbias,
                         void* ws, size_t ws_bytes, int dtype, biu_stream stream);

int    biu_foldt_ok(const biu_act* x_low, const biu_act* skip, const biu_act* y, int dtype);
size_t biu_foldt_packed_bytes(int cin_low, int cskip, int cout, int dtype);
int    biu_foldt_pack(const float* w_conv, const float* b_conv, const float* w_t, const float* b_t, int cin_low, int cup, int cskip, int cout,
                      int dtype, void* packed, biu_stream stream);
size_t biu_foldt_fwd_stats_floats(const biu_act* x_low, const biu_act* y);
int    biu_foldt_fwd_form(const biu_act* x_low, const biu_act* skip, const biu_act* y, int dtype);
int    biu_foldt_fwd(const biu_act* x_low, const biu_xform* xf_low, const biu_act* skip, const biu_xform* xf_skip, const void* packed,
                     const biu_act* y, float* bn_partial, size_t bn_partial_floats, int* bn_nblk, int dtype, biu_stream stream);
size_t biu_foldt_bwd_data_bnred_floats(const biu_act* dx_low);
int    biu_foldt_bwd_data(const biu_act* dy, const void* packed, const biu_act* dx_low, int acc_low, const biu_act* dskip, int acc_skip,
                          const biu_act* y_low, const float* scale, const float* shift, const float* slope, const float* mean,
                          const float* invstd, float* partial, size_t partial_floats, int* nblk, void* ws, size_t ws_bytes, int dtype,
                          biu_stream stream);
size_t biu_foldt_bwd_weight_workspace(int cin_low, int cskip, int cout, int dtype);
int    biu_foldt_bwd_weight_bn(const biu_act* x_low, const biu_xform* xf_low, const biu_act* skip, const biu_xform* xf_skip, const biu_act* da,
                               const biu_act* y, const float* scale, const float* shift, const float* slope, const float* coefA,
                               const float* coefB, const float* coefC, const float* dy_sum, const float* w_conv, const float* w_t, const float* b_t,
                               int cup, float* dw_conv, float* dw_t, float* db_t, void* ws, size_t ws_bytes, int dtype, biu_stream stream);
int    biu_foldt_bwd_weight_bn_phase(const biu_act* x_low, const biu_xform* xf_low, const biu_act* skip, const biu_xform* xf_skip, const biu_act* da,
                                     const biu_act* y, const float* scale, const float* shift, const float* slope, const float* coefA,
                                     const float* coefB, const float* coefC, const float* dy_sum, const float* w_conv, const float* w_t,
                                     const float* b_t, int cup, float* dw_conv, float* dw_t, float* db_t, void* ws, size_t ws_bytes, int dtype,
                                     int phases, biu_stream stream);

int biu_head_fwd(const biu_act* x, const biu_xform* xf, const float* w, const float* bias, int cout,
                 int act, float* logits, float* activated, int dtype, biu_stream stream);
size_t biu_head_bwd_workspace(int cin);
int biu_head_bwd(const biu_act* x, const biu_xform* xf, const float* w, int cout, const float* dlogits,
                 const biu_act* dx, float* dw, float* dbias, void* ws, size_t ws_bytes, int dtype,
                 biu_stream stream);
int biu_head_bwd_bnred(const biu_act* x, const biu_xform* xf, const float* w, int cout, const float* dlogits, const biu_act* dx,
                       float* dw, float* dbias, void* ws, size_t ws_bytes, const float* mean, const float* invstd,
                       float* partial, size_t partial_floats, int* nblk, int dtype, biu_stream stream);

int biu_max_join_fwd(const biu_act* a, const biu_xform* xa, const biu_act* b, const biu_xform* xb,
                     const biu_act* out, int dtype, biu_stream stream);
int biu_max_join_bwd(const biu_act* a, const biu_xform* xa, const biu_act* b, const biu_xform* xb,
                     const biu_act* dout, const biu_act* da, const biu_act* db, int accumulate,
                     int dtype, biu_stream stream);
int biu_act_add(const biu_act* src, const biu_act* dst, int accumulate, int dtype, biu_stream stream);
int biu_from_nchw(const float* src, const biu_act* dst, int dtype, biu_stream stream);
int biu_to_nchw(const biu_act* src, const biu_xform* xf, float* dst, int dtype, biu_stream stream);

int biu_add_relu_fwd(const biu_act* a, const biu_xform* xa, const biu_act* b, const biu_xform* xb, const biu_act* out, int dtype,
                     biu_stream stream);
int biu_add_relu_bwd(const biu_act* out, const biu_act* dout, const biu_act* da, const biu_act* db, int accumulate, int dtype,
                     biu_stream stream);
int biu_gate_fwd(const biu_act* e, const biu_xform* xe, const biu_act* psi, const biu_xform* xpsi, const biu_act* out, int dtype,
                 biu_stream stream);
int biu_gate_bwd(const biu_act* e, const biu_xform* xe, const biu_act* psi, const biu_xform* xpsi, const biu_act* dout,
                 const biu_act* de, int accumulate_e, const biu_act* dpsi, int dtype, biu_stream stream);

int biu_from_nchw_u8(const uint8_t* src, float divisor, const biu_act* dst, int dtype, biu_stream stream);
int biu_u8_to_f32(const uint8_t* src, float divisor, float* dst, long long n, biu_stream stream);
int biu_quantize_u8(const float* src, float scale, uint8_t* dst, long long n, biu_stream stream);
int biu_stitch_add(const void* patch, int patch_is_u8, const float* weight, int channels, int pd, int ph, int pw, float* acc, float* wsum,
                   int D, int H, int W, int z0, int y0, int x0, int set, biu_stream stream);
int biu_stitch_finish(const float* acc, const float* wsum, int layers, int channels, long long spatial, void* out, int out_is_u8,
                      biu_stream stream);

enum { BIU_ELEM_U8 = 0, BIU_ELEM_U16 = 1, BIU_ELEM_I16 = 2, BIU_ELEM_F32 = 3 };
enum { BIU_PREP_MINMAX = 0, BIU_PREP_MINMAX_EPS = 1, BIU_PREP_LOHI_EPS = 2 };
size_t biu_order_stats_workspace(long long segments, int nranks);
int biu_order_stats(const void* x, int elem, long long segments, long long n, long long stride, const long long* ranks, int nranks,
                    double* out, long long* nan_count, void* workspace, size_t workspace_bytes, biu_stream stream);
int biu_prep_finalize(const double* stats, int units, long long n, double q_lo, double q_hi, int family, double* scalars,
                      biu_stream stream);
int biu_prep_tiles(const void* src, int elem, int planes, int depth, int height, int width, const int* origins, int ntiles, int td, int th,
                   int tw, const double* scalars, int units, int pad_zero, int out_f32, int invert, void* out, biu_stream stream);

enum { BIU_MORPH_ERODE = 0, BIU_MORPH_DILATE = 1 };
enum { BIU_FOOT_DISK = 0, BIU_FOOT_SQUARE = 1 };
int biu_lut_u8(const uint8_t* src, const uint8_t* lut, uint8_t* dst, long long n, biu_stream stream);
int biu_morph_u8(const uint8_t* src, uint8_t* dst, int planes, int height, int width, int op, int footprint, int size, biu_stream stream);
int biu_thin_step_u8(const uint8_t* src, uint8_t* dst, int planes, int height, int width, int sub, const uint8_t* table,
                     unsigned long long* cleared, biu_stream stream);
int biu_tile_gather_u8(const uint8_t* src, int planes, int depth, int height, int width, const int* origins, int ntiles, int td, int th,
                       int tw, int invert, uint8_t* out, biu_stream stream);

#define BIU_AUG_GATE 1u
#define BIU_AUG_SSR 2u
#define BIU_AUG_BC 4u
#define BIU_AUG_BLUR 8u
#define BIU_AUG_MULT 16u
#define BIU_AUG_GAUSS 32u
#define BIU_AUG_ORDER_UNET 0
#define BIU_AUG_ORDER_SIAM 1
#define BIU_AUG_STAGE_MULT 1u
#define BIU_AUG_STAGE_GAUSS 2u
#define BIU_AUG_MAX_BLUR 15
typedef struct biu_aug_params {
    uint32_t flags, rot_k, blur_k, index;
    double m[6];
    float alpha, beta, noise_a, noise_b;
    float angle, scale, dx, dy;
} biu_aug_params;
int biu_augment_u8(const uint8_t* src, uint8_t* dst, int n, int planes, int h, int w, int is_mask, const biu_aug_params* params,
                   int stage_order, int max_blur_k, unsigned long long seed, unsigned epoch, unsigned field_id, biu_stream stream);
int biu_philox_u32(uint32_t* out, long long blocks, unsigned long long seed, unsigned c0, unsigned c1, unsigned c2, unsigned c3,
                   biu_stream stream);

#define BIU_AUGF_IMAGE 0
#define BIU_AUGF_MASK 1
#define BIU_AUGF_VECTOR 2
#define BIU_AUGF_ROT 1u
#define BIU_AUGF_SCALE 2u
#define BIU_AUGF_BLUR 4u
#define BIU_AUGF_SHOT 8u
#define BIU_AUGF_GAUSS 16u
#define BIU_AUGF_BC 32u
#define BIU_AUGF_STAGE_SHOT 3u
#define BIU_AUGF_STAGE_GAUSS 4u
#define BIU_AUGF_POISSON_CAP 128
typedef struct biu_augf_params {
    uint32_t flags, rot_k, blur_k, index;
    double m[6];
    float cos_t, sin_t, alpha, beta, shot_s, gauss_sigma;
    float angle, scale, dx, dy;
} biu_augf_params;
int biu_augment_f32(const void* src, int src_is_u8, float* dst, int n, int planes, int h, int w, int kind, const biu_augf_params* params,
                    int max_blur_k, unsigned long long seed, unsigned epoch, unsigned field_id, biu_stream stream);

#define BIU_SPLINE_R 16
int biu_spline_prefilter_f32(const void* src, int src_is_u8, float* coef, float* range, int n, int planes, int h, int w,
                             const biu_augf_params* params, biu_stream stream);
int biu_augment_f32_cubic(const void* src, int src_is_u8, const float* coef, const float* range, float* dst, int n, int planes, int h, int w,
                          const biu_augf_params* params, biu_stream stream);

typedef struct biu_augf_source {
    uint64_t offset;
    int32_t h, w;
} biu_augf_source;
int biu_augment_f32_crop(const void* arena, int arena_is_u8, unsigned long long arena_elems, float* dst, int n, int planes, int th, int tw,
                         int kind, const biu_augf_params* params, const biu_augf_source* sources, float nan_to_val, int max_blur_k,
                         unsigned long long seed, unsigned epoch, unsigned field_id, biu_stream stream);

#define BIU_AUGV_REFLECT 0
#define BIU_AUGV_CONSTANT 1
int biu_augment_vol_f32(const void* src, int src_is_u8, float* dst, int n, int channels, int depth, int h, int w,
                        int kind, int border, const biu_augf_params* params, int max_blur_k,
                        unsigned long long seed, unsigned epoch, unsigned field_id, biu_stream stream);
int biu_augment_vol_chunk(int n, int channels, int depth, int h, int w, int kind, int max_blur_k, int dst_aligned16);

typedef struct biu_augv_source {
    uint64_t offset;
    int32_t d, h, w;
    int32_t z0;
} biu_augv_source;
int biu_augment_vol_f32_crop(const void* arena, int arena_is_u8, unsigned long long arena_elems, float* dst,
                             int n, int channels, int td, int th, int tw, int kind, int border,
                             const biu_augf_params* params, const biu_augv_source* sources, float nan_to_val,
                             int max_blur_k, unsigned long long seed, unsigned epoch, unsigned field_id, biu_stream stream);

int biu_adam_step(int n, float* const* params, const float* const* grads, float* const* exp_avg,
                  float* const* exp_avg_sq, const int64_t* numel, float lr, float beta1, float beta2,
                  float eps, int step, float grad_scale, biu_stream stream);

int biu_adam_set_hyper(float* hyper, float lr, float beta1, float beta2, float eps, int step, float grad_scale, biu_stream stream);
int biu_adam_step_hyper(int n, float* const* params, const float* const* grads, float* const* exp_avg,
                        float* const* exp_avg_sq, const int64_t* numel, const float* hyper, biu_stream stream);

size_t biu_grad_clip_scratch_floats(int n);
int biu_grad_clip(int n, float* const* grads, const int64_t* numel, float max_norm, float* scratch, size_t scratch_floats, float* total_norm,
                  biu_stream stream);

#ifdef __cplusplus
}
#endif
#endif
```

Baseline: 779.7 million voxels/s.

## Batch weight-gradient finalize/unfold into one flush kernel over a persistent zeroed arena

New measurement: 775.3 million voxels/s. About the same (-0.6%).

```diff
diff --git a/bio_image_unet_amd/_lib.py b/bio_image_unet_amd/_lib.py
--- a/bio_image_unet_amd/_lib.py
+++ b/bio_image_unet_amd/_lib.py
@@ -154,6 +154,12 @@
     "biu_foldt_bwd_weight_workspace": (_Z, [_I, _I, _I, _I]),
     "biu_foldt_bwd_weight_bn": (_I, [_A, _X, _A, _X, _A, _A, _P, _P, _P, _P, _P, _P, _P, _P, _P, _P, _I, _P, _P, _P, _P, _Z, _I, _P]),
     "biu_foldt_bwd_weight_bn_phase": (_I, [_A, _X, _A, _X, _A, _A, _P, _P, _P, _P, _P, _P, _P, _P, _P, _P, _I, _P, _P, _P, _P, _Z, _I, _I, _P]),
+    "biu_wbatch_acc_bytes": (_Z, [_I, _I, _I]),
+    "biu_wbatch_table_jobs": (_I, []),
+    "biu_wbatch_begin": (_I, [_P, _Z, C.POINTER(C.c_int), _P]),
+    "biu_wbatch_flush": (_I, [_P]),
+    "biu_wbatch_end": (_I, [_P]),
+    "biu_wbatch_abort": (_I, [_P]),
     "biu_convt_fwd": (_I, [_A, _X, _P, _P, _P, _I, _A, _I, _P]),
     "biu_convt_bwd_data": (_I, [_A, _P, _P, _I, _A, _I, _I, _P]),
     "biu_convt_bwd_weight_workspace": (_Z, [_I, _I, _I, _I]),
diff --git a/bio_image_unet_amd/csrc/biu_api.hip b/bio_image_unet_amd/csrc/biu_api.hip
--- a/bio_image_unet_amd/csrc/biu_api.hip
+++ b/bio_image_unet_amd/csrc/biu_api.hip
@@ -8,7 +8,7 @@
     "conv_fwd", "conv_dgrad", "conv_wgrad", "convt_fwd", "convt_dgrad", "convt_wgrad", "convt_all", "c1", "c1_mfma", "cat",
     "fused_stats", "wgrad_bn", "dgrad_bnred", "pool_pair", "pool_pipe", "pool_bnred", "head_bnred", "ksplit", "m16", "m16x2", "rr16",
     "wroll", "wroll16", "wroll2d", "upconv", "foldt", "foldall", "foldck8", "foldgemm", "croll", "froll", "prepack", "wsplitbn",
-    "capturefork", "sidechain", "headrank1",
+    "capturefork", "sidechain", "headrank1", "wbatch",
 };
 constexpr int kNumOffTokens = sizeof(kOffTokens) / sizeof(kOffTokens[0]);
 static_assert(kNumOffTokens <= 64, "BiuEnv::off holds one bit per token");
diff --git a/bio_image_unet_amd/csrc/biu_conv_mfma.hip b/bio_image_unet_amd/csrc/biu_conv_mfma.hip
--- a/bio_image_unet_amd/csrc/biu_conv_mfma.hip
+++ b/bio_image_unet_amd/csrc/biu_conv_mfma.hip
@@ -3714,7 +3714,10 @@
     const int taps = kd * 9;
     const size_t need = wgrad_acc_bytes(a.CA, a.CB, taps);
     BIU_REQUIRE(ws_bytes >= need + (dbias ? biu_chan_sum_workspace(dy->c) : 0), BIU_ERR_WORKSPACE, "wgrad_mfma: workspace %zu too small", ws_bytes);
-    if (int zr = zero_ws(ws, need, nullptr, 0, st)) return zr;
+    float* batched = nullptr;
+    if (int br = biu_wbatch_alloc(st, need, &batched)) return br;
+    if (batched) a.ws = batched;
+    else if (int zr = zero_ws(ws, need, nullptr, 0, st)) return zr;
     if (a.r1_dl) rc = launch_wgrad_roll(a, st);
     else if (dtype == BIU_BF16 && kd == 3 && a.CB == 16 && !x1 && !biu_off("rr16")) rc = launch_wgrad<bf16_t, 3, 3, 1, 4, 8, 16, 1, 1, true>(a, st);
     else if (dtype == BIU_BF16 && kd == 3 && !biu_off("wroll") && wroll_fits(a)) rc = launch_wgrad_roll(a, st);
@@ -3729,9 +3732,13 @@
     else if (kd == 3 && x3_mode_of(kd, dtype) == 1) rc = launch_wgrad<f32x3_t, 3, 3, 1, 2, 4, 16, 1>(a, st);
     else rc = (kd == 3) ? launch_wgrad<float, 3, 3, 1, 4, 4, 16, 1>(a, st) : launch_wgrad<float, 1, 3, 1, 1, 16, 16, 4>(a, st);
     if (rc != BIU_OK) return rc;
-    hipLaunchKernelGGL(k_wgrad_finalize, dim3(grid_for((i64)a.CA * a.CB * taps, 256, 2048)), dim3(256), 0, st, (const float*)ws,
-                       a.CA, a.CB, taps, dw, dw_ld_cols, dw_c_off);
-    BIU_CHECK_LAUNCH("wgrad_finalize");
+    if (batched) {
+        if (int br = biu_wbatch_job(st, BIU_WB_FINALIZE, batched, a.CA, a.CB, taps, dw, dw_ld_cols, dw_c_off)) return br;
+    } else {
+        hipLaunchKernelGGL(k_wgrad_finalize, dim3(grid_for((i64)a.CA * a.CB * taps, 256, 2048)), dim3(256), 0, st, (const float*)ws,
+                           a.CA, a.CB, taps, dw, dw_ld_cols, dw_c_off);
+        BIU_CHECK_LAUNCH("wgrad_finalize");
+    }
     if (dbias) return biu_chan_sum_vec(dy, dbias, (char*)ws + need, dtype, st);
     return BIU_OK;
 }
@@ -3762,7 +3769,7 @@
     return 8 * wgrad_acc_bytes(cout, cin, 8);
 }
 int biu_mfma_upconv_wgrad(const biu_act* x, const biu_xform* xf, const biu_act* dy, float* dw, void* ws, size_t ws_bytes, int dtype,
-                          hipStream_t st, const BnBwdFuse* bn) {
+                          hipStream_t st, const BnBwdFuse* bn, bool ws_is_zero) {
     WgradArgs a;
     if (bn) {
         a.py = (const char*)bn->y->p; a.ypitch = bn->y->pitch;
@@ -3783,7 +3790,13 @@
     a.GD = a.BD = x->d; a.GH = a.BH = x->h; a.GW = a.BW = x->w;
     const size_t slice = wgrad_acc_bytes(a.CA, a.CB, 8);
     BIU_REQUIRE(ws_bytes >= 8 * slice, BIU_ERR_WORKSPACE, "upconv_wgrad: workspace %zu too small (need %zu)", ws_bytes, 8 * slice);
-    if (int zr = zero_ws(ws, 8 * slice, nullptr, 0, st)) return zr;
+    float* batched = nullptr;
+    if (dw && !ws_is_zero) {
+        if (int br = biu_wbatch_alloc(st, 8 * slice, &batched)) return br;
+        if (batched) ws = batched;
+    }
+    if (!batched && !ws_is_zero)
+        if (int zr = zero_ws(ws, 8 * slice, nullptr, 0, st)) return zr;
     a.fold_slice_f = slice / sizeof(float);
     if (dtype == BIU_BF16 && a.CA <= biu_env().fall_maxca && bn == nullptr && !biu_off("foldall")) {
         a.ws = (float*)ws;
@@ -3801,6 +3814,7 @@
         if (rc != BIU_OK) return rc;
     }
     if (!dw) return BIU_OK;
+    if (batched) return biu_wbatch_job(st, BIU_WB_UNFOLD, batched, a.CA, a.CB, 27, dw, (int)(slice / sizeof(float)), 0);
     hipLaunchKernelGGL(k_upconv_wgrad_unfold, dim3(grid_for((i64)a.CA * a.CB * 27, 256, 2048)), dim3(256), 0, st, (const float*)ws, slice / sizeof(float),
                        a.CA, a.CB, dw);
     BIU_CHECK_LAUNCH("upconv_wgrad_unfold");
@@ -3992,10 +4006,17 @@
         if (rc != BIU_OK) return rc;
     }
     if (phases & 4) {
-        int rc = biu_mfma_upconv_wgrad(x_low, xf_low, da, nullptr, ws, main_bytes, dtype, st, nullptr);
+        const size_t gbytes = 8 * wgrad_acc_bytes(cout, cin_low, 8);
+        float* garena = nullptr;
+        if (int br = biu_wbatch_alloc(st, gbytes, &garena)) return br;
+        if (garena)
+            if (int br = biu_wbatch_g_put(st, ws, garena)) return br;
+        int rc = biu_mfma_upconv_wgrad(x_low, xf_low, da, nullptr, garena ? (void*)garena : ws, garena ? gbytes : main_bytes, dtype, st, nullptr, garena != nullptr);
         if (rc != BIU_OK) return rc;
     }
     if (!(phases & 2)) return BIU_OK;
+    float* const garena = biu_wbatch_g_take(ws);
+    const float* const G = garena ? garena : (const float*)ws;
     if (has_bias) {
         const ShellDims sh = shell_dims(da->n, da->d, da->h, da->w);
         BIU_DISPATCH_DTYPE(dtype, hipLaunchKernelGGL(k_foldt_border_sums<T>, dim3(FOLDT_SUM_BLOCKS), dim3(256), foldt_sum_lds(cout), st,
@@ -4009,19 +4030,19 @@
     const size_t slice_f = wgrad_acc_bytes(cout, cin_low, 8) / sizeof(float);
     if (cup <= cin_low && biu_fold_gemm_ok(cin_low, cup, cout)) {
         int rc = biu_fold_gemm_layouts(w_conv, ccat, cup, cout, w_t, cin_low, lay, st);
-        if (rc == BIU_OK) rc = biu_fold_gemm_chain((const float*)ws, slice_f, lay, cin_low, cup, cout, ccat, dw_conv, dw_t, b_t, (const float*)Sk, st);
+        if (rc == BIU_OK) rc = biu_fold_gemm_chain(G, slice_f, lay, cin_low, cup, cout, ccat, dw_conv, dw_t, b_t, (const float*)Sk, st);
         if (rc != BIU_OK) return rc;
         if (db_t) hipLaunchKernelGGL(k_foldt_chain_bt, dim3(cup), dim3(256), 0, st, (const float*)Sk, w_conv, cup, cout, ccat, db_t);
         BIU_CHECK_LAUNCH("foldt_chain_bt");
-        return BIU_OK;
-    }
-    hipLaunchKernelGGL(k_foldt_chain_wconv, dim3((cup + 31) / 32, (cout + 31) / 32, 27), dim3(256), 0, st, (const float*)ws, slice_f, w_t, cin_low, cup, cout, ccat,
+        return garena ? biu_wbatch_clear(st, garena, 8 * slice_f) : BIU_OK;
+    }
+    hipLaunchKernelGGL(k_foldt_chain_wconv, dim3((cup + 31) / 32, (cout + 31) / 32, 27), dim3(256), 0, st, G, slice_f, w_t, cin_low, cup, cout, ccat,
                        dw_conv, b_t, (const float*)Sk);
-    hipLaunchKernelGGL(k_foldt_chain_wt, dim3((cup + 31) / 32, (cin_low + 31) / 32, 8), dim3(256), 0, st, (const float*)ws, slice_f, w_conv, cin_low, cup, cout, ccat,
+    hipLaunchKernelGGL(k_foldt_chain_wt, dim3((cup + 31) / 32, (cin_low + 31) / 32, 8), dim3(256), 0, st, G, slice_f, w_conv, cin_low, cup, cout, ccat,
                        dw_t);
     if (db_t) hipLaunchKernelGGL(k_foldt_chain_bt, dim3(cup), dim3(256), 0, st, (const float*)Sk, w_conv, cup, cout, ccat, db_t);
     BIU_CHECK_LAUNCH("foldt_chain");
-    return BIU_OK;
+    return garena ? biu_wbatch_clear(st, garena, 8 * slice_f) : BIU_OK;
 }
 
 int biu_mfma_convt_wgrad(const biu_act* x, const biu_xform* xf, const biu_act* dy, int kd, float* dw, float* dbias, void* ws,
@@ -4044,7 +4065,14 @@
     const size_t need = wgrad_acc_bytes(a.CA, a.CB, taps);
     BIU_REQUIRE(ws_bytes >= need + (dbias ? biu_chan_sum_workspace(dy->c) : 0), BIU_ERR_WORKSPACE, "convt_wgrad_mfma: workspace %zu too small", ws_bytes);
     a.dbias_out = dbias;
-    if (int zr = zero_ws(ws, need, dbias, dbias ? dy->c : 0, st)) return zr;
+    float *batched = nullptr, *bias_acc = nullptr;
+    if (int br = biu_wbatch_alloc(st, need, &batched)) return br;
+    if (batched && dbias) {
+        if (int br = biu_wbatch_alloc(st, (size_t)dy->c * sizeof(float), &bias_acc)) return br;
+        a.dbias_out = bias_acc;
+    }
+    if (batched) a.ws = batched;
+    else if (int zr = zero_ws(ws, need, dbias, dbias ? dy->c : 0, st)) return zr;
     const bool wide = a.CA > 32;
     if (dtype == BIU_BF16) {
         if (wide) rc = (kd == 2) ? launch_wgrad<bf16_t, 2, 2, 2, 2, 4, 16, 2, 2>(a, st) : launch_wgrad<bf16_t, 1, 2, 2, 1, 8, 16, 4, 2>(a, st);
@@ -4058,6 +4086,10 @@
         else rc = (kd == 2) ? launch_wgrad<float, 2, 2, 2, 2, 4, 16, 2>(a, st) : launch_wgrad<float, 1, 2, 2, 1, 8, 16, 4>(a, st);
     }
     if (rc != BIU_OK) return rc;
+    if (batched) {
+        if (int br = biu_wbatch_job(st, BIU_WB_FINALIZE, batched, a.CA, a.CB, taps, dw, 0, 0)) return br;
+        return bias_acc ? biu_wbatch_job(st, BIU_WB_FINALIZE, bias_acc, 1, dy->c, 1, dbias, 0, 0) : BIU_OK;
+    }
     hipLaunchKernelGGL(k_wgrad_finalize, dim3(grid_for((i64)a.CA * a.CB * taps, 256, 2048)), dim3(256), 0, st, (const float*)ws,
                        a.CA, a.CB, taps, dw);
     BIU_CHECK_LAUNCH("convt_wgrad_finalize");
diff --git a/bio_image_unet_amd/csrc/biu_internal.h b/bio_image_unet_amd/csrc/biu_internal.h
--- a/bio_image_unet_amd/csrc/biu_internal.h
+++ b/bio_image_unet_amd/csrc/biu_internal.h
@@ -91,7 +91,7 @@
 struct BnBwdFuse;
 size_t biu_mfma_upconv_wgrad_workspace(int cin, int cout, int dtype);
 int biu_mfma_upconv_wgrad(const biu_act* x, const biu_xform* xf, const biu_act* dy, float* dw, void* ws, size_t ws_bytes, int dtype,
-                          hipStream_t st, const BnBwdFuse* bn);
+                          hipStream_t st, const BnBwdFuse* bn, bool ws_is_zero = false);
 int biu_mfma_upconv_stat_rows(const biu_act* x, const biu_act* y);
 int biu_mfma_upconv_fwd(const biu_act* x, const biu_xform* xf, const void* packed, const float* bias, const biu_act* y, float* bn_partial,
                         int dtype, hipStream_t st, int accumulate = 0);
@@ -118,6 +118,14 @@
 bool biu_mfma_convt_wgrad_ok(const biu_act* x, const biu_act* dy, int kd, int dtype);
 int biu_mfma_convt_wgrad(const biu_act* x, const biu_xform* xf, const biu_act* dy, int kd, float* dw, float* dbias, void* ws,
                          size_t ws_bytes, int dtype, hipStream_t st);
+
+enum { BIU_WB_FINALIZE = 0, BIU_WB_UNFOLD = 1, BIU_WB_ZERO = 2 };
+bool biu_wbatch_open(hipStream_t st);
+int biu_wbatch_alloc(hipStream_t st, size_t bytes, float** out);
+int biu_wbatch_job(hipStream_t st, int kind, float* acc, int rows, int cols, int taps, float* dw, int ld_cols, int c_off);
+int biu_wbatch_g_put(hipStream_t st, const void* key, float* g);
+float* biu_wbatch_g_take(const void* key);
+int biu_wbatch_clear(hipStream_t st, float* p, size_t floats);
 
 bool biu_c1_conv_ok(const biu_act* x, const biu_act* y, int kd, int kh, int kw, int dil, int dtype);
 int biu_c1_conv_fwd(const biu_act* x, const biu_xform* xf, const float* w, const float* bias, int kd, const biu_act* y, int dtype, hipStream_t st);
diff --git a/bio_image_unet_amd/csrc/biu_wbatch.hip b/bio_image_unet_amd/csrc/biu_wbatch.hip
--- /dev/null
+++ b/bio_image_unet_amd/csrc/biu_wbatch.hip
@@ -0,0 +1,285 @@
+#include "biu_common.h"
+#include "biu_internal.h"
+
+#include <mutex>
+
+namespace {
+
+struct WbJob {
+    float* acc;
+    float* dw;
+    int rows, cols, taps;
+    int ld_cols, c_off;
+    int kind;
+    int blk0, nblk;
+};
+constexpr int WB_TABLE = 24;
+struct WbTable {
+    WbJob j[WB_TABLE];
+    int n;
+};
+
+constexpr int WB_MAX_OPEN = 8, WB_MAX_PENDING = 96, WB_MAX_LIVE_G = 8;
+struct WbBatch {
+    bool open;
+    hipStream_t st;
+    char* arena;
+    size_t bytes, used;
+    int* state;
+    bool failed;
+    int npending;
+    WbJob pending[WB_MAX_PENDING];
+    int nlive;
+    struct { const void* key; float* g; } live[WB_MAX_LIVE_G];
+};
+WbBatch g_batches[WB_MAX_OPEN];
+std::mutex g_mu;
+
+WbBatch* find_open(hipStream_t st) {
+    for (auto& b : g_batches)
+        if (b.open && b.st == st) return &b;
+    return nullptr;
+}
+
+constexpr int WB_STRIP = 64, WB_TILE_TAPS = 32;
+__device__ __forceinline__ void wb_finalize_tiled(const WbJob& j, int blk, float* tile) {
+    const int nstrips = (j.cols + WB_STRIP - 1) / WB_STRIP, ld = j.ld_cols > 0 ? j.ld_cols : j.cols;
+    const int items = j.rows * nstrips;
+    for (int item = blk; item < items; item += j.nblk) {
+        const int rr = item / nstrips, c0 = (item % nstrips) * WB_STRIP;
+        const int cw = j.cols - c0 < WB_STRIP ? j.cols - c0 : WB_STRIP, n = cw * j.taps;
+        for (int e = threadIdx.x; e < n; e += 256) {
+            const int tap = e / cw, c = e - tap * cw;
+            float* a = j.acc + ((size_t)tap * j.rows + rr) * j.cols + c0 + c;
+            tile[c * j.taps + tap] = *a;
+            *a = 0.f;
+        }
+        __syncthreads();
+        float* out = j.dw + ((size_t)rr * ld + (j.ld_cols > 0 ? j.c_off : 0) + c0) * j.taps;
+        for (int e = threadIdx.x; e < n; e += 256) out[e] = tile[e];
+        __syncthreads();
+    }
+}
+
+__device__ __forceinline__ void wb_finalize(const WbJob& j, int blk) {
+    const size_t total = (size_t)j.rows * j.cols * j.taps;
+    for (size_t i = (size_t)blk * 256 + threadIdx.x; i < total; i += (size_t)j.nblk * 256) {
+        const int tap = (int)(i % j.taps);
+        const size_t r = i / j.taps;
+        const int c = (int)(r % j.cols);
+        const int rr = (int)(r / j.cols);
+        const size_t o = j.ld_cols > 0 ? ((size_t)rr * j.ld_cols + j.c_off + c) * j.taps + tap : i;
+        const size_t s = ((size_t)tap * j.rows + rr) * j.cols + c;
+        j.dw[o] = j.acc[s];
+        j.acc[s] = 0.f;
+    }
+}
+
+__device__ __forceinline__ void wb_unfold(const WbJob& j, int blk) {
+    const size_t pairs = (size_t)j.rows * j.cols, slice_f = (size_t)j.ld_cols;
+    for (size_t r = (size_t)blk * 256 + threadIdx.x; r < pairs; r += (size_t)j.nblk * 256) {
+        float g[64];
+#pragma unroll
+        for (int p = 0; p < 8; ++p)
+#pragma unroll
+            for (int t = 0; t < 8; ++t) {
+                float* a = j.acc + (size_t)p * slice_f + (size_t)t * pairs + r;
+                g[p * 8 + t] = *a;
+                *a = 0.f;
+            }
+#pragma unroll
+        for (int k = 0; k < 27; ++k) {
+            const int kk[3] = {k / 9, (k / 3) % 3, k % 3};
+            float sum = 0.f;
+#pragma unroll
+            for (int p = 0; p < 8; ++p) {
+                int t = 0;
+#pragma unroll
+                for (int ax = 0; ax < 3; ++ax) {
+                    const int pa = (p >> (2 - ax)) & 1;
+                    const int ta = pa == 0 ? (kk[ax] >= 1 ? 1 : 0) : (kk[ax] == 2 ? 1 : 0);
+                    t |= ta << (2 - ax);
+                }
+                sum += g[p * 8 + t];
+            }
+            j.dw[r * 27 + k] = sum;
+        }
+    }
+}
+
+__device__ __forceinline__ void wb_zero(const WbJob& j, int blk) {
+    const size_t total = (size_t)j.rows * j.cols * j.taps;
+    for (size_t i = (size_t)blk * 256 + threadIdx.x; i < total; i += (size_t)j.nblk * 256) j.acc[i] = 0.f;
+}
+
+__global__ __launch_bounds__(256) void k_wbatch_flush(const WbTable t) {
+    int sel = 0;
+    for (int i = 1; i < t.n; ++i)
+        if ((int)blockIdx.x >= t.j[i].blk0) sel = i;
+    const WbJob j = t.j[sel];
+    const int blk = (int)blockIdx.x - j.blk0;
+    __shared__ float tile[WB_STRIP * WB_TILE_TAPS];
+    if (j.kind == BIU_WB_FINALIZE && j.taps <= WB_TILE_TAPS) wb_finalize_tiled(j, blk, tile);
+    else if (j.kind == BIU_WB_FINALIZE) wb_finalize(j, blk);
+    else if (j.kind == BIU_WB_UNFOLD) wb_unfold(j, blk);
+    else wb_zero(j, blk);
+}
+
+__global__ void k_wbatch_zero(float* __restrict__ p, size_t n) {
+    for (size_t i = (size_t)blockIdx.x * blockDim.x + threadIdx.x; i < n; i += (size_t)gridDim.x * blockDim.x) p[i] = 0.f;
+}
+
+int launch_zero(float* p, size_t n, hipStream_t st) {
+    if (n == 0) return BIU_OK;
+    hipLaunchKernelGGL(k_wbatch_zero, dim3(grid_for((i64)((n + 3) / 4), 256, 2048)), dim3(256), 0, st, p, n);
+    BIU_CHECK_LAUNCH("wbatch_zero");
+    return BIU_OK;
+}
+
+int flush_locked(WbBatch* b) {
+    for (int first = 0; first < b->npending; first += WB_TABLE) {
+        WbTable t;
+        t.n = b->npending - first < WB_TABLE ? b->npending - first : WB_TABLE;
+        int blocks = 0;
+        for (int i = 0; i < t.n; ++i) {
+            WbJob& j = t.j[i];
+            j = b->pending[first + i];
+            j.blk0 = blocks;
+            if (j.kind == BIU_WB_UNFOLD) j.nblk = grid_for((i64)j.rows * j.cols, 256, 1024);
+            else if (j.kind == BIU_WB_FINALIZE && j.taps <= WB_TILE_TAPS) j.nblk = grid_for((i64)j.rows * ((j.cols + WB_STRIP - 1) / WB_STRIP), 1, 2048);
+            else j.nblk = grid_for((i64)j.rows * j.cols * j.taps, 1024, 1024);
+            blocks += j.nblk;
+        }
+        for (int i = t.n; i < WB_TABLE; ++i) t.j[i] = WbJob{};
+        hipLaunchKernelGGL(k_wbatch_flush, dim3(blocks), dim3(256), 0, b->st, t);
+        if (hipGetLastError() != hipSuccess) {
+            b->failed = true;
+            b->npending = 0;
+            return biu_fail(BIU_ERR_LAUNCH, "wbatch_flush: launch failed");
+        }
+    }
+    b->npending = 0;
+    return BIU_OK;
+}
+
+}
+
+bool biu_wbatch_open(hipStream_t st) {
+    std::lock_guard<std::mutex> lk(g_mu);
+    return find_open(st) != nullptr;
+}
+
+int biu_wbatch_alloc(hipStream_t st, size_t bytes, float** out) {
+    std::lock_guard<std::mutex> lk(g_mu);
+    *out = nullptr;
+    WbBatch* b = find_open(st);
+    if (!b) return BIU_OK;
+    bytes = (bytes + 255) & ~(size_t)255;
+    BIU_REQUIRE(b->used + bytes <= b->bytes, BIU_ERR_WORKSPACE, "wbatch: arena of %zu bytes is full (%zu used, %zu more asked)", b->bytes, b->used, bytes);
+    *out = (float*)(b->arena + b->used);
+    b->used += bytes;
+    *b->state = 0;
+    return BIU_OK;
+}
+
+int biu_wbatch_job(hipStream_t st, int kind, float* acc, int rows, int cols, int taps, float* dw, int ld_cols, int c_off) {
+    std::lock_guard<std::mutex> lk(g_mu);
+    WbBatch* b = find_open(st);
+    BIU_REQUIRE(b, BIU_ERR_UNSUPPORTED, "wbatch: no batch is open on this stream");
+    if (b->npending == WB_MAX_PENDING)
+        if (int rc = flush_locked(b)) return rc;
+    WbJob j{};
+    j.acc = acc; j.dw = dw; j.rows = rows; j.cols = cols; j.taps = taps; j.ld_cols = ld_cols; j.c_off = c_off; j.kind = kind;
+    b->pending[b->npending++] = j;
+    return BIU_OK;
+}
+
+int biu_wbatch_g_put(hipStream_t st, const void* key, float* g) {
+    std::lock_guard<std::mutex> lk(g_mu);
+    WbBatch* b = find_open(st);
+    BIU_REQUIRE(b && b->nlive < WB_MAX_LIVE_G, BIU_ERR_UNSUPPORTED, "wbatch: more than %d folded levels between their parts 4 and 2", WB_MAX_LIVE_G);
+    for (int i = 0; i < b->nlive; ++i)
+        if (b->live[i].key == key) {
+            b->failed = true;
+            b->live[i].g = g;
+            return BIU_OK;
+        }
+    b->live[b->nlive].key = key;
+    b->live[b->nlive++].g = g;
+    return BIU_OK;
+}
+
+float* biu_wbatch_g_take(const void* key) {
+    std::lock_guard<std::mutex> lk(g_mu);
+    for (auto& b : g_batches) {
+        if (!b.open) continue;
+        for (int i = 0; i < b.nlive; ++i)
+            if (b.live[i].key == key) {
+                float* g = b.live[i].g;
+                b.live[i] = b.live[--b.nlive];
+                return g;
+            }
+    }
+    return nullptr;
+}
+
+int biu_wbatch_clear(hipStream_t st, float* p, size_t floats) {
+    BIU_REQUIRE(floats < ((size_t)1 << 31), BIU_ERR_SHAPE, "wbatch: region of %zu floats", floats);
+    if (biu_wbatch_open(st)) return biu_wbatch_job(st, BIU_WB_ZERO, p, 1, (int)floats, 1, nullptr, 0, 0);
+    return launch_zero(p, floats, st);
+}
+
+extern "C" size_t biu_wbatch_acc_bytes(int rows, int cols, int taps) {
+    if (rows <= 0 || cols <= 0 || taps <= 0) return 0;
+    return (((size_t)rows * cols * taps * sizeof(float)) + 255) & ~(size_t)255;
+}
+
+extern "C" int biu_wbatch_table_jobs(void) { return WB_TABLE; }
+
+extern "C" int biu_wbatch_begin(void* arena, size_t arena_bytes, int* state, biu_stream stream) {
+    if (biu_off("wbatch")) return BIU_OK;
+    BIU_REQUIRE(arena && state && (uintptr_t)arena % 256 == 0 && arena_bytes % sizeof(float) == 0, BIU_ERR_SHAPE,
+                "wbatch_begin: the arena must be 256-byte aligned, with a state word");
+    hipStream_t st = (hipStream_t)stream;
+    std::lock_guard<std::mutex> lk(g_mu);
+    BIU_REQUIRE(!find_open(st), BIU_ERR_UNSUPPORTED, "wbatch_begin: a batch is already open on this stream");
+    WbBatch* b = nullptr;
+    for (auto& c : g_batches) {
+        BIU_REQUIRE(!(c.open && c.arena == (char*)arena), BIU_ERR_UNSUPPORTED, "wbatch_begin: the arena belongs to an open batch");
+        if (!c.open && !b) b = &c;
+    }
+    BIU_REQUIRE(b, BIU_ERR_UNSUPPORTED, "wbatch_begin: %d batches are open", WB_MAX_OPEN);
+    if (*state != 1) {
+        if (int rc = launch_zero((float*)arena, arena_bytes / sizeof(float), st)) return rc;
+    }
+    *state = 1;
+    b->open = true; b->st = st; b->arena = (char*)arena; b->bytes = arena_bytes; b->used = 0; b->state = state;
+    b->failed = false; b->npending = 0; b->nlive = 0;
+    return BIU_OK;
+}
+
+extern "C" int biu_wbatch_flush(biu_stream stream) {
+    std::lock_guard<std::mutex> lk(g_mu);
+    WbBatch* b = find_open((hipStream_t)stream);
+    if (!b) return BIU_OK;
+    return flush_locked(b);
+}
+
+extern "C" int biu_wbatch_end(biu_stream stream) {
+    std::lock_guard<std::mutex> lk(g_mu);
+    WbBatch* b = find_open((hipStream_t)stream);
+    if (!b) return BIU_OK;
+    const int rc = flush_locked(b);
+    *b->state = (rc == BIU_OK && !b->failed && b->nlive == 0) ? 1 : 0;
+    b->open = false;
+    return rc;
+}
+
+extern "C" int biu_wbatch_abort(biu_stream stream) {
+    std::lock_guard<std::mutex> lk(g_mu);
+    WbBatch* b = find_open((hipStream_t)stream);
+    if (!b) return BIU_OK;
+    *b->state = 0;
+    b->open = false;
+    return BIU_OK;
+}
diff --git a/bio_image_unet_amd/engine.py b/bio_image_unet_amd/engine.py
--- a/bio_image_unet_amd/engine.py
+++ b/bio_image_unet_amd/engine.py
@@ -313,6 +313,14 @@
                                        lambda dst, st, kind=kind: lib.biu_conv_pack(kind, _ptr(w.data), *geom, dt, dst, st), job=(0, kind) + geom)
                                 for kind in (0, 1))
         eng.need_ws(lib.biu_conv_bwd_weight_workspace(*geom, dt))
+        acc = lib.biu_wbatch_acc_bytes
+        nb = acc(cout, xin.c, self.kd * self.kh * self.kw)
+        if self.form == "foldt":
+            nb = acc(cout, parts[1].c, 27) + 8 * acc(cout, convt.xin.c, 8)
+        elif self.fold_wg:
+            nb = 8 * acc(cout, xin.c, 8)
+        eng.need_wbatch(nb, side=self.form == "plain" and not self.fold_wg and self.kd == 3 and eng.tdtype == torch.bfloat16
+                        and yout.nvox <= _SIDE_WGRAD_VOX)
         eng.need_ws(lib.biu_conv_split_workspace(xin.c, yout.a(), None, self.kd, self.kh, self.kw, self.dil, dt))
         eng.need_ws(lib.biu_conv_split_workspace(cout, parts[0].a(), parts[1].a() if len(parts) == 2 else None, self.kd, self.kh, self.kw, self.dil, dt))
 
@@ -519,6 +527,7 @@
                                        lambda dst, st, kind=kind: lib.biu_convt_pack(kind, _ptr(w.data), *geom, dt, dst, st), job=(1, kind) + geom + (2, 2))
                                 for kind in (0, 1))
         eng.need_ws(lib.biu_convt_bwd_weight_workspace(*geom, dt))
+        eng.need_wbatch(lib.biu_wbatch_acc_bytes(xin.c, yout.c, self.kd * 4) + lib.biu_wbatch_acc_bytes(1, yout.c, 1))
 
     def fwd(self, eng):
         if self.folded_into is not None:
@@ -841,6 +850,11 @@
         self._side = None
         self._deferred = []
         self._fold_ev = None
+        self._wb_bytes = {"main": 0, "side": 0}
+        self._wb_arena: Dict[str, tuple] = {}
+        self._wb_open: Dict[str, tuple] = {}
+        self._wb_on = False
+        self.wbatch = True
 
     def busy(self) -> bool:
         return self._live is not None and self._live() is not None
@@ -879,12 +893,20 @@
     def need_ws(self, nbytes):
         self.ws_bytes = max(self.ws_bytes, int(nbytes))
 
+    def need_wbatch(self, nbytes, side: bool = False):
+        self._wb_bytes["main"] += int(nbytes)
+        if side:
+            self._wb_bytes["side"] += int(nbytes)
+
     def finalize(self):
         dev = self.device
         c = max(self._partial_c, 1)
         self.partial = torch.empty(max(BN_MAX_PARTIALS * c * 2, self._partial_floats), dtype=torch.float32, device=dev)
         self.coef = torch.empty((3, c), dtype=torch.float32, device=dev)
         self.ws = torch.empty(max(self.ws_bytes, 16), dtype=torch.uint8, device=dev)
+        for name, nbytes in self._wb_bytes.items():
+            if nbytes:
+                self._wb_arena[name] = (torch.empty(nbytes, dtype=torch.uint8, device=dev), C.c_int(0))
         seen = set()
         for nd_ in self.nodes:
             for p in nd_.params:
@@ -943,13 +965,36 @@
 
     def add_grad(self, p: nn.Parameter, g: torch.Tensor):
         if p in self.grads:
+            self._wb_flush()
             self.grads[p] = self.grads[p] + g
         else:
             self.grads[p] = g
         if self.grad_hook is not None:
             self._pseen[p] = self._pseen.get(p, 0) + 1
             if self._pseen[p] == self._pcount.get(p, 1):
+                self._wb_flush()
                 self.grad_hook(p, self.grads[p])
+
+    def _wb_begin(self, name: str):
+        if not self._wb_on or name in self._wb_open or name not in self._wb_arena:
+            return
+        arena, state = self._wb_arena[name]
+        if torch.cuda.is_current_stream_capturing():
+            state = C.c_int(0)
+        st = _stream()
+        check(lib._c.biu_wbatch_begin(_ptr(arena), arena.numel(), C.byref(state), st), "wbatch_begin")
+        self._wb_open[name] = (st, state)
+
+    def _wb_flush(self):
+        if self._wb_open:
+            check(lib._c.biu_wbatch_flush(_stream()), "wbatch_flush")
+
+    def _wb_close(self, abort: bool):
+        opened, self._wb_open = self._wb_open, {}
+        rcs = [lib._c.biu_wbatch_abort(st) if abort else lib._c.biu_wbatch_end(st) for st, _ in opened.values()]
+        if not abort:
+            for rc in rcs:
+                check(rc, "wbatch_end")
 
     def load_inputs(self, xs: Sequence[torch.Tensor]):
         st = _stream()
@@ -1020,7 +1065,9 @@
         label = lib.label
         with torch.cuda.stream(side):
             lib.label = label + suffix
+            self._wb_begin("side")
             yield
+            self._wb_flush()
             done.record(side)
         lib.label = label
         self._deferred.append((done, grads, keep))
@@ -1041,6 +1088,18 @@
             for k in b.leaves:
                 b.leaves[k] = False
                 b.nwr[k] = 0
+        self._wb_on = self.wbatch and self.trace is None
+        try:
+            self._wb_begin("main")
+            self._backward_nodes(head_grads)
+            self._flush_deferred(0)
+            self._wb_close(abort=False)
+        except BaseException:
+            self._wb_close(abort=True)
+            raise
+        return self.grads
+
+    def _backward_nodes(self, head_grads):
         lib.label = "head:bwd"
         if self.trace:
             self.trace("bwd", ("heads", head_grads), "pre")
@@ -1057,8 +1116,6 @@
             nd_.bwd(self)
             if self.trace:
                 self.trace("bwd", nd_, "post")
-        self._flush_deferred(0)
-        return self.grads
 
     def _backward_heads(self, head_grads):
         live = [(h, g) for h, g in zip(self.heads, head_grads) if g is not None]
diff --git a/include/biu.h b/include/biu.h
--- a/include/biu.h
+++ b/include/biu.h
@@ -256,6 +256,13 @@
                                      const float* b_t, int cup, float* dw_conv, float* dw_t, float* db_t, void* ws, size_t ws_bytes, int dtype,
                                      int phases, biu_stream stream);
 
+size_t biu_wbatch_acc_bytes(int rows, int cols, int taps);
+int    biu_wbatch_table_jobs(void);
+int    biu_wbatch_begin(void* arena, size_t arena_bytes, int* state, biu_stream stream);
+int    biu_wbatch_flush(biu_stream stream);
+int    biu_wbatch_end(biu_stream stream);
+int    biu_wbatch_abort(biu_stream stream);
+
 int biu_head_fwd(const biu_act* x, const biu_xform* xf, const float* w, const float* bias, int cout,
                  int act, float* logits, float* activated, int dtype, biu_stream stream);
 size_t biu_head_bwd_workspace(int cin);
```
